# gereonsuch/gr-FDC

Hardware: AMD Instinct MI355X
Metric: complex Msamples/s in, 64k-FFT/256-ch overlap-save; achieved HBM GB/s vs peak (higher is better)
Workload: dtype f32

## Files before the change

gr-fdc_amd/__init__.py:

```python
from ._lib import FdcError, lib, LIB_PATH
from .blocks import overlap_save, vector_cut_vxx, phase_shifting_windowing_vcc, fft_vcc, window_table
from .channelizer import (FrequencyDomainChannelizer, Pipeline, PipelineGroup, IQ_SC16, IQ_SC8, OQ_FC32, plan_preview, FREQMODE, VERBOSEMODE, WINDOWTYPES,
                          nextpow2, get_opt_channelparams, freq_converters, register_host, unregister_host, defaults, fine_tuning_increment, fine_tuning_nu)
from ._lib import (FDC_PIPE_FORCE_GENERIC, FDC_PIPE_NO_POLY, FDC_PIPE_NO_BLOCK, FDC_PIPE_PLAIN_STORES, FDC_PIPE_NT_LOADS,
                   FDC_PIPE_FULL_SPECTRUM, FDC_PIPE_WIDE_UNIFORM, FDC_PIPE_NO_FUSED,
                   FDC_SINKS_HOST_DECISIONS, FDC_SINKS_DEVICE_PAYLOAD, FDC_SINKS_LOOKAHEAD)
from .waterfall import Waterfall, WaterfallImage, Rows as WaterfallRows
from .sharding import span_for_rank, ring_bounds, ring_for_span
from .sinks import Sinks, SinksGroup, PowerActivationChannel, activity_detection_channelizer_vcm, SegmentDetection
```

gr-fdc_amd/_lib.py:

```python
import ctypes as C
import os

_HERE = os.path.dirname(os.path.abspath(__file__))
LIB_PATH = os.environ.get("FDC_AMD_LIB") or os.path.join(_HERE, "libfdc_amd.so")

FDC_OK = 0
STATUS_NAMES = {0: "FDC_OK", -1: "FDC_ERR_INVALID_ARGUMENT", -2: "FDC_ERR_HIP", -3: "FDC_ERR_NO_DEVICE",
                -4: "FDC_ERR_UNSUPPORTED", -5: "FDC_ERR_NOMEM"}


class FdcError(RuntimeError):
    def __init__(self, status, text):
        self.status = status
        super().__init__("%s: %s" % (STATUS_NAMES.get(status, status), text))


class fdc_channel(C.Structure):
    _fields_ = [("f", C.c_int32), ("l", C.c_int32), ("passbw", C.c_float), ("stopbw", C.c_float)]


class fdc_pipeline_cfg(C.Structure):
    _fields_ = [("device_id", C.c_int32), ("blocklen", C.c_int32), ("relinvovl", C.c_int32),
                ("windowtype", C.c_int32), ("nchannels", C.c_int32), ("channels", C.POINTER(fdc_channel)),
                ("max_blocks", C.c_int32), ("chunk_blocks", C.c_int32), ("keep_spectrum", C.c_int32),
                ("flags", C.c_int32), ("min_block_launch", C.c_int32), ("host_sub_blocks", C.c_int32)]


FDC_PIPE_FORCE_GENERIC, FDC_PIPE_NO_POLY, FDC_PIPE_NO_BLOCK, FDC_PIPE_PLAIN_STORES, FDC_PIPE_NT_LOADS = 1, 2, 4, 8, 16
FDC_PIPE_FULL_SPECTRUM = 32
FDC_PIPE_WIDE_UNIFORM = 64
FDC_PIPE_NO_FUSED = 128


class fdc_pac_cfg(C.Structure):
    _fields_ = [("cfreq", C.c_float), ("bw", C.c_float), ("id", C.c_int32)]


class fdc_segment_cfg(C.Structure):
    _fields_ = [("start", C.c_float), ("stop", C.c_float)]


class fdc_sinks_cfg(C.Structure):
    _fields_ = [("device_id", C.c_int32), ("blocklen", C.c_int32), ("relinvovl", C.c_int32),
                ("npac", C.c_int32), ("pac", C.POINTER(fdc_pac_cfg)),
                ("pac_thresh_db", C.c_float), ("pac_maxblocks", C.c_int32), ("pac_deactivation_delay", C.c_int32),
                ("nseg", C.c_int32), ("seg", C.POINTER(fdc_segment_cfg)),
                ("det_thresh_db", C.c_float), ("det_maxblocks", C.c_int32), ("minchandist", C.c_float),
                ("det_deactivation_delay", C.c_int32), ("window_flank_puffer", C.c_double), ("max_blocks", C.c_int32),
                ("det_variant", C.c_int32), ("verbose", C.c_int32), ("det_id", C.c_int32), ("flags", C.c_int32),
                ("threads", C.c_int32), ("seg_id_base", C.c_int32)]


FDC_SINKS_HOST_DECISIONS = 1
FDC_SINKS_DEVICE_PAYLOAD = 2
FDC_SINKS_LOOKAHEAD = 4
FDC_OQ_FC32, FDC_OQ_SC16, FDC_OQ_SC8 = 0, 1, 2


class fdc_pdu(C.Structure):
    _fields_ = [("kind", C.c_int32), ("source", C.c_int32), ("chan_id", C.c_int32), ("finalized", C.c_int32),
                ("part", C.c_int32), ("has_part", C.c_int32), ("rel_bw", C.c_double), ("rel_cfreq", C.c_double),
                ("blockstart", C.c_int64), ("blockend", C.c_int64), ("vectorstart", C.c_int64),
                ("vectorend", C.c_int64), ("nsamples", C.c_int64), ("samples", C.c_void_p), ("id", C.c_char * 72)]


class fdc_waterfall_cfg(C.Structure):
    _fields_ = [("blocklen", C.c_int32), ("blockdecimation", C.c_int32), ("loginput", C.c_int32),
                ("minvaldb", C.c_double), ("maxvaldb", C.c_double), ("colorscheme", C.c_int32)]


_vp = C.c_void_p
SYMBOLS = {
    "fdc_last_error": (C.c_char_p, []),
    "fdc_version": (C.c_char_p, []),
    "fdc_device_count": (C.c_int, []),
    "fdc_selftest_devices": (C.c_int, []),
    "fdc_selftest_exception_barrier": (C.c_int, []),
    "fdc_pipeline_create": (C.c_int, [C.POINTER(fdc_pipeline_cfg), C.POINTER(_vp)]),
    "fdc_pipeline_destroy": (None, [_vp]),
    "fdc_pipeline_input_samples": (C.c_int64, [_vp, C.c_int]),
    "fdc_pipeline_output_samples": (C.c_int64, [_vp, C.c_int]),
    "fdc_pipeline_channel_offset": (C.c_int64, [_vp, C.c_int, C.c_int]),
    "fdc_pipeline_channel_lout": (C.c_int32, [_vp, C.c_int]),
    "fdc_pipeline_work": (C.c_int, [_vp, _vp, C.c_int, C.POINTER(_vp), _vp]),
    "fdc_pipeline_work_real": (C.c_int, [_vp, _vp, C.c_int, C.POINTER(_vp), _vp]),
    "fdc_pipeline_work_span": (C.c_int, [_vp, _vp, _vp, C.c_int64, C.c_int, C.POINTER(_vp), _vp]),
    "fdc_pipeline_work_span_real": (C.c_int, [_vp, _vp, _vp, C.c_int64, C.c_int, C.POINTER(_vp), _vp]),
    "fdc_pipeline_work_iq": (C.c_int, [_vp, C.c_int32, C.c_float, _vp, C.c_int, C.POINTER(_vp), _vp]),
    "fdc_pipeline_work_span_iq": (C.c_int, [_vp, C.c_int32, C.c_float, _vp, _vp, C.c_int64, C.c_int, C.POINTER(_vp), _vp]),
    "fdc_pipeline_process_device_iq": (C.c_int, [_vp, C.c_int32, C.c_float, _vp, C.c_int64, C.c_int, _vp, _vp, _vp]),
    "fdc_pipeline_group_work_iq": (C.c_int, [_vp, C.c_int32, C.c_float, _vp, C.c_int, C.POINTER(_vp), _vp]),
    "fdc_pipeline_set_output_format": (C.c_int, [_vp, C.c_int32, C.c_float]),
    "fdc_pipeline_group_set_output_format": (C.c_int, [_vp, C.c_int32, C.c_float]),
    "fdc_fine_tuning_increment": (C.c_int, [C.c_double, C.POINTER(C.c_uint64)]),
    "fdc_pipeline_set_fine_tuning": (C.c_int, [_vp, C.POINTER(C.c_double), C.c_int]),
    "fdc_pipeline_group_set_fine_tuning": (C.c_int, [_vp, C.POINTER(C.c_double), C.c_int]),
    "fdc_pipeline_group_create": (C.c_int, [C.POINTER(fdc_pipeline_cfg), C.POINTER(C.c_int32), C.c_int, C.c_int, C.POINTER(_vp)]),
    "fdc_pipeline_group_destroy": (None, [_vp]),
    "fdc_pipeline_group_work": (C.c_int, [_vp, _vp, C.c_int, C.POINTER(_vp), _vp]),
    "fdc_pipeline_group_work_real": (C.c_int, [_vp, _vp, C.c_int, C.POINTER(_vp), _vp]),
    "fdc_pipeline_group_reset": (None, [_vp]),
    "fdc_pipeline_group_size": (C.c_int32, [_vp]),
    "fdc_pipeline_group_member": (_vp, [_vp, C.c_int]),
    "fdc_pipeline_group_device": (C.c_int32, [_vp, C.c_int]),
    "fdc_pipeline_group_member_max_blocks": (C.c_int32, [_vp]),
    "fdc_pipeline_group_last_spans": (C.c_int, [_vp, C.POINTER(C.c_int64), C.POINTER(C.c_int32), C.c_int]),
    "fdc_host_register": (C.c_int, [_vp, C.c_size_t]),
    "fdc_host_unregister": (C.c_int, [_vp]),
    "fdc_pipeline_reset": (None, [_vp]),
    "fdc_pipeline_process_device": (C.c_int, [_vp, _vp, C.c_int64, C.c_int, _vp, _vp, _vp]),
    "fdc_pipeline_synchronize": (C.c_int, [_vp]),
    "fdc_pipeline_stream": (_vp, [_vp]),
    "fdc_pipeline_reserve_compute_units": (C.c_int, [_vp, C.c_int32]),
    "fdc_pipeline_chunk_blocks": (C.c_int32, [_vp]),
    "fdc_pipeline_path": (C.c_int32, [_vp]),
    "fdc_pipeline_describe": (C.c_int32, [_vp, C.c_char_p, C.c_int32]),
    "fdc_pipeline_plan_preview": (C.c_int, [C.POINTER(fdc_pipeline_cfg), C.c_char_p, C.c_int32, C.POINTER(C.c_int32)]),
    "fdc_pipeline_enable_timing": (C.c_int, [_vp, C.c_int]),
    "fdc_pipeline_last_kernel_ms": (C.c_int, [_vp, C.POINTER(C.c_float), C.c_int]),
    "fdc_sinks_create": (C.c_int, [C.POINTER(fdc_sinks_cfg), C.POINTER(_vp)]),
    "fdc_sinks_destroy": (None, [_vp]),
    "fdc_pipeline_work_spectrum": (C.c_int, [_vp, _vp, C.c_int, C.POINTER(_vp), _vp, _vp]),
    "fdc_pipeline_work_sinks": (C.c_int, [_vp, _vp, C.c_int, C.POINTER(_vp), _vp, _vp]),
    "fdc_device_numa_node": (C.c_int, [C.c_int]),
    "fdc_selftest_worker_placement": (C.c_int, [C.c_int, C.POINTER(C.c_int32), C.POINTER(C.c_int32)]),
    "fdc_pipeline_process_device_power": (C.c_int, [_vp, _vp, C.c_int64, C.c_int, _vp, _vp, _vp, _vp]),
    "fdc_sinks_group_power": (_vp, [_vp]),
    "fdc_sinks_group_power_ahead": (_vp, [_vp]),
    "fdc_sinks_prepare_from_groups": (C.c_int, [_vp, C.c_int, C.c_int]),
    "fdc_pipeline_flush_sinks": (C.c_int, [_vp, _vp]),
    "fdc_pipeline_sinks_latency": (C.c_int32, [_vp, _vp]),
    "fdc_sinks_work": (C.c_int, [_vp, _vp, C.c_int]),
    "fdc_sinks_work_band": (C.c_int, [_vp, _vp, C.c_int, C.c_int32, C.c_int32]),
    "fdc_sinks_read_band": (C.c_int, [_vp, C.POINTER(C.c_int32), C.POINTER(C.c_int32)]),
    "fdc_sinks_pdu_emit_items": (C.c_int, [_vp, C.POINTER(C.c_int32), C.c_int]),
    "fdc_sinks_pdu_emit_order": (C.c_int, [_vp, C.POINTER(C.c_int32), C.POINTER(C.c_int32), C.c_int]),
    "fdc_sinks_group_create": (C.c_int, [C.POINTER(fdc_sinks_cfg), C.POINTER(C.c_int32), C.c_int, C.POINTER(_vp)]),
    "fdc_sinks_group_destroy": (None, [_vp]),
    "fdc_sinks_group_work": (C.c_int, [_vp, _vp, C.c_int]),
    "fdc_sinks_group_pdu_count": (C.c_int, [_vp]),
    "fdc_sinks_group_pdus": (C.c_int, [_vp, C.POINTER(fdc_pdu), C.c_int]),
    "fdc_sinks_group_size": (C.c_int32, [_vp]),
    "fdc_sinks_group_member": (_vp, [_vp, C.c_int]),
    "fdc_sinks_group_member_info": (C.c_int, [_vp, C.c_int] + [C.POINTER(C.c_int32)] * 5),
    "fdc_sinks_spectrum": (_vp, [_vp]),
    "fdc_sinks_stream": (_vp, [_vp]),
    "fdc_sinks_spectrum_ahead": (_vp, [_vp]),
    "fdc_sinks_fill_stream": (_vp, [_vp]),
    "fdc_sinks_prepare": (C.c_int, [_vp, C.c_int, C.c_int]),
    "fdc_sinks_blocklen": (C.c_int32, [_vp]),
    "fdc_sinks_max_blocks": (C.c_int32, [_vp]),
    "fdc_sinks_work_device": (C.c_int, [_vp, C.c_int]),
    "fdc_sinks_submit_device": (C.c_int, [_vp, C.c_int]),
    "fdc_sinks_flush": (C.c_int, [_vp]),
    "fdc_sinks_engine": (C.c_int32, [_vp]),
    "fdc_sinks_set_payload_format": (C.c_int, [_vp, C.c_int32, C.c_float]),
    "fdc_sinks_payload_format": (C.c_int, [_vp, C.POINTER(C.c_int32), C.POINTER(C.c_float)]),
    "fdc_sinks_payload_route": (C.c_int32, [_vp]),
    "fdc_sinks_group_set_payload_format": (C.c_int, [_vp, C.c_int32, C.c_float]),
    "fdc_set_log_callback": (None, [_vp, _vp]),
    "fdc_sinks_pdu_count": (C.c_int, [_vp]),
    "fdc_sinks_pdu": (C.c_int, [_vp, C.c_int, C.POINTER(fdc_pdu)]),
    "fdc_sinks_pdus": (C.c_int, [_vp, C.POINTER(fdc_pdu), C.c_int]),
    "fdc_sinks_pac_params": (C.c_int, [_vp, C.c_int, C.POINTER(C.c_int32)]),
    "fdc_sinks_segment_params": (C.c_int, [_vp, C.c_int, C.POINTER(C.c_int32)]),
    "fdc_overlap_save_create": (C.c_int, [C.c_int, C.c_int, C.c_int, C.c_int, C.POINTER(_vp)]),
    "fdc_overlap_save_work": (C.c_int, [_vp, _vp, C.c_int, _vp]),
    "fdc_overlap_save_destroy": (None, [_vp]),
    "fdc_vector_cut_create": (C.c_int, [C.c_int, C.c_int, C.c_int, C.c_int, C.c_int, C.POINTER(_vp)]),
    "fdc_vector_cut_work": (C.c_int, [_vp, _vp, C.c_int, _vp]),
    "fdc_vector_cut_destroy": (None, [_vp]),
    "fdc_phase_window_create": (C.c_int, [C.c_int, C.c_int, C.c_int, C.c_int, C.c_float, C.c_float, C.c_int,
                                          C.POINTER(_vp)]),
    "fdc_phase_window_work": (C.c_int, [_vp, _vp, C.c_int, _vp]),
    "fdc_phase_window_destroy": (None, [_vp]),
    "fdc_window_table": (C.c_int, [C.c_int, C.c_int, C.c_float, C.c_float, C.c_int, C.c_int, C.c_int, _vp]),
    "fdc_fft_vcc": (C.c_int, [C.c_int, C.c_int, C.c_int, C.c_int, _vp, C.c_int, _vp]),
    "fdc_waterfall_check": (C.c_int, [C.POINTER(fdc_waterfall_cfg), C.POINTER(fdc_waterfall_cfg)]),
    "fdc_waterfall_create": (C.c_int, [C.c_int, C.POINTER(fdc_waterfall_cfg), C.c_int32, C.POINTER(_vp)]),
    "fdc_waterfall_destroy": (None, [_vp]),
    "fdc_waterfall_reset": (None, [_vp]),
    "fdc_waterfall_set_levels": (C.c_int, [_vp, C.c_double, C.c_double]),
    "fdc_waterfall_set_colorscheme": (C.c_int, [_vp, C.c_int32]),
    "fdc_waterfall_rows_done": (C.c_int64, [_vp]),
    "fdc_waterfall_color_table": (C.c_int, [C.c_int32, _vp, _vp]),
    "fdc_waterfall_edges": (C.c_int, [C.c_int32, C.c_double, C.c_double, _vp]),
    "fdc_waterfall_work": (C.c_int, [_vp, _vp, C.c_int, _vp, _vp, _vp, C.c_int, C.POINTER(C.c_int32)]),
    "fdc_pipeline_work_waterfall": (C.c_int, [_vp, _vp, _vp, C.c_int, C.POINTER(_vp), _vp, _vp, _vp, C.c_int,
                                              C.POINTER(C.c_int32)]),
}

_lib = None


def lib():
    global _lib
    if _lib is None:
        if not os.path.exists(LIB_PATH):
            raise ImportError("gr-fdc_amd: %s is missing — build it with `make -C gr-fdc_amd/csrc` "
                              "(or __graft_entry__.build()); there is no CPU fallback" % LIB_PATH)
        h = C.CDLL(LIB_PATH)
        for name, (res, args) in SYMBOLS.items():
            fn = getattr(h, name)
            fn.restype = res
            fn.argtypes = args
        _lib = h
    return _lib


def check(status):
    if status < 0:
        raise FdcError(status, lib().fdc_last_error().decode())
    return status
```

gr-fdc_amd/channelizer.py:

```python
import ctypes as C
import math

import numpy as np

from . import _lib


class FREQMODE:
    normalized, basebandfs, centerfreqfs = range(3)


class VERBOSEMODE:
    NOLOG, LOGTOCONSOLE, LOGTOFILE = range(3)


class WINDOWTYPES:
    RECTANGULAR, HANN, RAMP = range(3)


def nextpow2(k):
    if k < 1:
        raise ValueError('Cannot evaluate next power 2 of {}'.format(k))
    return 1 << int(math.ceil(math.log2(k)))


def get_opt_channelparams(blocksize, relinvovl, freq, bw):
    occupied = blocksize * bw
    l = nextpow2(occupied)
    if l < 1.2 * occupied:
        l *= 2
    passband = float(occupied) / float(l) * 1.1
    stopband = 1.0
    if passband >= 1.0:
        passband = 1.0
    elif passband < 0.7:
        stopband = passband + 0.25
    centre = int(_round_half_away(freq * blocksize)) % blocksize
    first = centre - l / 2
    if first < 0:
        first = (first + blocksize) % blocksize
    if first + l > blocksize:
        first = blocksize - l
    return int(first), int(l), int(l) - int(l) // relinvovl, float(passband), float(stopband)


def _round_half_away(x):
    ax = abs(x)
    r = math.floor(ax)
    if ax - r >= 0.5:
        r += 1.0
    return r if x >= 0 else -r


def freq_converters(freqmode, fs=1.0, centerfrequency=0.0):
    if freqmode in (FREQMODE.normalized, 'normalized'):
        return (FREQMODE.normalized, lambda f: (f + 0.5) % 1.0, lambda f: f - 0.5, lambda bw: bw % 1.0, lambda bw: bw)
    if freqmode in (FREQMODE.basebandfs, 'basebandfs'):
        return (FREQMODE.basebandfs, lambda f: (f / fs + 0.5) % 1.0, lambda f: (f - 0.5) * fs,
                lambda bw: (bw / fs) % 1.0, lambda bw: bw * fs)
    if freqmode in (FREQMODE.centerfreqfs, 'centerfreqfs'):
        return (FREQMODE.centerfreqfs, lambda f: ((f - centerfrequency) / fs + 0.5) % 1.0,
                lambda f: (f - 0.5) * fs + centerfrequency, lambda bw: (bw / fs) % 1.0, lambda bw: bw * fs)
    raise ValueError('Unknown Frequency mode. Exiting...')


def register_host(arr):
    _lib.check(_lib.lib().fdc_host_register(arr.ctypes.data, arr.nbytes))


def unregister_host(arr):
    _lib.check(_lib.lib().fdc_host_unregister(arr.ctypes.data))


defaults = {}


def _default_cfg_fields():
    flags = 0
    if defaults.get("FDC_FORCE_GENERIC"):
        flags |= _lib.FDC_PIPE_FORCE_GENERIC
    if defaults.get("FDC_NO_POLY"):
        flags |= _lib.FDC_PIPE_NO_POLY
    if defaults.get("FDC_NO_BLOCK"):
        flags |= _lib.FDC_PIPE_NO_BLOCK
    if defaults.get("FDC_FULL_SPECTRUM"):
        flags |= _lib.FDC_PIPE_FULL_SPECTRUM
    if defaults.get("FDC_WIDE_UNIFORM"):
        flags |= _lib.FDC_PIPE_WIDE_UNIFORM
    if defaults.get("FDC_NO_FUSED"):
        flags |= _lib.FDC_PIPE_NO_FUSED
    if "FDC_BLOCK_HINTS" in defaults:
        h = int(defaults["FDC_BLOCK_HINTS"])
        flags |= (0 if h & 1 else _lib.FDC_PIPE_PLAIN_STORES) | (_lib.FDC_PIPE_NT_LOADS if h & 2 else 0)
    return flags, int(defaults.get("FDC_BLOCK_MIN_BLOCKS", 0) or 0), int(defaults.get("FDC_HOST_SUB", 0) or 0)


def plan_preview(blocklen, relinvovl, channels, windowtype=WINDOWTYPES.HANN, max_blocks=64, flags=0):
    chans = [(int(f), int(l), float(p), float(s)) for (f, l, p, s) in channels]
    arr = (_lib.fdc_channel * max(1, len(chans)))()
    for i, (f, l, p, s) in enumerate(chans):
        arr[i].f, arr[i].l, arr[i].passbw, arr[i].stopbw = f, l, p, s
    cfg = _lib.fdc_pipeline_cfg(0, int(blocklen), int(relinvovl), int(windowtype), len(chans), arr, int(max_blocks), 0, 0, int(flags), 0, 0)
    buf = C.create_string_buffer(640)
    asg = (C.c_int32 * max(1, len(chans)))()
    rc = _lib.lib().fdc_pipeline_plan_preview(C.byref(cfg), buf, 640, asg)
    if rc == -1:
        raise ValueError(_lib.lib().fdc_last_error().decode())
    _lib.check(rc)
    return rc, buf.value.decode(), [int(asg[i]) for i in range(len(chans))]


IQ_SC16, IQ_SC8 = 1, 2
IQ_FORMATS = {"sc16": IQ_SC16, "sc8": IQ_SC8}


def iq_format(x):
    dt = np.asarray(x).dtype if not isinstance(x, np.dtype) else x
    if dt == np.int16:
        return IQ_SC16
    if dt == np.int8:
        return IQ_SC8
    raise TypeError("complex integer input is int16 (sc16) or int8 (sc8) interleaved I/Q, not %s" % dt)


def _iq_input(x, scale, H):
    if not isinstance(x, np.ndarray):
        raise TypeError("complex integer input must be a numpy int16 or int8 array")
    fmt = iq_format(x)
    if x.ndim == 2:
        if x.shape[1] != 2:
            raise ValueError("complex integer input of shape (n, 2) holds I and Q in its columns; got shape %s" % (x.shape,))
    elif x.ndim != 1:
        raise ValueError("complex integer input is a flat interleaved array or one of shape (n, 2); got shape %s" % (x.shape,))
    elif x.size % 2:
        raise ValueError("a flat interleaved I/Q array has an even number of values")
    n = x.size // 2
    if H and n % H:
        raise ValueError("input must be a whole number of (N - N/R)-sample items")
    with np.errstate(over="ignore"):
        sc = np.float32(scale)
    if not np.isfinite(sc) or sc == 0:
        raise ValueError("scale must be finite and not zero (float32), got %r" % (scale,))
    return np.ascontiguousarray(x), fmt, n, sc


OQ_FC32 = 0
OQ_FORMATS = {None: OQ_FC32, "fc32": OQ_FC32, "sc16": IQ_SC16, "sc8": IQ_SC8}
_OQ_DTYPES = {IQ_SC16: np.int16, IQ_SC8: np.int8}


def _oq_format(fmt, scale):
    if not (fmt is None or isinstance(fmt, str)) or fmt not in OQ_FORMATS:
        raise ValueError("output format is None, 'fc32', 'sc16' or 'sc8', not %r" % (fmt,))
    try:
        with np.errstate(over="ignore"):
            sc = np.float32(scale)
    except (TypeError, ValueError):
        raise ValueError("scale must be a finite, non-zero number, got %r" % (scale,))
    if not np.isfinite(sc) or sc == 0:
        raise ValueError("scale must be finite and not zero (float32), got %r" % (scale,))
    return OQ_FORMATS[fmt], sc


def fine_tuning_increment(nu):
    inc = C.c_uint64(0)
    rc = _lib.lib().fdc_fine_tuning_increment(float(nu), C.byref(inc))
    if rc == -1:
        raise ValueError(_lib.lib().fdc_last_error().decode())
    _lib.check(rc)
    return int(inc.value)


def fine_tuning_nu(blocksize, freq, f, l):
    d = float(freq) * blocksize - (f + l / 2.0)
    d -= blocksize * math.floor(d / blocksize + 0.5)
    return d / l


def _set_fine_tuning(fn, handle, nchan, nu):
    if nu is None:
        rc = fn(handle, None, nchan)
    else:
        arr = np.ascontiguousarray(nu, dtype=np.float64)
        if arr.ndim != 1:
            raise ValueError("fine tuning takes one frequency per channel")
        rc = fn(handle, arr.ctypes.data_as(C.POINTER(C.c_double)), int(arr.size))
    if rc == -1:
        raise ValueError(_lib.lib().fdc_last_error().decode())
    _lib.check(rc)


class _OutputFormat:
    _oq = OQ_FC32
    _oq_scale = np.float32(1.0)

    def output_format(self):
        return ({OQ_FC32: "fc32", IQ_SC16: "sc16", IQ_SC8: "sc8"}[self._oq], float(self._oq_scale))

    def _new_outs(self, nb):
        if self._oq == OQ_FC32:
            return [np.empty(nb * lo, dtype=np.complex64) for lo in self.lout]
        return [np.empty((nb * lo, 2), dtype=_OQ_DTYPES[self._oq]) for lo in self.lout]

    def _check_outs(self, outs, nb):
        if outs is None:
            return self._new_outs(nb)
        if len(outs) != len(self.lout):
            raise ValueError("outs needs one array per channel")
        dt = np.complex64 if self._oq == OQ_FC32 else _OQ_DTYPES[self._oq]
        per = 1 if self._oq == OQ_FC32 else 2
        for o, lo in zip(outs, self.lout):
            if not isinstance(o, np.ndarray) or o.dtype != dt or not o.flags.c_contiguous or o.size != per * nb * lo:
                if self._oq == OQ_FC32:
                    raise ValueError("outs[c] must be contiguous complex64 with nblocks*lout_c samples")
                raise ValueError("outs[c] must be contiguous %s with nblocks*lout_c interleaved I/Q samples (the output format)" % np.dtype(dt).name)
        return outs


class Pipeline(_OutputFormat):

    def __init__(self, blocklen, relinvovl, channels, windowtype=WINDOWTYPES.HANN, max_blocks=64,
                 device_id=0, chunk_blocks=0, keep_spectrum=False, flags=None, min_block_launch=None, host_sub_blocks=None):
        self._h = C.c_void_p()
        self.N, self.R = int(blocklen), int(relinvovl)
        self.channels = [(int(f), int(l), float(p), float(s)) for (f, l, p, s) in channels]
        arr = (_lib.fdc_channel * max(1, len(self.channels)))()
        for i, (f, l, p, s) in enumerate(self.channels):
            arr[i].f, arr[i].l, arr[i].passbw, arr[i].stopbw = f, l, p, s
        dflags, dmin, dsub = _default_cfg_fields()
        cfg = _lib.fdc_pipeline_cfg(device_id, self.N, self.R, int(windowtype), len(self.channels), arr,
                                    int(max_blocks), int(chunk_blocks), int(bool(keep_spectrum)),
                                    dflags if flags is None else int(flags), dmin if min_block_launch is None else int(min_block_launch),
                                    dsub if host_sub_blocks is None else int(host_sub_blocks))
        rc = _lib.lib().fdc_pipeline_create(C.byref(cfg), C.byref(self._h))
        if rc == -1:
            raise ValueError(_lib.lib().fdc_last_error().decode())
        _lib.check(rc)
        self.max_blocks = int(max_blocks)
        self.keep_spectrum = bool(keep_spectrum)
        self.ovl = self.N // self.R if self.N >= self.R else 0
        self.H = self.N - self.ovl
        self.lout = [_lib.lib().fdc_pipeline_channel_lout(self._h, c) for c in range(len(self.channels))]

    def output_samples(self, nblocks):
        return int(_lib.lib().fdc_pipeline_output_samples(self._h, nblocks))

    def channel_offset(self, c, nblocks):
        return int(_lib.lib().fdc_pipeline_channel_offset(self._h, c, nblocks))

    def set_output_format(self, fmt, scale=1.0):
        code, sc = _oq_format(fmt, scale)
        _lib.check(_lib.lib().fdc_pipeline_set_output_format(self._h, code, float(sc)))
        self._oq, self._oq_scale = code, sc if code else np.float32(1.0)

    def set_fine_tuning(self, nu):
        _set_fine_tuning(_lib.lib().fdc_pipeline_set_fine_tuning, self._h, len(self.channels), nu)

    def work(self, x, want_spectrum=False, sinks=None, outs=None):
        x = np.ascontiguousarray(x, dtype=np.complex64)
        if x.size % self.H:
            raise ValueError("input must be a whole number of (N - N/R)-sample items")
        nb = x.size // self.H
        outs = self._check_outs(outs, nb)
        ptrs = (C.c_void_p * max(1, len(outs)))(*[o.ctypes.data for o in outs])
        spec = np.empty(nb * self.N, dtype=np.complex64) if want_spectrum else None
        if sinks is not None:
            _lib.check(_lib.lib().fdc_pipeline_work_sinks(self._h, x.ctypes.data, nb, ptrs,
                                                         spec.ctypes.data if spec is not None else None, sinks._h))
        else:
            _lib.check(_lib.lib().fdc_pipeline_work(self._h, x.ctypes.data, nb, ptrs,
                                                   spec.ctypes.data if spec is not None else None))
        return (outs, spec) if want_spectrum else outs

    def work_waterfall(self, x, waterfall):
        from .waterfall import Rows, WIDTH
        x = np.ascontiguousarray(x, dtype=np.complex64)
        if x.size % self.H:
            raise ValueError("input must be a whole number of (N - N/R)-sample items")
        nb = x.size // self.H
        outs = [np.empty(nb * lo, dtype=np.complex64) for lo in self.lout]
        ptrs = (C.c_void_p * max(1, len(outs)))(*[o.ctypes.data for o in outs])
        cap = waterfall.rows_for(nb)
        rows, idx, rgb = np.empty((cap, WIDTH), np.float32), np.empty((cap, WIDTH), np.uint16), np.empty((cap, WIDTH, 3), np.uint8)
        n = C.c_int32(0)
        _lib.check(_lib.lib().fdc_pipeline_work_waterfall(self._h, waterfall._h, x.ctypes.data, nb, ptrs, rows.ctypes.data, idx.ctypes.data,
                                                          rgb.ctypes.data, cap, C.byref(n)))
        return outs, Rows(rows[:n.value], idx[:n.value], rgb[:n.value])

    def flush_sinks(self, sinks):
        return _lib.check(_lib.lib().fdc_pipeline_flush_sinks(self._h, sinks._h))

    def sinks_latency(self, sinks):
        return int(_lib.lib().fdc_pipeline_sinks_latency(self._h, sinks._h))

    def work_sinks_raw(self, in_ptr, nblocks, out_ptrs, sinks):
        return _lib.check(_lib.lib().fdc_pipeline_work_sinks(self._h, in_ptr, int(nblocks), out_ptrs, None, sinks._h))

    def work_real(self, x, want_spectrum=False):
        x = np.ascontiguousarray(x, dtype=np.float32)
        if x.size % self.H:
            raise ValueError("input must be a whole number of (N - N/R)-sample items")
        nb = x.size // self.H
        outs = self._new_outs(nb)
        ptrs = (C.c_void_p * max(1, len(outs)))(*[o.ctypes.data for o in outs])
        spec = np.empty(nb * self.N, dtype=np.complex64) if want_spectrum else None
        _lib.check(_lib.lib().fdc_pipeline_work_real(self._h, x.ctypes.data, nb, ptrs,
                                                    spec.ctypes.data if spec is not None else None))
        return (outs, spec) if want_spectrum else outs

    def work_iq(self, x, scale=1.0, want_spectrum=False, outs=None):
        x, fmt, n, sc = _iq_input(x, scale, self.H)
        nb = n // self.H
        outs = self._check_outs(outs, nb)
        ptrs = (C.c_void_p * max(1, len(outs)))(*[o.ctypes.data for o in outs])
        spec = np.empty(nb * self.N, dtype=np.complex64) if want_spectrum else None
        _lib.check(_lib.lib().fdc_pipeline_work_iq(self._h, fmt, float(sc), x.ctypes.data, nb, ptrs,
                                                  spec.ctypes.data if spec is not None else None))
        return (outs, spec) if want_spectrum else outs

    def work_span_iq(self, halo, x, first_block, scale=1.0, want_spectrum=False):
        x, fmt, n, sc = _iq_input(x, scale, self.H)
        hp = None
        if halo is not None:
            halo, hfmt, hn, _ = _iq_input(halo, scale, 0)
            if hfmt != fmt or hn != self.ovl:
                raise ValueError("halo: N/R samples of the input's format")
            hp = halo.ctypes.data
        nb = n // self.H
        outs = self._new_outs(nb)
        ptrs = (C.c_void_p * max(1, len(outs)))(*[o.ctypes.data for o in outs])
        spec = np.empty(nb * self.N, dtype=np.complex64) if want_spectrum else None
        _lib.check(_lib.lib().fdc_pipeline_work_span_iq(self._h, fmt, float(sc), hp, x.ctypes.data, int(first_block), nb, ptrs,
                                                       spec.ctypes.data if spec is not None else None))
        return (outs, spec) if want_spectrum else outs

    def work_raw(self, in_ptr, nblocks, out_ptrs):
        return _lib.check(_lib.lib().fdc_pipeline_work(self._h, in_ptr, int(nblocks), out_ptrs, None))

    def work_spectrum(self, spec_items, want_spectrum=False, sinks=None):
        spec_items = np.ascontiguousarray(spec_items, dtype=np.complex64)
        if spec_items.size % self.N:
            raise ValueError("input must be a whole number of N-sample spectrum items")
        nb = spec_items.size // self.N
        outs = [np.empty(nb * lo, dtype=np.complex64) for lo in self.lout]
        ptrs = (C.c_void_p * max(1, len(outs)))(*[o.ctypes.data for o in outs])
        spec = np.empty(nb * self.N, dtype=np.complex64) if want_spectrum else None
        _lib.check(_lib.lib().fdc_pipeline_work_spectrum(self._h, spec_items.ctypes.data, nb, ptrs,
                                                        spec.ctypes.data if spec is not None else None,
                                                        sinks._h if sinks is not None else None))
        return (outs, spec) if want_spectrum else outs

    def reset(self):
        _lib.lib().fdc_pipeline_reset(self._h)

    def process_device(self, d_ring, first_block, nblocks, d_out, d_spectrum=None, stream=None, d_group_power=None):
        if d_group_power:
            _lib.check(_lib.lib().fdc_pipeline_process_device_power(self._h, d_ring, int(first_block), int(nblocks), d_out, d_spectrum,
                                                                   d_group_power, stream))
        else:
            _lib.check(_lib.lib().fdc_pipeline_process_device(self._h, d_ring, int(first_block), int(nblocks), d_out,
                                                             d_spectrum, stream))

    def process_device_iq(self, fmt, scale, d_ring, first_block, nblocks, d_out, d_spectrum=None, stream=None):
        fmt = IQ_FORMATS.get(fmt, fmt) if isinstance(fmt, str) else int(fmt)
        if fmt not in (IQ_SC16, IQ_SC8):
            raise ValueError("fmt is 'sc16' or 'sc8'")
        _lib.check(_lib.lib().fdc_pipeline_process_device_iq(self._h, fmt, float(np.float32(scale)), d_ring, int(first_block), int(nblocks),
                                                            d_out, d_spectrum, stream))

    def synchronize(self):
        _lib.check(_lib.lib().fdc_pipeline_synchronize(self._h))

    def reserve_compute_units(self, n):
        return _lib.check(_lib.lib().fdc_pipeline_reserve_compute_units(self._h, int(n)))

    def stream(self):
        return _lib.lib().fdc_pipeline_stream(self._h)

    def enable_timing(self, on=True):
        _lib.check(_lib.lib().fdc_pipeline_enable_timing(self._h, int(on)))

    def last_kernel_ms(self):
        ms = (C.c_float * 4)()
        _lib.check(_lib.lib().fdc_pipeline_last_kernel_ms(self._h, ms, 4))
        return [float(v) for v in ms]

    def path(self):
        return int(_lib.lib().fdc_pipeline_path(self._h))

    def describe(self):
        buf = C.create_string_buffer(512)
        _lib.lib().fdc_pipeline_describe(self._h, buf, 512)
        return buf.value.decode()

    def chunk_blocks(self):
        return int(_lib.lib().fdc_pipeline_chunk_blocks(self._h))
# ... 340 lines not shown
```

gr-fdc_amd/csrc/fdc_api.hip:

```cpp
#include "fdc_pipeline.hpp"

#include <cstdarg>
#include <stdexcept>
#include <system_error>

using namespace fdc::pipe;

namespace {

thread_local std::string g_err;

struct HostRange { uintptr_t lo, hi, dev; };
std::mutex g_reg_mu;
std::vector<HostRange> g_reg;

}

namespace fdc {
const char *debug_env(const char *name)
{
    static const bool on = [] { const char *d = getenv("FDC_DEBUG_ENV"); return d && d[0] == '1'; }();
    return on ? getenv(name) : nullptr;
}
int set_error(int code, const char *fmt, ...)
{
    char buf[512];
    va_list ap;
    va_start(ap, fmt);
    vsnprintf(buf, sizeof buf, fmt, ap);
    va_end(ap);
    g_err = buf;
    return code;
}
int pick_device(int device_id)
{
    int n = 0;
    if (hipGetDeviceCount(&n) != hipSuccess || n <= 0)
        return set_error(FDC_ERR_NO_DEVICE, "no HIP device visible (this library has no CPU fallback)");
    if (device_id < 0 || device_id >= n) return set_error(FDC_ERR_INVALID_ARGUMENT, "device_id %d out of range [0,%d)", device_id, n);
    HIPCHK(hipSetDevice(device_id));
    static std::mutex mu;
    static std::vector<char> ready;
    std::lock_guard<std::mutex> lk(mu);
    if ((int)ready.size() < n) ready.resize((size_t)n, 0);
    if (!ready[(size_t)device_id]) {
        const hipError_t e = fdc::init_kernels();
        if (e != hipSuccess) return set_error(FDC_ERR_HIP, "kernel attribute setup failed: %s", hipGetErrorString(e));
        ready[(size_t)device_id] = 1;
    }
    return FDC_OK;
}

namespace pipe {
std::vector<float2> make_twiddles(int n)
{
    std::vector<float2> t(n);
    for (int k = 0; k < n; k++) {
        const double a = -2.0 * M_PI * double(k) / double(n);
        t[k] = make_float2(float(std::cos(a)), float(std::sin(a)));
    }
    return t;
}

bool host_registered(const void *ptr, size_t bytes, void **devptr)
{
    const uintptr_t a = reinterpret_cast<uintptr_t>(ptr);
    std::lock_guard<std::mutex> lk(g_reg_mu);
    for (const HostRange &r : g_reg)
        if (a >= r.lo && a + bytes <= r.hi) {
            if (devptr) *devptr = reinterpret_cast<void *>(r.dev + (a - r.lo));
            return true;
        }
    return false;
}

int out_staging(fdc_pipeline *p)
{
    if (p->sum_lout > 0 && !p->d_out) HIPCHK(p->d_out.alloc((size_t)p->cfg.max_blocks * p->sum_lout));
    return FDC_OK;
}
}
}

namespace fdc {
int pipeline_output_format(const fdc_pipeline *p, float *scale)
{
    if (scale) *scale = p->out_scale;
    return p->out_form;
}
}

extern "C" {

const char *fdc_last_error(void) { return g_err.c_str(); }
const char *fdc_version(void) { return "gr-fdc_amd 0.1 (gfx950)"; }

int fdc_device_count(void)
{
    int n = 0;
    if (hipGetDeviceCount(&n) != hipSuccess) return 0;
    return n;
}

int fdc_selftest_exception_barrier(void)
{
    struct Case { int kind, want; };
    const Case cases[] = {{0, FDC_ERR_NOMEM}, {1, FDC_ERR_NOMEM}, {2, FDC_ERR_HIP}, {3, FDC_ERR_HIP}, {4, 7}};
    for (const Case &c : cases) {
        const int got = fdc::guarded("fdc_selftest_exception_barrier", [&]() -> int {
            switch (c.kind) {
            case 0: throw std::bad_alloc();
            case 1: throw std::system_error(std::make_error_code(std::errc::resource_unavailable_try_again), "thread");
            case 2: throw std::runtime_error("runtime");
            case 3: throw 42;
            default: return 7;
            }
        });
        if (got != c.want) return set_error(FDC_ERR_HIP, "exception barrier: kind %d came back as %d, expected %d", c.kind, got, c.want);
        if (c.want < 0 && g_err.empty()) return set_error(FDC_ERR_HIP, "exception barrier: kind %d left no text", c.kind);
    }
    return FDC_OK;
}

int fdc_selftest_devices(void)
{
    FDC_ENTRY("fdc_selftest_devices")
    const int ndev = fdc_device_count();
    if (ndev <= 0) return set_error(FDC_ERR_NO_DEVICE, "no HIP device visible (this library has no CPU fallback)");
    constexpr int N = 65536, R = 2, C = 256, NB = 96, H = N - N / R, LOUT = 128;
    std::vector<fdc_channel> ch(C);
    for (int c = 0; c < C; c++) ch[(size_t)c] = fdc_channel{256 * c, 256, 0.88f, 1.0f};
    std::vector<float> x((size_t)2 * NB * H);
    uint32_t lcg = 12345u;
    for (float &v : x) { lcg = lcg * 1664525u + 1013904223u; v = (float)((int32_t)(lcg >> 8) - (1 << 23)) * (1.0f / (1 << 23)); }
    std::vector<std::vector<float>> out((size_t)C, std::vector<float>((size_t)2 * NB * LOUT));
    std::vector<void *> outs((size_t)C);
    for (int c = 0; c < C; c++) outs[(size_t)c] = out[(size_t)c].data();
    uint64_t ref = 0;
    auto checksum = [&](double *energy) {
        uint64_t h = 1469598103934665603ull;
        *energy = 0.0;
        for (int c = 0; c < C; c++) {
            const unsigned char *b = reinterpret_cast<const unsigned char *>(out[(size_t)c].data());
            for (size_t i = 0; i < out[(size_t)c].size() * sizeof(float); i++) { h ^= b[i]; h *= 1099511628211ull; }
            for (float v : out[(size_t)c]) *energy += (double)v * v;
        }
        return h;
    };
    fdc_pipeline_cfg cfg{};
    cfg.blocklen = N; cfg.relinvovl = R; cfg.windowtype = FDC_WIN_HANN; cfg.nchannels = C; cfg.channels = ch.data();
    cfg.max_blocks = NB; cfg.host_sub_blocks = NB;
    cfg.min_block_launch = 1;
    for (int d = 0; d < ndev; d++) {
        cfg.device_id = d;
        fdc_pipeline *p = nullptr;
        int rc = fdc_pipeline_create(&cfg, &p);
        if (rc != FDC_OK) return set_error(rc, "selftest: device %d: create failed: %s", d, std::string(g_err).c_str());
        if (fdc_pipeline_path(p) != 3) { fdc_pipeline_destroy(p); return set_error(FDC_ERR_UNSUPPORTED, "selftest: device %d: not on the one-kernel path", d); }
        rc = fdc_pipeline_work(p, x.data(), NB, outs.data(), nullptr);
        fdc_pipeline_destroy(p);
        if (rc != NB) return set_error(rc < 0 ? rc : FDC_ERR_HIP, "selftest: device %d: work failed: %s", d, std::string(g_err).c_str());
        double energy = 0.0;
        const uint64_t h = checksum(&energy);
        if (!(energy > 0.0)) return set_error(FDC_ERR_HIP, "selftest: device %d produced no output", d);
        if (d == 0) ref = h;
        else if (h != ref) return set_error(FDC_ERR_HIP, "selftest: device %d differs from device 0 (checksum %016llx vs %016llx)", d,
                                       (unsigned long long)h, (unsigned long long)ref);
    }
    {
        std::vector<int32_t> devs;
        for (int d = 0; d < std::max(ndev, 2); d++) devs.push_back(d % ndev);
        fdc_pipeline_group *g = nullptr;
        int rc = fdc_pipeline_group_create(&cfg, devs.data(), (int)devs.size(), 4, &g);
        if (rc != FDC_OK) return set_error(rc, "selftest: group over %d device(s): create failed: %s", ndev, std::string(g_err).c_str());
        for (auto &o : out) std::fill(o.begin(), o.end(), 0.0f);
        const int n1 = NB / 3, n2 = NB - n1;
        std::vector<void *> outs2((size_t)C);
        for (int c = 0; c < C; c++) outs2[(size_t)c] = out[(size_t)c].data() + (size_t)2 * n1 * LOUT;
        rc = fdc_pipeline_group_work(g, x.data(), n1, outs.data(), nullptr);
        if (rc == n1) rc = fdc_pipeline_group_work(g, x.data() + (size_t)2 * n1 * H, n2, outs2.data(), nullptr);
        fdc_pipeline_group_destroy(g);
        if (rc != n2) return set_error(rc < 0 ? rc : FDC_ERR_HIP, "selftest: group over %d device(s): work failed: %s", ndev, std::string(g_err).c_str());
        double energy = 0.0;
        const uint64_t h = checksum(&energy);
        if (h != ref) return set_error(FDC_ERR_HIP, "selftest: the group over %d device(s) differs from device 0 (checksum %016llx vs %016llx)", ndev,
                                  (unsigned long long)h, (unsigned long long)ref);
    }
    return ndev;
    FDC_ENTRY_END
}

int fdc_window_table(int windowtype, int blocklen, float passbw, float stopbw, int numphasestates, int step,
                     int normalize, float *w)
{
    FDC_ENTRY("fdc_window_table")
    if (blocklen < 1 || numphasestates < 1 || !w) return set_error(FDC_ERR_INVALID_ARGUMENT, "bad window table arguments");
    fdc::window_table(windowtype, blocklen, passbw, stopbw, numphasestates, step, normalize != 0,
                      reinterpret_cast<std::complex<float> *>(w));
    return FDC_OK;
    FDC_ENTRY_END
}

int fdc_host_register(void *ptr, size_t bytes)
{
    FDC_ENTRY("fdc_host_register")
    if (!ptr || !bytes) return set_error(FDC_ERR_INVALID_ARGUMENT, "fdc_host_register: empty range");
    int n = 0;
    if (hipGetDeviceCount(&n) != hipSuccess || n <= 0) return set_error(FDC_ERR_NO_DEVICE, "no HIP device visible");
    HIPCHK(hipHostRegister(ptr, bytes, hipHostRegisterMapped | hipHostRegisterPortable));
    void *dev = nullptr;
    hipError_t e = hipHostGetDevicePointer(&dev, ptr, 0);
    if (e != hipSuccess) { (void)hipHostUnregister(ptr); return set_error(FDC_ERR_HIP, "hipHostGetDevicePointer failed: %s", hipGetErrorString(e)); }
    const uintptr_t a = reinterpret_cast<uintptr_t>(ptr);
    std::lock_guard<std::mutex> lk(g_reg_mu);
    g_reg.push_back(HostRange{a, a + bytes, reinterpret_cast<uintptr_t>(dev)});
    return FDC_OK;
    FDC_ENTRY_END
}

int fdc_host_unregister(void *ptr)
{
    FDC_ENTRY("fdc_host_unregister")
    const uintptr_t a = reinterpret_cast<uintptr_t>(ptr);
    {
        std::lock_guard<std::mutex> lk(g_reg_mu);
        auto it = std::find_if(g_reg.begin(), g_reg.end(), [a](const HostRange &r) { return r.lo == a; });
        if (it == g_reg.end()) return set_error(FDC_ERR_INVALID_ARGUMENT, "fdc_host_unregister: range was not registered here");
        g_reg.erase(it);
    }
    HIPCHK(hipHostUnregister(ptr));
    return FDC_OK;
    FDC_ENTRY_END
}

void fdc_pipeline_destroy(fdc_pipeline *p)
{
    if (!p) return;
    if (p->stream) (void)hipStreamSynchronize(p->stream);
    if (p->ev_hier) { (void)hipEventSynchronize(p->ev_hier); (void)hipEventDestroy(p->ev_hier); }
    for (auto st : {p->s_in, p->s_out}) if (st) { (void)hipStreamSynchronize(st); (void)hipStreamDestroy(st); }
    for (auto e : p->events) (void)hipEventDestroy(e);
    for (int i = 0; i < 2; i++)
        for (auto e : {p->ev_in[i], p->ev_k[i], p->ev_out[i]}) if (e) (void)hipEventDestroy(e);
    if (p->stream) (void)hipStreamDestroy(p->stream);
    delete p;
}

int fdc_pipeline_create(const fdc_pipeline_cfg *cfg, fdc_pipeline **out)
{
    FDC_ENTRY("fdc_pipeline_create")
    if (!cfg || !out) return set_error(FDC_ERR_INVALID_ARGUMENT, "null argument");
    *out = nullptr;
    int rc = validate_cfg(cfg);
    if (rc != FDC_OK) return rc;
    rc = pick_device(cfg->device_id);
    if (rc != FDC_OK) return rc;

    fdc_pipeline *p = new fdc_pipeline();
    struct Owner { fdc_pipeline *p; ~Owner() { if (p) fdc_pipeline_destroy(p); } } owner{p};
    const int N = cfg->blocklen, R = cfg->relinvovl;
    p->cfg = *cfg; p->cfg.channels = nullptr;
    p->N = N; p->R = R; p->ovl = N / R; p->H = N - p->ovl; p->C = cfg->nchannels;
    std::vector<std::complex<float>> pool;
    build_channel_records(p, cfg, pool);

    const int flags = effective_flags(cfg->flags);
    p->cfg.flags = flags;
    p->cfg_generic = (flags & FDC_PIPE_FORCE_GENERIC) != 0;
    p->block_hints = ((flags & FDC_PIPE_PLAIN_STORES) ? 0 : 1) | ((flags & FDC_PIPE_NT_LOADS) ? 2 : 0);
    if (cfg->min_block_launch >= 1) p->block_min = cfg->min_block_launch;
    if (const char *bm = fdc::debug_env("FDC_BLOCK_MIN_BLOCKS")) if (atoi(bm) >= 1) p->block_min = atoi(bm);

    std::vector<int32_t> flat, rflat;
    group_by_width(p, nullptr, p->groups, p->group_off, p->g_aligned, p->g_out_aligned, flat);
    classify_plan(p, cfg, flags);
    if (p->split) group_by_width(p, &p->rem, p->rgroups, p->rgroup_off, p->rg_aligned, p->rg_out_aligned, rflat);

    int chunk = cfg->chunk_blocks;
    if (chunk <= 0) chunk = (int)std::max<int64_t>(1, (2048ll << 20) / (2ll * N * 8));
    p->chunk = std::min(chunk, cfg->max_blocks);

    rc = build_device_state(p, cfg, pool, flat, rflat);
    if (rc != FDC_OK) return rc;
    owner.p = nullptr;
    *out = p;
    return FDC_OK;
    FDC_ENTRY_END
}

int fdc_pipeline_plan_preview(const fdc_pipeline_cfg *cfg, char *buf, int32_t n, int32_t *assignment)
{
    FDC_ENTRY("fdc_pipeline_plan_preview")
    if (!cfg) return set_error(FDC_ERR_INVALID_ARGUMENT, "null argument");
    const int rc = validate_cfg(cfg);
    if (rc != FDC_OK) return rc;
    std::unique_ptr<fdc_pipeline> p(new fdc_pipeline());
    p->cfg = *cfg; p->cfg.channels = nullptr;
    p->N = cfg->blocklen; p->R = cfg->relinvovl; p->ovl = p->N / p->R; p->H = p->N - p->ovl; p->C = cfg->nchannels;
    std::vector<std::complex<float>> pool;
    build_channel_records(p.get(), cfg, pool);
    const int flags = effective_flags(cfg->flags);
    p->cfg.flags = flags;
    p->cfg_generic = (flags & FDC_PIPE_FORCE_GENERIC) != 0;
    classify_plan(p.get(), cfg, flags);
    if (assignment) {
        for (int c = 0; c < p->C; c++) assignment[c] = -1;
        for (size_t k = 0; k < p->banks.size(); k++) for (int c : p->banks[k].chan) assignment[c] = (int32_t)k;
        for (const auto &al : p->bank_alias) assignment[al.first] = -2 - al.second;
    }
    if (buf && n > 0) fdc_pipeline_describe(p.get(), buf, n);
    return fdc_pipeline_path(p.get());
    FDC_ENTRY_END
}

int64_t fdc_pipeline_input_samples(const fdc_pipeline *p, int nblocks) { return p ? (int64_t)nblocks * p->H : 0; }
int64_t fdc_pipeline_output_samples(const fdc_pipeline *p, int nblocks) { return p ? (int64_t)nblocks * p->sum_lout : 0; }
int64_t fdc_pipeline_channel_offset(const fdc_pipeline *p, int c, int nblocks)
{
    if (!p || c < 0 || c >= p->C) return -1;
    return (int64_t)nblocks * p->chans[c].out_off;
}
int32_t fdc_pipeline_channel_lout(const fdc_pipeline *p, int c)
{
    if (!p || c < 0 || c >= p->C) return -1;
    return p->chans[c].lout;
}
void *fdc_pipeline_stream(fdc_pipeline *p) { return p ? (void *)p->stream : nullptr; }
int fdc_pipeline_reserve_compute_units(fdc_pipeline *p, int32_t n)
{
    FDC_ENTRY("fdc_pipeline_reserve_compute_units")
    if (!p) return fdc::set_error(FDC_ERR_INVALID_ARGUMENT, "null handle");
    if (n < 0 || n >= p->ncu) return fdc::set_error(FDC_ERR_INVALID_ARGUMENT, "%d compute units of %d cannot be left out", (int)n, p->ncu);
    p->reserved_cu = n;
    p->reserve_user = n > 0;
    return p->ncu - n;
    FDC_ENTRY_END
}
int32_t fdc_pipeline_chunk_blocks(const fdc_pipeline *p) { return p ? p->chunk : -1; }
int32_t fdc_pipeline_path(const fdc_pipeline *p)
{
    if (!p) return -1;
    if (p->fused) return 5;
    if (p->poly_block && p->split) return 4;
    if (p->poly_block) return 3;
    if (p->poly_ok) return 2;
    if (p->fwd_block || (p->N == 65536 && !p->cfg_generic)) return 1;
    return 0;
}

int32_t fdc_pipeline_describe(const fdc_pipeline *p, char *buf, int32_t n)
{
    if (!p || !buf || n < 1) return -1;
    char t[640];
    const int path = fdc_pipeline_path(p);
    int k = std::snprintf(t, sizeof(t), "N = %d, R = %d, %d channels; path %d: ", p->N, p->R, p->C, path);
    auto add = [&](const char *fmt, auto... a) { if (k < (int)sizeof(t)) k += std::snprintf(t + k, sizeof(t) - (size_t)k, fmt, a...); };
    auto kernel = [](int L) { return L == 256 ? "k_blk256" : L == 512 ? "k_blk512" : L == 1024 ? "k_blk1024" : "k_blknar"; };
    auto where = [](int L, int r) { return r == 0 ? "on the grid" : 2 * r == L ? "half a channel off the grid" : 4 * r == L ? "a quarter of a channel off the grid" : "three quarters of a channel off the grid"; };
    if (p->fused) {
        int nw = 0;
        for (const auto &w : p->f4_wave) nw += !w.empty();
        add("k_f4096, transform + %d channel transforms in one launch (spectrum in LDS, %s per workgroup, rows on %d wave%s)", p->C,
            p->f4_teams == 1 ? "one block" : "two blocks", nw, nw == 1 ? "" : "s");
    } else if (p->poly_block) {
        bool one_width = true, all256 = true;
        for (const auto &b : p->banks) { one_width = one_width && b.L == p->banks[0].L; all256 = all256 && b.L == 256; }
        if (all256) {
            add("k_blk256, %d tiling%s (r =", (int)p->banks.size(), p->banks.size() == 1 ? "" : "s");
            for (const auto &b : p->banks) add(" %d", b.r);
            add("%s", ")");
        } else if (one_width) {
            add("%s, l = %d, bank of %d %s", kernel(p->banks[0].L), p->banks[0].L, (int)p->banks[0].chan.size(), where(p->banks[0].L, p->banks[0].r));
            for (size_t i = 1; i < p->banks.size(); i++) add(" + bank of %d %s", (int)p->banks[i].chan.size(), where(p->banks[i].L, p->banks[i].r));
        } else {
            for (size_t i = 0; i < p->banks.size(); i++) {
                const auto &b = p->banks[i];
                add("%s%s bank of %d, l = %d", i ? " + " : "", kernel(b.L), (int)b.chan.size(), b.L);
                if (b.L == 256) add(" (r = %d)", b.r); else add(" %s", where(b.L, b.r));
            }
        }
        if (p->banks.size() > 1 && !all256) add(" (%s launches)", p->banks.size() == 2 ? "two" : p->banks.size() == 3 ? "three" : "four");
        if (!p->bank_alias.empty()) add(" + %d copies of channels with the same slice", (int)p->bank_alias.size());
        if (p->split) add(" + %d other channels on a partial spectrum", (int)p->rem.size());
    } else if (p->poly_ok) {
        add("two launches (stage 1 + stage 2), l = %d", p->banks[0].L);
    } else {
        add("%s", "forward transform to a spectrum in memory + channel kernels");
    }
    if (!p->wf_route.empty()) add("; waterfall rows: %s", p->wf_route.c_str());
    if (!p->iq_route.empty()) add("; input %s", p->iq_route.c_str());
    if (!p->oq_route.empty()) add("; output %s", p->oq_route.c_str());
    if (!p->fine_route.empty()) add("; fine tuning: %s", p->fine_route.c_str());
    std::snprintf(buf, (size_t)n, "%s", t);
    return k;
}

int fdc_pipeline_synchronize(fdc_pipeline *p)
{
    FDC_ENTRY("fdc_pipeline_synchronize")
    if (!p) return set_error(FDC_ERR_INVALID_ARGUMENT, "null handle");
    HIPCHK(hipSetDevice(p->cfg.device_id));
    HIPCHK(hipStreamSynchronize(p->stream));
    return FDC_OK;
    FDC_ENTRY_END
}

int fdc_pipeline_enable_timing(fdc_pipeline *p, int enable)
{
    FDC_ENTRY("fdc_pipeline_enable_timing")
    if (!p) return set_error(FDC_ERR_INVALID_ARGUMENT, "null handle");
    p->timing = enable != 0;
    p->timing_stride = enable > 1 ? enable : 1;
    p->timing_seq = 0;
    p->ev_used = 0; p->ev_spans.clear();
    return FDC_OK;
    FDC_ENTRY_END
}

int fdc_pipeline_last_kernel_ms(fdc_pipeline *p, float *ms, int n)
{
    FDC_ENTRY("fdc_pipeline_last_kernel_ms")
    if (!p || !ms || n < 4) return set_error(FDC_ERR_INVALID_ARGUMENT, "need room for 4 values");
    ms[0] = ms[1] = ms[2] = 0.f;
    ms[3] = (float)p->ev_spans.size();
    for (auto &sp : p->ev_spans) {
        float a = 0, b = 0, c = 0;
        HIPCHK(hipEventSynchronize(p->events[sp[3]]));
        HIPCHK(hipEventElapsedTime(&a, p->events[sp[0]], p->events[sp[1]]));
        HIPCHK(hipEventElapsedTime(&b, p->events[sp[1]], p->events[sp[2]]));
        HIPCHK(hipEventElapsedTime(&c, p->events[sp[2]], p->events[sp[3]]));
        switch ((int)sp[4]) {
        case kSpanBanks: ms[0] += a; ms[1] += b; ms[2] += c; break;
        case kSpanTwoLaunch: ms[0] += a; ms[1] += c; break;
        case kSpanSpectrumLds: ms[1] += a + b; ms[2] += c; break;
        default: ms[0] += a; ms[1] += b; ms[2] += c;
        }
    }
    p->ev_used = 0; p->ev_spans.clear();
    return 4;
    FDC_ENTRY_END
}

void fdc_pipeline_reset(fdc_pipeline *p)
{
    if (!p) return;
    p->blockcount = 0;
    if (p->ev_hier && p->hier_ring_busy) (void)hipEventSynchronize(p->ev_hier);
    if (p->d_ring) {
        (void)hipSetDevice(p->cfg.device_id);
        (void)hipMemsetAsync(p->d_ring, 0, sizeof(float2) * (size_t)p->ovl, p->stream);
        if (p->d_iq) (void)hipMemsetAsync(p->d_iq, 0, fdc::kIqRingBytes * (size_t)p->ovl, p->stream);
        (void)hipStreamSynchronize(p->stream);
    }
    p->in_form = -1;
    p->in_scale = 0.f;
    p->iq_route.clear();
    p->oq_route.clear();
    p->fine_route.clear();
}

int fdc_pipeline_set_output_format(fdc_pipeline *p, int32_t format, float scale)
{
    FDC_ENTRY("fdc_pipeline_set_output_format")
    if (!p) return set_error(FDC_ERR_INVALID_ARGUMENT, "null handle");
    if (format != FDC_OQ_FC32 && format != FDC_OQ_SC16 && format != FDC_OQ_SC8) return set_error(FDC_ERR_INVALID_ARGUMENT, "unknown output format %d", (int)format);
    if (!std::isfinite(scale) || scale == 0.0f) return set_error(FDC_ERR_INVALID_ARGUMENT, "the output scale must be finite and not zero");
    if (p->hier_filled > 0)
        return set_error(FDC_ERR_INVALID_ARGUMENT, "a pipelined sinks batch is still inside the handle: fdc_pipeline_flush_sinks until it returns 0 first");
    if (format && !p->d_out) {
        HIPCHK(hipSetDevice(p->cfg.device_id));
        RCCHK(out_staging(p));
    }
    p->out_form = format;
    p->out_scale = format ? scale : 1.0f;
    return FDC_OK;
    FDC_ENTRY_END
}

int fdc_fine_tuning_increment(double nu, uint64_t *inc)
{
    FDC_ENTRY("fdc_fine_tuning_increment")
    if (!inc) return set_error(FDC_ERR_INVALID_ARGUMENT, "null argument");
    if (!(std::fabs(nu) < 0.5)) return set_error(FDC_ERR_INVALID_ARGUMENT, "the fine-tuning frequency must be inside (-0.5, 0.5) cycles per output sample");
    const double r = std::nearbyint(std::ldexp(nu, 64));
    *inc = r < 0 ? (uint64_t)0 - (uint64_t)(-r) : (uint64_t)r;
    return FDC_OK;
    FDC_ENTRY_END
}

int fdc_pipeline_set_fine_tuning(fdc_pipeline *p, const double *nu, int n)
{
    FDC_ENTRY("fdc_pipeline_set_fine_tuning")
    if (!p) return set_error(FDC_ERR_INVALID_ARGUMENT, "null handle");
    if (n != p->C) return set_error(FDC_ERR_INVALID_ARGUMENT, "fine tuning: %d frequencies for %d channels", n, p->C);
    if (p->hier_filled > 0)
        return set_error(FDC_ERR_INVALID_ARGUMENT, "a pipelined sinks batch is still inside the handle: fdc_pipeline_flush_sinks until it returns 0 first");
    std::vector<uint64_t> inc((size_t)p->C, 0);
    bool on = false;
    for (int c = 0; nu && c < p->C; c++) {
        RCCHK(fdc_fine_tuning_increment(nu[c], &inc[(size_t)c]));
        on = on || inc[(size_t)c] != 0;
    }
    if (!on) { p->fine_on = false; p->fine_route.clear(); return FDC_OK; }
    std::vector<fdc::FineChan> fc((size_t)p->C), f4(64, fdc::FineChan{0, 0});
    long long off = 0;
    for (int c = 0; c < p->C; c++) { fc[(size_t)c] = fdc::FineChan{inc[(size_t)c], off}; off += (p->chans[(size_t)c].lout + 1) & ~1; }
    std::vector<float2> step((size_t)off, make_float2(1.0f, 0.0f));
    for (int c = 0; c < p->C; c++)
        for (int j = 0; j < p->chans[(size_t)c].lout; j++)
            step[(size_t)(fc[(size_t)c].step_off + j)] = unit(std::ldexp((double)(inc[(size_t)c] * (uint64_t)j), -64));
    if (p->fused)
        for (int w = 0; w < 4 * p->f4_teams; w++)
            for (size_t k = 0; k < p->f4_wave[w].size() && k < 8; k++) f4[(size_t)(8 * w) + k] = fc[(size_t)(p->f4_wave[w][k] >> 1)];
    HIPCHK(hipSetDevice(p->cfg.device_id));
    HIPCHK(hipStreamSynchronize(p->stream));
    if (!p->d_fine) HIPCHK(p->d_fine.alloc(fc.size()));
    if (!p->d_fstep) HIPCHK(p->d_fstep.alloc(step.size()));
    if (p->fused && !p->d_f4fine) HIPCHK(p->d_f4fine.alloc(f4.size()));
    HIPCHK(hipMemcpy(p->d_fine, fc.data(), sizeof(fdc::FineChan) * fc.size(), hipMemcpyHostToDevice));
    HIPCHK(hipMemcpy(p->d_fstep, step.data(), sizeof(float2) * step.size(), hipMemcpyHostToDevice));
    if (p->fused) HIPCHK(hipMemcpy(p->d_f4fine, f4.data(), sizeof(fdc::FineChan) * f4.size(), hipMemcpyHostToDevice));
    p->fine_on = true;
    return FDC_OK;
    FDC_ENTRY_END
}

}
```

gr-fdc_amd/csrc/fdc_block256.hip:

```cpp
#include "fdc_blockcommon.hpp"
#include "fdc_iq.hpp"

namespace fdc {

extern __shared__ __attribute__((aligned(16))) unsigned char fdc_smem_blk[];

typedef unsigned long long u8v __attribute__((ext_vector_type(8)));

template <int P>
struct BlkGeom {
    static_assert(P == 2 || P == 4 || P == 8, "passes of 32 columns: N = 16384, 32768 or 65536");
    static constexpr int kN1 = 32 * P;
    static constexpr int kN = 256 * kN1;
    static constexpr int kJT = P == 8 ? 4 : 8;
    static constexpr int kJB = P == 8 ? 2 : P == 4 ? 4 : 8;
    static constexpr int kLd = P == 2 ? 32 * P + 2 : 32 * P + 6;
    static constexpr int kTripBytes = 16 * kJT * kLd * 8;
    static constexpr int kOffCt = kTripBytes > kStripsEnd ? kTripBytes : kStripsEnd;
    static constexpr int kOffWrow = P == 8 ? 136960 : kOffCt + 32 * P * 8;
    static constexpr int kOffB = kOffWrow + 16 * 18 * 8;
    static constexpr int kOffSA = kOffB + 32 * 18 * 8;
    static constexpr int kOffSoff = kOffSA + 16 * P * 18 * 8;
    static constexpr int kLds = kOffSoff + kN1 * 4;
    static constexpr int kOffSoffOff = kOffSA + 16 * P * 16 * 8;
    static constexpr int kOffWrowF = kOffSoffOff + kN1 * 4;
    static constexpr int kLdsOff = kOffWrowF + 16 * 18 * 8;
    static_assert(kLdsOff <= 160 * 1024 && kLds <= 160 * 1024, "LDS budget");
    static_assert(kOffCt >= kStripsEnd && kOffCt + 32 * P * 8 <= kOffWrow, "stage-2 trip buffer and twiddles below the tables, tables above the strips");
    static_assert((16 * (kJB - 1) * kLd + 32 * (P - 1)) * 8 < 65536, "ds offsets of a base register");
};


template <int P, bool NT, bool OFF, bool FWD, bool R4 = false, bool HALF = false, class TI = float2, class TO = float2>
__global__ FDC_PLAIN_DS __launch_bounds__(512, (P == 2 && !OFF && !R4 && !FWD) ? 4 : 2) void k_blk256(const TI *__restrict__ in, size_t in_stride, TO *__restrict__ out,
                                                const float2 *__restrict__ tw256, const float2 *__restrict__ twq,
                                                const float2 *__restrict__ cbt, const float *__restrict__ shn,
                                                const long long *__restrict__ slot_off, long long out_base,
                                                long long nb_call, unsigned out_bytes, int nb, int hints,
                                                unsigned long long *__restrict__ dbg , int roff, long long first_block,
                                                float2 *__restrict__ fwd_scratch, const unsigned *__restrict__ keep,
                                                typename IqTail<TI, TO>::type gpow )
{
    typedef BlkGeom<P> GM;
    constexpr bool kIq = !std::is_same<TI, float2>::value, kOq = !std::is_same<TO, float2>::value;
    static_assert(!kIq || !FWD, "integer input: the channelizer forms (the forward transform takes widened input)");
    static_assert(!kOq || !FWD, "integer output: the channelizer forms");
    constexpr unsigned kEs = (unsigned)sizeof(TI);
    constexpr unsigned kOs = (unsigned)sizeof(TO);
    [[maybe_unused]] const float iq_scale = iq_tail_scale(gpow);
    [[maybe_unused]] const float oq_scale = oq_tail_scale(gpow);
    static_assert(!HALF || (!OFF && !FWD), "the half-slot form is a variant of the on-grid channelizer");
    constexpr int kN1 = GM::kN1, kLd = GM::kLd, kJT = GM::kJT, kJB = GM::kJB;
    float2 *scr = reinterpret_cast<float2 *>(fdc_smem_blk);
    float2 *wrow = reinterpret_cast<float2 *>(fdc_smem_blk + GM::kOffWrow);
    float2 *Bt = reinterpret_cast<float2 *>(fdc_smem_blk + GM::kOffB);
    float2 *SA = reinterpret_cast<float2 *>(fdc_smem_blk + GM::kOffSA);
    constexpr int kSaLd = OFF ? 16 : 18;
    unsigned *soff = reinterpret_cast<unsigned *>(fdc_smem_blk + (OFF ? GM::kOffSoffOff : GM::kOffSoff));
    float2 *ctab = reinterpret_cast<float2 *>(fdc_smem_blk + GM::kOffCt);
    const int tid = threadIdx.x;
    const int w = tid >> 6, lane = tid & 63, col = lane & 3, b = lane >> 2, c5 = 4 * w + col;
    unsigned mqs[4] = {~0u, ~0u, ~0u, ~0u};
    if (FWD && keep) {
        const int wu = __builtin_amdgcn_readfirstlane(w) % P;
#pragma unroll
        for (int q = 0; q < 4; q++) mqs[q] = keep[wu * 4 + q];
    }

    const int grid = gridDim.x, first = xcd_first_block();
    if (first >= nb) return;

    constexpr unsigned inbytes = (unsigned)GM::kN * kEs;
    constexpr unsigned kRowGrp = (unsigned)kN1 * 16u * kEs;
    const unsigned voff = (unsigned)(b * kN1 + c5) * kEs;
    [[maybe_unused]] auto ld_in = [&](__amdgpu_buffer_rsrc_t r, unsigned soff, auto aux) __attribute__((always_inline)) -> cf {
        constexpr int kAux = decltype(aux)::value;
        if constexpr (sizeof(TI) == 4) return mk(__uint_as_float(__builtin_amdgcn_raw_buffer_load_b32(r, voff, soff, kAux)), 0.f);
        else return mk(__uint_as_float((unsigned)__builtin_amdgcn_raw_buffer_load_b16(r, voff, soff, kAux)), 0.f);
    };
    const __amdgpu_buffer_rsrc_t rcb = make_rsrc(cbt, (unsigned)kN1 * 16u * 8u);
    const unsigned voffc = (unsigned)(c5 * 16 + b) * 8u;
    cf LA[16], LB[16], cbA, cbB;
    {
        const __amdgpu_buffer_rsrc_t rin = make_rsrc(in + (size_t)first * in_stride, inbytes);
#pragma unroll
        for (int a = 0; a < 16; a++) {
            if constexpr (kIq) LA[a] = ld_in(rin, (unsigned)a * kRowGrp, std::integral_constant<int, 0>{});
            else LA[a] = bld2(rin, voff, (unsigned)a * kRowGrp);
        }
        cbA = bld2(rcb, voffc, 0);
    }
    float2 *wrowF = OFF ? reinterpret_cast<float2 *>(fdc_smem_blk + GM::kOffWrowF) : wrow;
    const int r16 = roff & 15;
    for (int i = tid; i < 256; i += 512) {
        wrow[(i >> 4) * 18 + (i & 15)] = tw256[((i >> 4) * (i & 15)) & 255];
        if (OFF)
            wrowF[(i >> 4) * 18 + (i & 15)] = tw256[((i >> 4) * ((((i & 15) - r16) & 15) + roff)) & 255];
    }
    for (int i = tid; i < kN1; i += 512) {
        const long long o = slot_off[i];
        soff[(i % P) * 32 + ((i / P) & 1) * 16 + rev16((i / P) >> 1)] = o >= 0 ? (unsigned)((o * nb_call + out_base) * kOs) : 0xFFFFFFFFu;
    }
    for (int i = tid; i < 32 * P; i += 512) ctab[i] = tw256[((i / P) * (i % P) * (8 / P)) & 255];
    Bt[(tid >> 4) * 18 + (tid & 15)] = twq[HALF ? tid ^ 8 : tid];
    for (int i = tid; i < 256 * P; i += 512) {
        const int ps = i >> 8, bb = (i >> 4) & 15, q = i & 15, qt = HALF ? q ^ 8 : q;
        const float2 t = twq[(size_t)(32 * ps) * 16 + qt];
        const float s = shn[bb + 16 * qt];
        SA[(ps * 16 + bb) * kSaLd + q] = make_float2(t.x * s, t.y * s);
    }
    __syncthreads();

    float2 *const scrw = scr + w * kStripPts + lane;
    const float2 *const scrr = scr + w * kStripPts + col + 68 * b;
    const float2 *const wr = wrow + b * 18;
    const float2 *const wrf = wrowF + b * 18;
    const float2 *const btr = Bt + c5 * 18;
    const __amdgpu_buffer_rsrc_t rout = make_rsrc(out, out_bytes);
    constexpr bool kScr = FWD || R4;
    const __amdgpu_buffer_rsrc_t rscr = make_rsrc(kScr ? fwd_scratch + (size_t)blockIdx.x * 32768 : fwd_scratch, kScr ? 32768u * 8u : 0u);


    for (int m = first; m < nb; m += grid) {
        const int mnext = m + grid < nb ? m + grid : m;
        const float sgn = (OFF && !R4 && (roff & 1) && ((first_block + m) & 1)) ? -1.0f : 1.0f;
        cf phs = mk(1.f, 0.f);
        if constexpr (OFF && R4) {
            const int pc = (int)((((first_block + m) & 3) * (roff & 3)) & 3);
            phs = mk(pc == 0 ? 1.f : pc == 2 ? -1.f : 0.f, pc == 1 ? 1.f : pc == 3 ? -1.f : 0.f);
        }
        typedef unsigned long long gvec __attribute__((ext_vector_type(P)));
        gvec G[8];
#define FDC_GGET(j, ps) unpack_cf(G[j][ps])
#define FDC_GPUT(j, ps, val) G[j][ps] = pack_cf(val)
        auto one_pass = [&](const int ps, cf (&cur)[16], const cf cbc, cf (&L)[16], cf &cbn) __attribute__((always_inline)) {
            const cf cb = (OFF && R4) ? cmul(cbc, phs) : OFF ? cbc * sgn : cbc;
            const int pn = ps < P - 1 ? ps + 1 : 0;
            const int mb = ps < P - 1 ? m : mnext;
            const __amdgpu_buffer_rsrc_t rin = make_rsrc(in + (size_t)mb * in_stride + 32 * pn, inbytes);
            if constexpr (kIq) {
                if (hints & 2) {
#pragma unroll
                    for (int a = 0; a < 16; a++) L[a] = ld_in(rin, (unsigned)a * kRowGrp, std::integral_constant<int, 2>{});
                } else {
#pragma unroll
                    for (int a = 0; a < 16; a++) L[a] = ld_in(rin, (unsigned)a * kRowGrp, std::integral_constant<int, 0>{});
                }
            } else if (hints & 2) {
#pragma unroll
                for (int a = 0; a < 16; a++) L[a] = bld2_nt(rin, voff, (unsigned)a * kRowGrp);
            } else {
#pragma unroll
                for (int a = 0; a < 16; a++) L[a] = bld2(rin, voff, (unsigned)a * kRowGrp);
            }
            cbn = bld2(rcb, voffc, (unsigned)pn * 4096u);
            if constexpr (kIq) {
#pragma unroll
                for (int a = 0; a < 16; a++) cur[a] = iq_widen_bits(TI{}, __float_as_uint(cur[a].x), iq_scale);
            }
            dft16<false>(cur);
            cf tw[16];
#pragma unroll
            for (int i = 0; i < 8; i++) {
                const float4 t = ld4(&wrf[2 * i]);
                tw[2 * i] = mk(t.x, t.y); tw[2 * i + 1] = mk(t.z, t.w);
            }
            if (OFF) {
#pragma unroll
                for (int p = 0; p < 16; p++) st2(&scrw[68 * ((p - r16) & 15)], cmul(cur[rev16(p)], tw[p]));
            } else {
                st2(&scrw[0], cur[rev16(0)]);
#pragma unroll
                for (int p = 1; p < 16; p++) st2(&scrw[68 * p], cmul(cur[rev16(p)], tw[p]));
            }
            __builtin_amdgcn_wave_barrier();
            cf v[16];
            strip_get(v, scrr);
            if constexpr (FWD) {
                dft16<false>(v);
                const float2 *sar = SA + (ps * 16 + b) * kSaLd;
#pragma unroll
                for (int i = 0; i < 8; i++) {
                    const float4 t0 = ld4(&btr[2 * i]), t1 = ld4(&sar[2 * i]);
                    const cf y0 = cmul(cmul(cmul(v[rev16(2 * i)], mk(t0.x, t0.y)), mk(t1.x, t1.y)), cb);
                    const cf y1 = cmul(cmul(cmul(v[rev16(2 * i + 1)], mk(t0.z, t0.w)), mk(t1.z, t1.w)), cb);
                    if (i < 4) { FDC_GPUT(2 * i, ps, y0); FDC_GPUT(2 * i + 1, ps, y1); }
                    else {
                        bst2(rscr, (unsigned)tid * 8u + (unsigned)(2 * i - 8) * 4096u, (unsigned)ps * 32768u, y0);
                        bst2(rscr, (unsigned)tid * 8u + (unsigned)(2 * i - 7) * 4096u, (unsigned)ps * 32768u, y1);
                    }
                }
            } else {
                dft16<false>(v);
                cf u[16];
                {
                    const float2 *sar = SA + (ps * 16 + b) * kSaLd;
#pragma unroll
                    for (int i = 0; i < 8; i++) {
                        const float4 t0 = ld4(&btr[2 * i]), t1 = ld4(&sar[2 * i]);
                        u[HALF ? 2 * i : (2 * i) ^ 8] = cmul(cmul(v[rev16(2 * i)], mk(t0.x, t0.y)), mk(t1.x, t1.y));
                        u[HALF ? 2 * i + 1 : (2 * i + 1) ^ 8] = cmul(cmul(v[rev16(2 * i + 1)], mk(t0.z, t0.w)), mk(t1.z, t1.w));
                    }
                }
                dft16<true>(u);
#pragma unroll
                for (int i = 0; i < 8; i++) {
                    const float4 t = ld4(&wr[2 * i]);
                    tw[2 * i] = mk(t.x, t.y); tw[2 * i + 1] = mk(t.z, t.w);
                }
                u[rev16(0)] = cmul(u[rev16(0)], cb);
#pragma unroll
                for (int p = 1; p < 16; p++) u[rev16(p)] = cmul(cmulc(u[rev16(p)], tw[p]), cb);
                strip_trip(u, scrw, scrr);
                dft16<true>(u);
#pragma unroll
                for (int j = 0; j < 8; j++) FDC_GPUT(j, ps, u[rev16(8 + j)]);
                if constexpr (R4) {
#pragma unroll
                    for (int j = 0; j < 4; j++) bst2(rscr, (unsigned)tid * 8u + (unsigned)j * 4096u, (unsigned)ps * 16384u, u[rev16(4 + j)]);
                }
            }
        };
        if constexpr (OFF && P == 8) {
#pragma nounroll
            for (int ps = 0; ps < P; ps++) {
                cf cur[16];
#pragma unroll
                for (int a = 0; a < 16; a++) cur[a] = LA[a];
                one_pass(ps, cur, cbA, LA, cbA);
            }
        } else {
#pragma nounroll
            for (int pp = 0; pp < P; pp += 2) {
                one_pass(pp, LA, cbA, LB, cbB);
                one_pass(pp + 1, LB, cbB, LA, cbA);
            }
        }
        auto stage2 = [&](auto get, const int rowbase, auto njc) __attribute__((always_inline)) {
            constexpr int kNJ = decltype(njc)::value;
            constexpr int kNTrip = (kNJ + kJT - 1) / kJT;
            __syncthreads();
            int t2 = tid;
            asm volatile("" : "+v"(t2));
            const int lane2 = t2 & 63, w2 = __builtin_amdgcn_readfirstlane(t2 >> 6), b_2 = lane2 >> 2, c5_2 = 4 * w2 + (lane2 & 3);
            const int klo2 = w2 % P, rh2 = w2 / P;
            float2 *const gw0 = scr + b_2 * kLd + c5_2;
            int rowjb = 16 * kJB * kLd;
            asm volatile("" : "+v"(rowjb));
            float2 *const gw1 = gw0 + rowjb;
            const float2 *const gr = scr + (64 * rh2 + lane2) * kLd + 32 * klo2;
            const uint4 *const sow = reinterpret_cast<const uint4 *>(soff + 32 * klo2);
#pragma unroll
            for (int tr = 0; tr < kNTrip; tr++) {
                const int ja = kNJ - kJT * tr < kJT ? kNJ - kJT * tr : kJT;
                cf ct[P];
                {
                    const float2 *ctr = reinterpret_cast<const float2 *>(fdc_smem_blk + GM::kOffCt) + c5_2 * P;
#pragma unroll
                    for (int i = 0; i < P / 2; i++) {
                        const float4 t = ld4(&ctr[2 * i]);
                        ct[2 * i] = mk(t.x, t.y); ct[2 * i + 1] = mk(t.z, t.w);
                    }
                }
                cf src[kJT][P];
#pragma unroll
                for (int jj = 0; jj < kJT; jj++)
#pragma unroll
                    for (int ps = 0; ps < P; ps++) if (jj < ja) src[jj][ps] = get(kJT * tr + jj, ps);
#pragma unroll
                for (int jj = 0; jj < kJT; jj++) {
                    if (jj >= ja) continue;
                    cf a[P];
#pragma unroll
                    for (int ps = 0; ps < P; ps++) a[ps] = src[jj][ps];
                    pass_dft<P>(a);
                    float2 *const gw = (jj < kJB ? gw0 : gw1) + (jj % kJB) * 16 * kLd;
                    st2(&gw[0], a[0]);
#pragma unroll
                    for (int k = 1; k < P; k++) st2(&gw[32 * k], cmul(a[pass_idx<P>(k)], ct[k]));
                }
                __builtin_amdgcn_sched_barrier(0);
                __syncthreads();
                const bool reads = P == 8 || 4 * rh2 < ja;
                cf v[32];
                if (reads) {
#pragma unroll
                    for (int i = 0; i < 16; i++) {
                        const float4 t = ld4(&gr[2 * i]);
                        v[2 * i] = mk(t.x, t.y); v[2 * i + 1] = mk(t.z, t.w);
                    }
                }
                __syncthreads();
                __builtin_amdgcn_sched_barrier(0);
                if (reads) {
                    dft32<false>(v);
                    const int trow0 = 16 * kJT * tr + 64 * rh2, trow = trow0 + lane2;
                    const unsigned rb = (unsigned)(m * (FWD ? GM::kN : (R4 ? 192 : 128)) + rowbase + trow) * kOs;
                    unsigned mq = FWD ? mqs[((rowbase + trow0) >> 6) & 3] : ~0u;
                    if constexpr (FWD) asm volatile("" : "+s"(mq));
#pragma unroll
                    for (int q = 0; q < 8; q++) {
                        const uint4 t = sow[q];
                        const unsigned so[4] = {t.x, t.y, t.z, t.w};
#pragma unroll
                        for (int e = 0; e < 4; e++) {
                            const unsigned o = FWD ? (so[e] | (((mq >> (4 * q + e)) & 1u) - 1u)) : so[e];
                            if constexpr (kOq) {
                                const unsigned u = oq_bits(TO{}, v[4 * q + e], oq_scale);
                                if constexpr (kOs == 4) __builtin_amdgcn_raw_buffer_store_b32(u, rout, (o == 0xFFFFFFFFu ? 0xFFFFFFF0u : o + rb), 0, NT ? 2 : 0);
                                else __builtin_amdgcn_raw_buffer_store_b16((unsigned short)u, rout, (o == 0xFFFFFFFFu ? 0xFFFFFFF0u : o + rb), 0, NT ? 2 : 0);
                            } else
                                bst2t<NT>(rout, (o == 0xFFFFFFFFu ? 0xFFFFFFF0u : o + rb), v[4 * q + e]);
                        }
                    }
                    if constexpr (FWD) {
                        if (gpow) {
                            float t16[16];
#pragma unroll
                            for (int i = 0; i < 16; i++) {
                                const float s0 = __builtin_fmaf(v[i].y, v[i].y, v[i].x * v[i].x);
                                const float s1 = __builtin_fmaf(v[i + 16].y, v[i + 16].y, v[i + 16].x * v[i + 16].x);
                                asm("s_nop 1\n\tv_add_f32_dpp %0, %1, %1 row_ror:8 row_mask:0xf bank_mask:0x3\n\t"
                                    "v_add_f32_dpp %0, %2, %2 row_ror:8 row_mask:0xf bank_mask:0xc" : "=&v"(t16[i]) : "v"(s0), "v"(s1));
                            }
                            float t8[8];
#pragma unroll
                            for (int i = 0; i < 8; i++)
                                asm("s_nop 1\n\tv_add_f32_dpp %0, %1, %1 row_shl:4 row_mask:0xf bank_mask:0x5\n\t"
                                    "v_add_f32_dpp %0, %2, %2 row_shr:4 row_mask:0xf bank_mask:0xa" : "=&v"(t8[i]) : "v"(t16[i]), "v"(t16[i + 8]));
                            const bool b1 = (lane2 & 2) != 0, b0 = (lane2 & 1) != 0;
                            float t4[4], t2[2];
#pragma unroll
                            for (int i = 0; i < 4; i++) {
                                const float keepv = b1 ? t8[i + 4] : t8[i], send = b1 ? t8[i] : t8[i + 4];
                                t4[i] = keepv + __builtin_bit_cast(float, __builtin_amdgcn_update_dpp(0, __builtin_bit_cast(int, send), 0x4E , 0xF, 0xF, false));
                            }
#pragma unroll
                            for (int i = 0; i < 2; i++) {
                                const float keepv = b0 ? t4[i + 2] : t4[i], send = b0 ? t4[i] : t4[i + 2];
                                t2[i] = keepv + __builtin_bit_cast(float, __builtin_amdgcn_update_dpp(0, __builtin_bit_cast(int, send), 0xB1 , 0xF, 0xF, false));
                            }
                            const int i16 = lane2 & 15, rho = lane2 >> 4, gsrc = 2 * (i16 & 1);
                            const int a0 = (16 * gsrc + 4 * rho + (i16 >> 2)) * 4, a1 = a0 + 64;
                            const int z0 = __builtin_bit_cast(int, t2[0]), z1 = __builtin_bit_cast(int, t2[1]);
                            const int f0a = __builtin_amdgcn_ds_bpermute(a0, z0), f0b = __builtin_amdgcn_ds_bpermute(a0, z1);
                            const int f1a = __builtin_amdgcn_ds_bpermute(a1, z0), f1b = __builtin_amdgcn_ds_bpermute(a1, z1);
                            const bool odd = (i16 & 2) != 0;
                            float2 pr;
                            pr.x = __builtin_bit_cast(float, odd ? f0b : f0a);
                            pr.y = __builtin_bit_cast(float, odd ? f1b : f1a);
                            const int reg = 8 * rho + (i16 >> 1), slot = klo2 + P * ((reg >> 4) + 2 * (4 * (reg & 3) + ((reg & 15) >> 2)));
                            *reinterpret_cast<float2 *>(gpow + (size_t)m * (GM::kN / 16) + 16 * slot + (rowbase + trow0) / 16 + gsrc) = pr;
                        }
                    }
                }
                __builtin_amdgcn_sched_barrier(0);
            }
        };
        stage2([&](int j, int ps) { return FDC_GGET(j, ps); }, R4 ? 64 : 0, std::integral_constant<int, 8>{});
        if constexpr (FWD) {
            asm volatile("s_waitcnt vmcnt(0)" ::: "memory");
            stage2([&](int j, int ps) { return bld2_sc1(rscr, (unsigned)tid * 8u + (unsigned)(j * 4096 + ps * 32768), 0u); }, 128,
                   std::integral_constant<int, 8>{});
        }
        if constexpr (R4) {
            asm volatile("s_waitcnt vmcnt(0)" ::: "memory");
            stage2([&](int j, int ps) { return bld2_sc1(rscr, (unsigned)tid * 8u + (unsigned)(j * 4096 + ps * 16384), 0u); }, 0,
                   std::integral_constant<int, 4>{});
        }
    }
}

template <class TI>
static hipError_t init_block_kernels_in()
{
    hipError_t e;
#define FDC_SETB(P, A, B, R4) \
    e = hipFuncSetAttribute(reinterpret_cast<const void *>(k_blk256<P, A, B, false, R4, false, TI>), hipFuncAttributeMaxDynamicSharedMemorySize, \
                            B ? BlkGeom<P>::kLdsOff : BlkGeom<P>::kLds); \
    if (e != hipSuccess) return e;
#define FDC_SETH(P, A, R4) \
    e = hipFuncSetAttribute(reinterpret_cast<const void *>(k_blk256<P, A, false, false, R4, true, TI>), hipFuncAttributeMaxDynamicSharedMemorySize, BlkGeom<P>::kLds); \
    if (e != hipSuccess) return e;
#define FDC_SETP(P) \
    FDC_SETB(P, true, false, false) FDC_SETB(P, false, false, false) FDC_SETB(P, true, true, false) FDC_SETB(P, false, true, false) \
    FDC_SETB(P, true, false, true) FDC_SETB(P, false, false, true) FDC_SETB(P, true, true, true) FDC_SETB(P, false, true, true) \
    FDC_SETH(P, true, false) FDC_SETH(P, false, false) FDC_SETH(P, true, true) FDC_SETH(P, false, true)
    FDC_SETP(2) FDC_SETP(4) FDC_SETP(8)
#undef FDC_SETP
#undef FDC_SETH
#undef FDC_SETB
    return hipSuccess;
}

template <class TI, class TO> struct kOqR4Narrowed {
    static constexpr bool value = std::is_same<TI, float2>::value && !std::is_same<TO, float2>::value;
};

template <class TI, class TO>
static hipError_t init_block_kernels_oq()
{
    hipError_t e;
#define FDC_SETB(P, B, R4) \
    e = hipFuncSetAttribute(reinterpret_cast<const void *>(k_blk256<P, true, B, false, R4, false, TI, TO>), hipFuncAttributeMaxDynamicSharedMemorySize, \
                            B ? BlkGeom<P>::kLdsOff : BlkGeom<P>::kLds); \
    if (e != hipSuccess) return e;
#define FDC_SETH(P, R4) \
    e = hipFuncSetAttribute(reinterpret_cast<const void *>(k_blk256<P, true, false, false, R4, true, TI, TO>), hipFuncAttributeMaxDynamicSharedMemorySize, BlkGeom<P>::kLds); \
    if (e != hipSuccess) return e;
#define FDC_SETP(P) \
    FDC_SETB(P, false, false) FDC_SETB(P, true, false) FDC_SETB(P, false, true) FDC_SETB(P, true, true) FDC_SETH(P, false) FDC_SETH(P, true)
    FDC_SETP(2) FDC_SETP(4)
    FDC_SETB(8, false, false) FDC_SETB(8, true, false) FDC_SETH(8, false)
    if constexpr (!kOqR4Narrowed<TI, TO>::value) { FDC_SETB(8, false, true) FDC_SETB(8, true, true) FDC_SETH(8, true) }
#undef FDC_SETP
#undef FDC_SETH
#undef FDC_SETB
    return hipSuccess;
}

hipError_t init_block_kernels()
{
    hipError_t e = init_block_kernels_in<sc16>();
    if (e != hipSuccess) return e;
    if ((e = init_block_kernels_in<sc8>()) != hipSuccess) return e;
    if ((e = init_block_kernels_oq<float2, sc16>()) != hipSuccess) return e;
    if ((e = init_block_kernels_oq<float2, sc8>()) != hipSuccess) return e;
    if ((e = init_block_kernels_oq<sc16, sc16>()) != hipSuccess) return e;
    if ((e = init_block_kernels_oq<sc16, sc8>()) != hipSuccess) return e;
    if ((e = init_block_kernels_oq<sc8, sc16>()) != hipSuccess) return e;
    if ((e = init_block_kernels_oq<sc8, sc8>()) != hipSuccess) return e;
#define FDC_SETB(P, A, B, F, R4) \
    e = hipFuncSetAttribute(reinterpret_cast<const void *>(k_blk256<P, A, B, F, R4>), hipFuncAttributeMaxDynamicSharedMemorySize, \
                            B ? BlkGeom<P>::kLdsOff : BlkGeom<P>::kLds); \
    if (e != hipSuccess) return e;
#define FDC_SETP(P) \
    FDC_SETB(P, true, false, false, false) FDC_SETB(P, false, false, false, false) FDC_SETB(P, true, true, false, false) \
    FDC_SETB(P, false, true, false, false) FDC_SETB(P, true, false, false, true) FDC_SETB(P, false, false, false, true) \
    FDC_SETB(P, true, true, false, true) FDC_SETB(P, false, true, false, true)
    FDC_SETP(2) FDC_SETP(4) FDC_SETP(8)
    FDC_SETB(8, true, false, true, false) FDC_SETB(8, false, false, true, false) FDC_SETB(4, true, false, true, false) FDC_SETB(4, false, false, true, false)
    FDC_SETB(2, true, false, true, false) FDC_SETB(2, false, false, true, false)
#undef FDC_SETP
#undef FDC_SETB
#define FDC_SETH(P, A, R4) \
    e = hipFuncSetAttribute(reinterpret_cast<const void *>(k_blk256<P, A, false, false, R4, true>), hipFuncAttributeMaxDynamicSharedMemorySize, BlkGeom<P>::kLds); \
    if (e != hipSuccess) return e;
#define FDC_SETHP(P) FDC_SETH(P, true, false) FDC_SETH(P, false, false) FDC_SETH(P, true, true) FDC_SETH(P, false, true)
    FDC_SETHP(2) FDC_SETHP(4) FDC_SETHP(8)
#undef FDC_SETHP
#undef FDC_SETH
    return hipSuccess;
}

bool poly_block_supports(int N) { return N == 16384 || N == 32768 || N == 65536; }

template <class TI, class TO = float2>
static hipError_t poly_block_in(const BlockLaunch &b, const TI *in, TO *out, float iq_scale, float oq_scale = 1.0f)
{
    if (b.nb_chunk <= 0) return hipSuccess;
    if (b.L != 256 || b.r < 0 || b.r >= 256) return hipErrorInvalidValue;
    constexpr bool kIq = !std::is_same<TI, float2>::value, kOq = !std::is_same<TO, float2>::value;
    const bool nt = (b.hints & 1) != 0, r4 = b.R == 4;
    if (kOq && !nt) return hipErrorInvalidValue;
    auto iq_tail = [](float si, float so) -> typename IqTail<TI, TO>::type {
        if constexpr (!kIq && !kOq) return (void)si, (void)so, (float *)nullptr;
        else if constexpr (kIq && kOq) return make_float2(si, so);
        else if constexpr (kIq) return (void)so, si;
        else return (void)si, so;
    };
    const bool halfslot = b.half();
    if (!poly_block_supports(b.N) || (b.R != 2 && !r4) || (r4 && !b.scratch)) return hipErrorInvalidValue;
    const int grid = b.grid(b.N == 16384 && b.R == 2 && (!b.r || halfslot) ? 2 : 1);
#define FDC_L(P, A, O, R4, H, roff) \
    hipExtLaunchKernelGGL((k_blk256<P, A || kOq, O, false, R4, H, TI, TO>), dim3((unsigned)grid), dim3(512), O ? BlkGeom<P>::kLdsOff : BlkGeom<P>::kLds, b.s, \
                          b.ev_start, b.ev_stop, 0u, in, b.in_stride, out, b.tw256, b.twq, b.cbt, b.shn, b.slot_off, (long long)b.mbase * (R4 ? 192 : 128), \
                          (long long)b.nb_call, b.out_bytes, b.nb_chunk, b.hints, (unsigned long long *)nullptr, roff, b.first_block, \
                          R4 ? b.scratch : (float2 *)nullptr, (const unsigned *)nullptr, iq_tail(iq_scale, oq_scale))
#define FDC_LB(P, A, O, R4) FDC_L(P, A, O, R4, false, b.r)
#define FDC_LH(P, A, R4) FDC_L(P, A, false, R4, true, 0)
#define FDC_R4(P) if constexpr (P != 8 || !kOqR4Narrowed<TI, TO>::value)
#define FDC_LP(P) \
    do { \
        if (halfslot) { \
            if (r4) { FDC_R4(P) { if (nt) FDC_LH(P, true, true); else FDC_LH(P, false, true); } else return hipErrorInvalidValue; } \
            else { if (nt) FDC_LH(P, true, false); else FDC_LH(P, false, false); } \
        } else if (r4 && b.r) { FDC_R4(P) { if (nt) FDC_LB(P, true, true, true); else FDC_LB(P, false, true, true); } else return hipErrorInvalidValue; } \
        else if (r4) { FDC_R4(P) { if (nt) FDC_LB(P, true, false, true); else FDC_LB(P, false, false, true); } else return hipErrorInvalidValue; } \
        else if (b.r) { if (nt) FDC_LB(P, true, true, false); else FDC_LB(P, false, true, false); } \
        else { if (nt) FDC_LB(P, true, false, false); else FDC_LB(P, false, false, false); } \
    } while (0)
    if (b.N == 65536) FDC_LP(8); else if (b.N == 32768) FDC_LP(4); else FDC_LP(2);
#undef FDC_LP
#undef FDC_R4
#undef FDC_LH
#undef FDC_LB
#undef FDC_L
    return hipGetLastError();
}

hipError_t launch_poly_block(const BlockLaunch &b) { return poly_block_in(b, b.in, b.out, 1.0f); }

hipError_t launch_poly_block_iq(const BlockLaunch &b, int fmt, float scale, const void *in)
{
    if (fmt == kIqSc16) return poly_block_in(b, static_cast<const sc16 *>(in), b.out, scale);
    if (fmt == kIqSc8) return poly_block_in(b, static_cast<const sc8 *>(in), b.out, scale);
    return hipErrorInvalidValue;
}

template <class TO>
static hipError_t poly_block_oq_in(const BlockLaunch &b, int ifmt, float iscale, const void *in, TO *out, float oscale)
{
    if (ifmt == kIqFloat) return poly_block_in<float2, TO>(b, static_cast<const float2 *>(in), out, 1.0f, oscale);
    if (ifmt == kIqSc16) return poly_block_in<sc16, TO>(b, static_cast<const sc16 *>(in), out, iscale, oscale);
    if (ifmt == kIqSc8) return poly_block_in<sc8, TO>(b, static_cast<const sc8 *>(in), out, iscale, oscale);
    return hipErrorInvalidValue;
}

hipError_t launch_poly_block_oq(const BlockLaunch &b, int ifmt, float iscale, const void *in, int ofmt, float oscale, void *out)
{
    if (ofmt == kIqSc16) return poly_block_oq_in(b, ifmt, iscale, in, static_cast<sc16 *>(out), oscale);
    if (ofmt == kIqSc8) return poly_block_oq_in(b, ifmt, iscale, in, static_cast<sc8 *>(out), oscale);
    return hipErrorInvalidValue;
}

hipError_t launch_block_fft(int N, const float2 *in, size_t in_stride, float2 *out, int nitems, const float2 *tw256,
                            const float2 *twq, const float2 *cbt0, const float *shn1, const long long *slot_off,
                            float2 *scratch , int ncu, int hints, hipStream_t s, hipEvent_t *ev,
                            const unsigned *keep, float *gpow )
{
    if (!poly_block_supports(N)) return hipErrorInvalidValue;
    const int per = (int)(((size_t)1 << 28) / (size_t)N);
    for (int m0 = 0; m0 < nitems; m0 += per) {
        const int nb = nitems - m0 < per ? nitems - m0 : per;
        int grid = ncu > 0 ? ncu : 256;
        if (grid > nb) grid = nb;
        hipEvent_t e0 = ev && m0 == 0 ? ev[0] : nullptr, e2 = ev && m0 + nb >= nitems ? ev[1] : nullptr;
#define FDC_LF(P, A) \
        hipExtLaunchKernelGGL((k_blk256<P, A, false, true>), dim3((unsigned)grid), dim3(512), BlkGeom<P>::kLds, s, e0, e2, 0u, in + (size_t)m0 * in_stride, \
                              in_stride, out + (size_t)m0 * (size_t)N, tw256, twq, cbt0, shn1, slot_off, 0ll, 1ll, \
                              (unsigned)((size_t)nb * (size_t)N * 8), nb, hints, (unsigned long long *)nullptr, 0, 0ll, scratch, keep, \
                              gpow ? gpow + (size_t)m0 * (size_t)(N / 16) : (float *)nullptr)
        const bool nt = (hints & 1) != 0;
        if (N == 65536) { if (nt) FDC_LF(8, true); else FDC_LF(8, false); }
        else if (N == 32768) { if (nt) FDC_LF(4, true); else FDC_LF(4, false); }
        else { if (nt) FDC_LF(2, true); else FDC_LF(2, false); }
#undef FDC_LF
    }
    if (ev) { hipError_t e = hipEventRecord(ev[2], s); if (e != hipSuccess) return e; }
    return hipGetLastError();
}

}
```

gr-fdc_amd/csrc/fdc_enqueue.hip:

```cpp
#include "fdc_pipeline.hpp"

namespace fdc { namespace pipe {

static int get_event(fdc_pipeline *p, size_t *idx)
{
    if (p->ev_used == p->events.size()) {
        hipEvent_t e;
        HIPCHK(hipEventCreate(&e));
        p->events.push_back(e);
    }
    *idx = p->ev_used++;
    return FDC_OK;
}

DeviceCall device_call(const fdc_pipeline *p, void *stream, void *d_spectrum, int fmt, float scale)
{
    DeviceCall call;
    call.fmt = fmt; call.scale = scale;
    call.stream = stream ? static_cast<hipStream_t>(stream) : p->stream;
    call.spectrum = d_spectrum;
    call.ncu = p->ncu - p->reserved_cu;
    return call;
}

int channels_wide(fdc_pipeline *p, const float2 *spec, float2 *d_out, const int32_t *d_gids, int ngroup, int l, const Span &span, hipStream_t s)
{
    const int nb = span.nb;
    const int per = (int)std::max<long long>(1, std::min<long long>(nb, (long long)p->big_pts / ((long long)ngroup * l)));
    const int lout = l - l / p->R;
    for (int m0 = 0; m0 < nb; m0 += per) {
        const int n = std::min(per, nb - m0);
        HIPCHK(fdc::launch_wide_tasks(p->d_wtasks, p->d_chans, d_gids, ngroup, p->R, n, span.m0 + m0, span.nblocks, span.first_block, s));
        HIPCHK(fdc::launch_extract_wide(spec + (size_t)m0 * p->N, p->N, p->d_wtasks, n * ngroup, l, l - lout, p->d_wins, p->d_big, d_out, p->d_tw, p->ntab, s,
                                        (float)l));
    }
    return FDC_OK;
}

static int run_channel_groups(fdc_pipeline *p, bool rem, const float2 *spec, float2 *d_out, const Span &span, hipStream_t s)
{
    const auto &groups = rem ? p->rgroups : p->groups;
    const auto &off = rem ? p->rgroup_off : p->group_off;
    const auto &al = rem ? p->rg_aligned : p->g_aligned;
    const auto &oal = rem ? p->rg_out_aligned : p->g_out_aligned;
    const int32_t *ids = rem ? p->d_rgroups : p->d_groups;
    for (size_t g = 0; g < groups.size(); g++) {
        const int l = groups[g].first, ng = (int)groups[g].second.size();
        if (l > 4096)
            RCCHK(channels_wide(p, spec, d_out, ids + off[g], ng, l, span, s));
        else if (l == 256 && ((256 / p->R) & 1) == 0 && !p->cfg_generic)
            HIPCHK(fdc::launch_channels256(spec, d_out, p->d_chans, ids + off[g], ng, al[g] != 0, oal[g] != 0, p->N, p->R, span.nb, span.m0, span.nblocks,
                                           span.first_block, p->d_wins, p->d_tw256, s));
        else if ((l == 512 || l == 1024) && l <= p->N && !p->cfg_generic)
            HIPCHK(fdc::launch_channels_wide(spec, d_out, p->d_chans, ids + off[g], ng, l, p->N, p->R, span.nb, span.m0, span.nblocks, span.first_block,
                                             p->d_wins, p->d_tw, p->ntab, s));
        else
            HIPCHK(fdc::launch_channels(spec, d_out, p->d_chans, ids + off[g], ng, l, p->N, p->R, span.nb, span.m0, span.nblocks, span.first_block, p->d_wins,
                                        p->d_tw, p->ntab, s));
    }
    return FDC_OK;
}

static int run_remainder(fdc_pipeline *p, const DeviceCall &call, const float2 *in0, float2 *d_out, const Span &span, hipEvent_t ev2, hipEvent_t ev3)
{
    hipStream_t s = call.stream;
    const int nb = span.nb;
    if (p->fwd_block && nb >= p->block_min)
        HIPCHK(fdc::launch_block_fft(p->N, in0, (size_t)p->H, p->d_spec, nb, p->d_tw256, p->d_ftwq, p->d_fcbt, p->d_fshn,
                                          p->d_fslot, p->d_fscr, call.ncu, p->block_hints, s, nullptr, p->d_keep));
    else if (p->N == 65536)
        HIPCHK(fdc::launch_fft65536(in0, (size_t)p->H, p->d_spec, p->d_tmp, nb, p->N / 2, 1.0f / (float)p->N, p->d_tw256,
                                    p->d_twf, s, nullptr));
    else
        HIPCHK(fdc::launch_fft(in0, (size_t)p->H, p->d_spec, p->d_tmp, p->N, nb, false, 0, p->N / 2, 1.0f / (float)p->N, p->d_tw, p->ntab,
                               s, nullptr, p->d_twf, p->cfg_generic));
    if (ev2) HIPCHK(hipEventRecord(ev2, s));
    RCCHK(run_channel_groups(p, true, p->d_spec, d_out, span, s));
    if (ev3) HIPCHK(hipEventRecord(ev3, s));
    return FDC_OK;
}

static int launch_bank(fdc_pipeline *p, const DeviceCall &call, const fdc_pipeline::Bank &bk, fdc::BlockLaunch b, const void *raw, void *oq)
{
    b.in_stride = (size_t)p->H;
    b.slot_off = bk.d_slot_off;
    b.ncu = call.ncu; b.hints = p->block_hints;
    b.s = call.stream;
    b.N = p->N; b.R = p->R; b.scratch = p->d_fscr;
    b.L = bk.L; b.r = bk.r;
    b.cbt = bk.d_cbt; b.shn = bk.d_shn; b.tab = bk.d_tab;
    b.tw256 = p->d_tw256;
    b.twq = bk.L == 512 ? p->d_twq512 : bk.L == 1024 ? p->d_twq1k : p->d_twq;
    b.twl = bk.L == 512 ? p->d_tw512 : bk.L == 1024 ? p->d_tw1k : nullptr;
    if (oq) {
        if (bk.L != 256) return set_error(FDC_ERR_UNSUPPORTED, "integer stores in a %d-bin bank", bk.L);
        HIPCHK(fdc::launch_poly_block_oq(b, raw ? call.fmt : 0, call.scale, raw ? raw : static_cast<const void *>(b.in), call.ofmt, call.oscale, oq));
        return FDC_OK;
    }
    if (raw) {
        if (bk.L != 256) return set_error(FDC_ERR_UNSUPPORTED, "integer loads in a %d-bin bank", bk.L);
        HIPCHK(fdc::launch_poly_block_iq(b, call.fmt, call.scale, raw));
        return FDC_OK;
    }
    switch (bk.L) {
    case 256: HIPCHK(fdc::launch_poly_block(b)); break;
    case 512: HIPCHK(fdc::launch_poly_block512(b)); break;
    case 1024: HIPCHK(fdc::launch_poly_block1024(b)); break;
    default: HIPCHK(fdc::launch_poly_block_narrow(b));
    }
    return FDC_OK;
}

static bool int_kernels(const fdc_pipeline *p, const DeviceCall &call)
{
    if (call.spectrum || call.rows || p->cfg_generic) return false;
    if (p->fused) return true;
    if (!p->poly_ok || !p->poly_block || p->split) return false;
    for (const auto &b : p->banks) if (b.L != 256) return false;
    return true;
}

static bool iq_fused(const fdc_pipeline *p, const DeviceCall &call, bool few)
{
    return int_kernels(p, call) && (p->fused || !(few && two_launch_possible(p)));
}

static bool oq_fused(const fdc_pipeline *p, const DeviceCall &call, int nblocks)
{
    if (!int_kernels(p, call)) return false;
    if (p->fused) return true;
    if (p->fine_on) return false;
    if (!(p->block_hints & 1) || (!call.fmt && p->N == 65536 && p->R == 4)) return false;
    for (int m0 = 0; m0 < nblocks; m0 += p->chunk)
        if (std::min(p->chunk, nblocks - m0) < p->block_min && two_launch_possible(p)) return false;
    return true;
}

int process_device_impl(fdc_pipeline *p, DeviceCall &call, const void *d_ring, int64_t first_block, int nblocks, void *d_out)
{
    if (nblocks < 0 || first_block < 0) return set_error(FDC_ERR_INVALID_ARGUMENT, "negative block count/index");
    if (nblocks == 0) return FDC_OK;
    if (!d_ring || (p->C > 0 && !d_out)) return set_error(FDC_ERR_INVALID_ARGUMENT, "null device buffer");
    void *const d_spectrum = call.spectrum;
    if (d_spectrum && !p->cfg.keep_spectrum && !call.own_spectrum) return set_error(FDC_ERR_INVALID_ARGUMENT, "spectrum output needs keep_spectrum");
    if ((int64_t)nblocks * p->sum_lout * 8 > 0xFFFFF000ll)
        return set_error(FDC_ERR_INVALID_ARGUMENT, "nblocks %d x %lld output samples per block is more than the 4 GiB one call may produce", nblocks, (long long)p->sum_lout);
    HIPCHK(hipSetDevice(p->cfg.device_id));
    hipStream_t s = call.stream;
    const int fmt = call.fmt, ofmt = call.ofmt;
    const float2 *ring = static_cast<const float2 *>(d_ring);
    const unsigned char *iring = static_cast<const unsigned char *>(d_ring);
    const size_t esz = fdc::iq_bytes(fmt);
    const bool ofused = ofmt && oq_fused(p, call, nblocks);
    call.ofused = ofused;
    if (ofmt && !ofused && !call.fout) return set_error(FDC_ERR_INVALID_ARGUMENT, "integer output: no float staging");
    float2 *o = ofmt && !ofused ? call.fout : static_cast<float2 *>(d_out);
    const size_t osz = ofused ? fdc::iq_bytes(ofmt) : sizeof(float2);
    unsigned char *const ob = ofused ? static_cast<unsigned char *>(d_out) : reinterpret_cast<unsigned char *>(o);
    const bool use_poly = p->poly_ok && !d_spectrum;
    const unsigned out_bytes = (unsigned)((int64_t)nblocks * p->sum_lout * (int64_t)osz);
    const bool fine = p->fine_on && p->C > 0, fine_fused = fine && p->fused && !d_spectrum;
    auto rotate = [&](const Span &g) -> int {
        if (fine) HIPCHK(fdc::launch_fine_rotate(o, p->d_chans, p->d_fine, p->d_fstep, p->C, g.nb, g.m0, g.nblocks, g.first_block, s));
        return FDC_OK;
    };
    for (int m0 = 0; m0 < nblocks; m0 += p->chunk) {
        const int nb = std::min(p->chunk, nblocks - m0);
        const Span grp{nb, m0, nblocks, first_block};
        float2 *spec = d_spectrum ? static_cast<float2 *>(d_spectrum) + (size_t)m0 * p->N : p->d_spec;
        hipEvent_t ev[3]; hipEvent_t *evp = nullptr; std::array<size_t, 5> span{};
        const bool tg = p->timing && (p->timing_seq++ % p->timing_stride) == 0;
        if (tg) {
            for (int i = 0; i < 4; i++) RCCHK(get_event(p, &span[i]));
            for (int i = 0; i < 3; i++) ev[i] = p->events[span[i]];
            evp = ev;
        }
        const float2 *in0 = ring + (size_t)m0 * p->H;
        const void *raw0 = iring + (size_t)m0 * p->H * esz;
        const bool few = nb < p->block_min;
        const bool ifused = fmt && iq_fused(p, call, few);
        if (fmt && !ifused) {
            HIPCHK(fdc::launch_iq_to_complex(fmt, call.scale, raw0, call.wide, (size_t)nb * p->H + (size_t)p->ovl, s));
            in0 = call.wide;
            call.all_fused = false;
        }
        if (p->fused && !d_spectrum) {
            if (tg) HIPCHK(hipEventRecord(p->events[span[0]], s));
            float *wf = call.rows ? call.rows + (size_t)(first_block - call.rows_first + m0) * fdc::kWfWidth : nullptr;
            if (fine_fused)
                HIPCHK(fdc::launch_fused4096_fine(ifused ? fmt : 0, call.scale, ifused ? raw0 : static_cast<const void *>(in0), (size_t)p->H, ofused ? ofmt : 0, call.oscale,
                                                  ofused ? d_out : static_cast<void *>(o), nb, p->R, m0, nblocks, first_block, p->d_tw, p->ntab, p->d_wins, p->d_f4rows,
                                                  p->f4_cls, p->f4_teams, p->d_f4fine, p->d_fstep, s));
            else if (ofused)
                HIPCHK(fdc::launch_fused4096_oq(ifused ? fmt : 0, call.scale, ifused ? raw0 : static_cast<const void *>(in0), (size_t)p->H, ofmt, call.oscale, d_out, nb,
                                                p->R, m0, nblocks, first_block, p->d_tw, p->ntab, p->d_wins, p->d_f4rows, p->f4_cls, p->f4_teams, s));
            else if (ifused)
                HIPCHK(fdc::launch_fused4096_iq(fmt, call.scale, raw0, (size_t)p->H, o, nb, p->R, m0, nblocks, first_block, p->d_tw, p->ntab, p->d_wins, p->d_f4rows,
                                                p->f4_cls, p->f4_teams, s));
            else
                HIPCHK(fdc::launch_fused4096(in0, (size_t)p->H, o, nb, p->R, m0, nblocks, first_block, p->d_tw, p->ntab, p->d_wins, p->d_f4rows, p->f4_cls, p->f4_teams, s, wf));
            if (tg) { HIPCHK(hipEventRecord(p->events[span[1]], s)); span[2] = span[3] = span[1]; span[4] = kSpanBanks; p->ev_spans.push_back(span); }
            continue;
        }
        if (use_poly && p->poly_block && !(few && two_launch_possible(p))) {
            fdc::BlockLaunch b{};
            b.in = in0; b.out = o;
            b.nb_chunk = nb; b.mbase = m0; b.nb_call = nblocks;
            b.first_block = first_block + m0; b.out_bytes = out_bytes;
            for (size_t k = 0; k < p->banks.size(); k++) {
                b.ev_start = tg && k == 0 ? p->events[span[0]] : nullptr;
                b.ev_stop = tg && k + 1 == p->banks.size() ? p->events[span[1]] : nullptr;
                RCCHK(launch_bank(p, call, p->banks[k], b, ifused ? raw0 : nullptr, ofused ? d_out : nullptr));
            }
            for (const auto &al : p->bank_alias) {
                const fdc::ChanDev &dc = p->chans[(size_t)al.first], &sc = p->chans[(size_t)al.second];
                HIPCHK(hipMemcpyAsync(ob + osz * ((size_t)nblocks * dc.out_off + (size_t)m0 * dc.lout), ob + osz * ((size_t)nblocks * sc.out_off + (size_t)m0 * sc.lout),
                                      osz * (size_t)nb * dc.lout, hipMemcpyDeviceToDevice, s));
            }
            if (p->split) RCCHK(run_remainder(p, call, in0, o, grp, tg ? p->events[span[2]] : nullptr, tg ? p->events[span[3]] : nullptr));
            else if (tg) span[2] = span[3] = span[1];
            if (tg) { span[4] = kSpanBanks; p->ev_spans.push_back(span); }
            RCCHK(rotate(grp));
            continue;
        }
        if (use_poly) {
            const fdc_pipeline::Bank &bk = p->banks[0];
            if (tg) HIPCHK(hipEventRecord(p->events[span[0]], s));
            if (bk.L != 256)
                HIPCHK(fdc::launch_poly_stage1_generic(in0, (size_t)p->H, p->d_g, p->N, bk.L, p->R, nb, bk.d_shn, p->d_tw, p->ntab, p->d_t2g, s));
            else
                HIPCHK(fdc::launch_poly_stage1(in0, (size_t)p->H, p->d_g, p->N / 256, p->R, nb, p->d_tw256, p->d_twq, bk.d_cbt, bk.d_shn, call.ncu, s));
            if (tg) { HIPCHK(hipEventRecord(p->events[span[1]], s)); span[2] = span[1]; }
            if (bk.L != 256)
                HIPCHK(fdc::launch_poly_stage2_generic(p->d_g, o, p->N / bk.L, p->R, nb, m0, nblocks, bk.d_slot_off, p->d_tw, p->ntab, s, bk.L));
            else if (p->N != 65536 && p->N != 262144)
                HIPCHK(fdc::launch_poly_stage2_generic(p->d_g, o, p->N / 256, p->R, nb, m0, nblocks, bk.d_slot_off, p->d_tw, p->ntab, s));
            else
                HIPCHK(fdc::launch_poly_stage2(p->d_g, o, p->N / 256, p->R, nb, m0, nblocks, p->d_tw256, p->d_tw1024, bk.d_slot_off, out_bytes, call.ncu, s));
            if (p->split) RCCHK(run_remainder(p, call, in0, o, grp, nullptr, nullptr));
            RCCHK(rotate(grp));
            if (tg) {
                HIPCHK(hipEventRecord(p->events[span[3]], s));
                span[4] = kSpanTwoLaunch;
                p->ev_spans.push_back(span);
            }
            continue;
        }
        float *const gp = (call.gpow && d_spectrum) ? call.gpow + (size_t)(spec - call.gpow_origin) / 16 : nullptr;
        if (p->fwd_block && !few)
            HIPCHK(fdc::launch_block_fft(p->N, in0, (size_t)p->H, spec, nb, p->d_tw256, p->d_ftwq, p->d_fcbt,
                                              p->d_fshn, p->d_fslot, p->d_fscr, call.ncu, p->block_hints, s, evp, d_spectrum ? nullptr : p->d_keep, gp));
        else {
            if (p->N == 65536 && !p->cfg_generic)
                HIPCHK(fdc::launch_fft65536(in0, (size_t)p->H, spec, p->d_tmp, nb, p->N / 2,
                                            1.0f / (float)p->N, p->d_tw256, p->d_twf, s, evp));
            else
                HIPCHK(fdc::launch_fft(in0, (size_t)p->H, spec, p->d_tmp, p->N, nb, false, 0, p->N / 2,
                                       1.0f / (float)p->N, p->d_tw, p->ntab, s, evp, p->d_twf, p->cfg_generic, d_spectrum ? ~0ull : p->keep4096));
            if (gp) HIPCHK(fdc::launch_group_power(spec, p->N, nb, gp, s));
        }
        RCCHK(run_channel_groups(p, false, spec, o, grp, s));
        RCCHK(rotate(grp));
        if (tg) {
            HIPCHK(hipEventRecord(p->events[span[3]], s));
            span[4] = p->N <= fdc::kMaxLdsFft ? kSpanSpectrumLds : kSpanSpectrum;
            p->ev_spans.push_back(span);
        }
    }
    if (ofmt && !ofused && call.narrow && p->C > 0) HIPCHK(fdc::launch_complex_to_iq(ofmt, call.oscale, call.fout, d_out, (size_t)nblocks * p->sum_lout, s));
    if (fine) p->fine_route = fine_fused ? "fused" : "rotated";
    return FDC_OK;
}

std::string route(int fmt, bool fused, const char *otherwise)
{
    return std::string(fmt == FDC_IQ_SC16 ? "sc16" : "sc8") + ": " + (fused ? "fused" : otherwise);
}

static int process_device_oq(fdc_pipeline *p, DeviceCall &call, const void *d_ring, int64_t first_block, int nblocks, void *d_out)
{
    const int ofmt = p->out_form;
    if (!ofmt || nblocks <= 0) return process_device_impl(p, call, d_ring, first_block, nblocks, d_out);
    call.ofmt = ofmt; call.oscale = p->out_scale; call.fout = p->d_out;
    if (!oq_fused(p, call, nblocks)) {
        if (nblocks > p->cfg.max_blocks)
            return set_error(FDC_ERR_INVALID_ARGUMENT, "integer output on this plan: nblocks %d above max_blocks %d", nblocks, p->cfg.max_blocks);
        if (!p->d_out && p->sum_lout > 0) return set_error(FDC_ERR_HIP, "integer output: no float staging");
    }
    const int rc = process_device_impl(p, call, d_ring, first_block, nblocks, d_out);
    if (rc == FDC_OK) p->oq_route = route(ofmt, call.ofused, "narrowed");
    return rc;
}

int check_iq_form(int32_t format, float scale)
{
    if (format != FDC_IQ_SC16 && format != FDC_IQ_SC8) return set_error(FDC_ERR_INVALID_ARGUMENT, "unknown complex integer format %d", (int)format);
    if (!std::isfinite(scale) || scale == 0.0f) return set_error(FDC_ERR_INVALID_ARGUMENT, "the scale must be finite and not zero");
    return FDC_OK;
}

} }

using namespace fdc::pipe;

extern "C" {

int fdc_pipeline_process_device(fdc_pipeline *p, const void *d_ring, int64_t first_block, int nblocks,
                                void *d_out, void *d_spectrum, void *stream)
{
    FDC_ENTRY("fdc_pipeline_process_device")
    if (!p) return set_error(FDC_ERR_INVALID_ARGUMENT, "null handle");
    DeviceCall call = device_call(p, stream, d_spectrum);
    return process_device_oq(p, call, d_ring, first_block, nblocks, d_out);
    FDC_ENTRY_END
}

int fdc_pipeline_process_device_iq(fdc_pipeline *p, int32_t format, float scale, const void *d_ring, int64_t first_block, int nblocks,
                                   void *d_out, void *d_spectrum, void *stream)
{
    FDC_ENTRY("fdc_pipeline_process_device_iq")
    if (!p) return set_error(FDC_ERR_INVALID_ARGUMENT, "null handle");
    RCCHK(check_iq_form(format, scale));
    if (reinterpret_cast<uintptr_t>(d_ring) & 3) return set_error(FDC_ERR_INVALID_ARGUMENT, "the integer ring must be 4-byte aligned");
    DeviceCall call = device_call(p, stream, d_spectrum, format, scale);
    if (nblocks > 0 && !p->d_iqw) {
        bool need = false;
        for (int m0 = 0; m0 < nblocks && !need; m0 += p->chunk) need = !iq_fused(p, call, std::min(p->chunk, nblocks - m0) < p->block_min);
        if (need) {
            HIPCHK(hipSetDevice(p->cfg.device_id));
            HIPCHK(p->d_iqw.alloc((size_t)p->chunk * p->H + (size_t)p->ovl));
        }
    }
    call.wide = p->d_iqw;
    const int rc = process_device_oq(p, call, d_ring, first_block, nblocks, d_out);
    if (rc == FDC_OK && nblocks > 0) p->iq_route = route(format, call.all_fused, "widened");
    return rc;
    FDC_ENTRY_END
}

int fdc_pipeline_process_device_power(fdc_pipeline *p, const void *d_ring, int64_t first_block, int nblocks, void *d_out, void *d_spectrum,
                                      void *d_group_power, void *stream)
{
    FDC_ENTRY("fdc_pipeline_process_device_power")
    if (!p) return set_error(FDC_ERR_INVALID_ARGUMENT, "null handle");
    if (p->out_form) return set_error(FDC_ERR_INVALID_ARGUMENT, "fdc_pipeline_process_device_power writes complex float outputs only (the handle's output format is not FC32)");
    if (p->fine_on) return set_error(FDC_ERR_INVALID_ARGUMENT, "fdc_pipeline_process_device_power writes the channels as they are cut: switch fine tuning off first");
    if (d_group_power && (!d_spectrum || (p->N & 15))) return set_error(FDC_ERR_INVALID_ARGUMENT, "group powers go with a spectrum output of a block length that is a multiple of 16");
    DeviceCall call = device_call(p, stream, d_spectrum);
    call.gpow = static_cast<float *>(d_group_power);
    call.gpow_origin = static_cast<const float2 *>(d_spectrum);
    return process_device_impl(p, call, d_ring, first_block, nblocks, d_out);
    FDC_ENTRY_END
}

}
```

gr-fdc_amd/csrc/fdc_kernels.h:

```cpp
#pragma once
#include <hip/hip_runtime.h>
#include <stdint.h>

namespace fdc {

constexpr int kThreads = 256;
constexpr int kMaxLdsFft = 8192;

struct ChanDev {
    int32_t f;
    int32_t l;
    int32_t lout;
    int32_t shift;
    int64_t out_off;
    int32_t win_off;
    int32_t pad;
};

struct PowerCell { int32_t start, len; float scale; int32_t pad; };
struct ExtractTask {
    int32_t slot;
    int32_t start;
    int32_t win_off;
    int32_t pad;
    int64_t out_off;
};

struct TileGeom {
    int L, log2L, TC, log2TC, ld, NB;
    size_t lds_bytes() const { return (size_t)L * ld * sizeof(float2); }
};
TileGeom tile_geom(int L);

struct BigGeom { int N, N1, N2; TileGeom a , b ; };
BigGeom big_geom(int N);

hipError_t init_kernels();

hipError_t launch_fft(const float2 *in, size_t in_stride, float2 *out, float2 *tmp, int N, int nitems,
                      bool inverse, int in_rot, int out_rot, float scale, const float2 *tw, int ntab,
                      hipStream_t s, hipEvent_t *ev ,
                      const float2 *twf = nullptr ,
                      bool generic_only = false ,
                      unsigned long long keep4096 = ~0ull );

hipError_t launch_channels(const float2 *spec, float2 *out, const ChanDev *chans, const int32_t *group,
                           int ngroup, int l, int N, int R, int nb_chunk, int mbase, int nb_call,
                           int64_t first_block, const float2 *wins, const float2 *tw, int ntab, hipStream_t s);

hipError_t init_fast_kernels();
hipError_t launch_fft65536(const float2 *in, size_t in_stride, float2 *out, float2 *tmp, int nitems, int out_rot,
                           float scale, const float2 *tw256, const float2 *twf, hipStream_t s, hipEvent_t *ev);
hipError_t launch_channels256(const float2 *spec, float2 *out, const ChanDev *chans, const int32_t *group,
                              int ngroup, bool aligned, bool out_aligned, int N, int R, int nb_chunk, int mbase,
                              int nb_call, int64_t first_block, const float2 *wins, const float2 *tw256,
                              hipStream_t s);

hipError_t init_wide_kernels();
hipError_t launch_channels_wide(const float2 *spec, float2 *out, const ChanDev *chans, const int32_t *group, int ngroup, int l,
                                int N, int R, int nb_chunk, int mbase, int nb_call, int64_t first_block, const float2 *wins,
                                const float2 *tw, int ntab, hipStream_t s);

hipError_t launch_fft4096(const float2 *in, size_t in_stride, float2 *out, int nitems, bool inverse, int in_rot, int out_rot,
                          float scale, const float2 *tw, int ntab, hipStream_t s,
                          unsigned long long keep = ~0ull );

struct F4Row { int32_t f, win_off, shift, xch, lout, valid; long long out_off; };
hipError_t init_fused4096_kernels();
int fused4096_tile_points();
hipError_t launch_fused4096(const float2 *in, size_t in_stride, float2 *out, int nb_chunk, int R, int mbase, int nb_call, int64_t first_block,
                            const float2 *tw, int ntab, const float2 *wins, const F4Row *rows, unsigned wcls, int teams , hipStream_t s,
                            float *wf = nullptr );
hipError_t launch_fused4096_iq(int fmt, float scale, const void *in, size_t in_stride, float2 *out, int nb_chunk, int R, int mbase, int nb_call,
                               int64_t first_block, const float2 *tw, int ntab, const float2 *wins, const F4Row *rows, unsigned wcls, int teams, hipStream_t s);
hipError_t launch_fused4096_oq(int ifmt, float iscale, const void *in, size_t in_stride, int ofmt, float oscale, void *out, int nb_chunk, int R, int mbase,
                               int nb_call, int64_t first_block, const float2 *tw, int ntab, const float2 *wins, const F4Row *rows, unsigned wcls, int teams,
                               hipStream_t s);

struct FineChan;
hipError_t launch_fused4096_fine(int ifmt, float iscale, const void *in, size_t in_stride, int ofmt, float oscale, void *out, int nb_chunk, int R, int mbase,
                                 int nb_call, int64_t first_block, const float2 *tw, int ntab, const float2 *wins, const F4Row *rows, unsigned wcls, int teams,
                                 const FineChan *fine_rows, const float2 *fine_step, hipStream_t s);

struct ScatterEnt { float2 *dst; long long out_off; int lout; int pad; };
hipError_t launch_scatter_out(const float2 *src, const ScatterEnt *tab, int nchan, int nb, long long row0, hipStream_t s);
hipError_t launch_scatter_oq(int src_fmt, const void *src, int ofmt, float scale, const ScatterEnt *tab, int nchan, int nb, long long row0, hipStream_t s);

hipError_t launch_poly_stage1(const float2 *in, size_t in_stride, float2 *g, int N1, int R, int nb_chunk,
                              const float2 *tw256, const float2 *twq, const float2 *cbt, const float *shn,
                              int ncu , hipStream_t s);
hipError_t launch_poly_stage2(const float2 *g, float2 *out, int N1 , int R, int nb_chunk, int mbase,
                              int nb_call, const float2 *tw256, const float2 *tw1024 ,
                              const long long *slot_off, unsigned out_bytes ,
                              int ncu, hipStream_t s);

hipError_t launch_poly_stage2_generic(const float2 *g, float2 *out, int N1, int R, int nb_chunk, int mbase, int nb_call,
                                      const long long *slot_off, const float2 *tw, int ntab, hipStream_t s,
                                      int L = 256 );
hipError_t launch_poly_stage1_generic(const float2 *in, size_t in_stride, float2 *g, int N, int L, int R, int nb_chunk, const float *shn,
                                      const float2 *tw, int ntab, const float2 *t2, hipStream_t s);
int poly_stage1_generic_tile_columns(int N, int L);

struct BlockLaunch {
    const float2 *in;
    size_t in_stride;
    float2 *out;
    int nb_chunk, mbase, nb_call;
    const long long *slot_off;
    unsigned out_bytes;
    int ncu;
    int hints;
    hipStream_t s;
    hipEvent_t ev_start, ev_stop;
    int N, R;
    float2 *scratch;
    int L, r;
    long long first_block;
    const float2 *cbt;
    const float *shn;
    const float2 *tw256, *twq;
    const float2 *twl;
    const float2 *tab;

    bool half() const { return r == L / 2; }
    int grid(int per_cu = 1) const
    {
        const int g = (ncu > 0 ? ncu : 256) * per_cu;
        return g > nb_chunk ? nb_chunk : g;
    }
};

hipError_t init_block_kernels();
hipError_t launch_poly_block(const BlockLaunch &b);
hipError_t launch_poly_block_iq(const BlockLaunch &b, int fmt, float scale, const void *in);
hipError_t launch_poly_block_oq(const BlockLaunch &b, int ifmt, float iscale, const void *in, int ofmt, float oscale, void *out);
bool poly_block_supports(int N);

hipError_t init_block512_kernels();
hipError_t launch_poly_block512(const BlockLaunch &b);
bool poly_block512_supports(int N, int R);

hipError_t init_block1024_kernels();
hipError_t launch_poly_block1024(const BlockLaunch &b);
bool poly_block1024_supports(int N, int R);

bool poly_block_narrow_supports(int N, int L, int R);
hipError_t init_block_narrow_kernels();
int poly_block_narrow_table_points(int L, int N);
void poly_block_narrow_tables(int L, int N, const float *shn, float2 *img, bool half = false ,
                              int r = 0 );
hipError_t launch_poly_block_narrow(const BlockLaunch &b);

hipError_t launch_block_fft(int N, const float2 *in, size_t in_stride, float2 *out, int nitems, const float2 *tw256,
                            const float2 *twq, const float2 *cbt0 , const float *shn1 ,
                            const long long *slot_off , float2 *scratch ,
                            int ncu, int hints, hipStream_t s,
                            hipEvent_t *ev ,
                            const unsigned *keep = nullptr ,
                            float *gpow = nullptr );
hipError_t launch_cell_power_groups(const float2 *spec, const float *gpow, int N, const PowerCell *cells, int ncells, int nblocks, float *out, hipStream_t s);
hipError_t launch_group_power(const float2 *spec, int N, int nblocks, float *gpow, hipStream_t s);

hipError_t launch_real_to_complex(const float *in, float2 *out, size_t n, hipStream_t s);
hipError_t launch_iq_to_complex(int fmt, float scale, const void *in, float2 *out, size_t n, hipStream_t s);
hipError_t launch_complex_to_iq(int fmt, float scale, const float2 *in, void *out, size_t n, hipStream_t s);

hipError_t launch_fine_rotate(float2 *out, const ChanDev *chans, const FineChan *fine, const float2 *step, int nchan, int nb_chunk, int mbase, int nb_call,
                              int64_t first_block, hipStream_t s);

hipError_t launch_scale(const float2 *in, float2 *out, size_t n, float k, hipStream_t s);

hipError_t launch_cell_power(const float2 *spec, int N, const PowerCell *cells, int ncells, int nblocks, float *out,
                             hipStream_t s);
hipError_t launch_extract_wide(const float2 *spec, int N, const ExtractTask *tasks, int ntasks, int w, int skip, const float2 *wins,
                               float2 *tmp, float2 *out, const float2 *tw, int ntab, hipStream_t s, float scale = 1.0f);
hipError_t launch_wide_tasks(ExtractTask *tasks, const ChanDev *chans, const int32_t *group, int ngroup, int R, int nb_chunk, int mbase, int nb_call,
                             int64_t first_block, hipStream_t s);
constexpr int kMaxExtractClasses = 12;
struct ExtractClass { int32_t tile0, task0, ntasks, log2w, log2TC, ld, skip, pad; };
struct ExtractClasses { ExtractClass c[kMaxExtractClasses]; int32_t n; };
hipError_t launch_extract_multi(const float2 *spec, int N, const ExtractTask *tasks, const int *w, const size_t *first, const size_t *cnt,
                                int nclass, int R, const float2 *wins, float2 *out, const float2 *tw, int ntab, hipStream_t s);
hipError_t launch_extract(const float2 *spec, int N, const ExtractTask *tasks, int ntasks, int w, int skip,
                          const float2 *wins, float2 *out, const float2 *tw, int ntab, hipStream_t s);

hipError_t launch_extract256(const float2 *spec, int N, const ExtractTask *tasks, int ntasks, int skip, const float2 *wins, float2 *out,
                             const float2 *tw256, hipStream_t s);
hipError_t launch_extract256_narrow(int fmt, float scale, const float2 *spec, int N, const ExtractTask *tasks, int ntasks, int skip, const float2 *wins,
                                    float2 *out, void *nout, long long used_a, const float2 *tw256, hipStream_t s);

hipError_t launch_overlap_save(const unsigned char *ring, unsigned char *out, size_t in_item_bytes,
                               size_t out_item_bytes, int nitems, hipStream_t s);
hipError_t launch_vector_cut(const unsigned char *in, unsigned char *out, size_t in_item_bytes, size_t shift_bytes,
                             size_t out_item_bytes, int nitems, hipStream_t s);
hipError_t launch_phase_window(const float2 *in, float2 *out, const float2 *win, int l, int R, int shift,
                               int counter0, int nitems, hipStream_t s);

}
```

gr-fdc_amd/csrc/fdc_pipeline.hpp:

```cpp
#pragma once
#include "../../include/fdc_amd.h"
#include "fdc_buffers.hpp"
#include "fdc_kernels.h"
#include "fdc_window.hpp"
#include "fdc_guard.hpp"
#include "fdc_plan_cost.hpp"
#include "fdc_waterfall.hpp"
#include "fdc_iq.hpp"
#include "fdc_fine.hpp"

#include <algorithm>
#include <array>
#include <cmath>
#include <complex>
#include <cstdio>
#include <cstdlib>
#include <cstring>
#include <memory>
#include <mutex>
#include <string>
#include <utility>
#include <vector>

namespace fdc {
int pick_device(int device_id);
const char *debug_env(const char *name);
}
using fdc::pick_device;
using fdc::set_error;

#define HIPCHK(expr)                                                                                        \
    do {                                                                                                    \
        hipError_t _e = (expr);                                                                             \
        if (_e != hipSuccess) return set_error(FDC_ERR_HIP, "%s failed: %s", #expr, hipGetErrorString(_e)); \
    } while (0)
#define RCCHK(expr) do { const int _rc = (expr); if (_rc != FDC_OK) return _rc; } while (0)
#define CHK_DEV(expr)                                                                           \
    do {                                                                                        \
        hipError_t _e = (expr);                                                                 \
        if (_e != hipSuccess)                                                                   \
            return set_error(_e == hipErrorOutOfMemory ? FDC_ERR_NOMEM : FDC_ERR_HIP, "%s failed: %s", #expr, hipGetErrorString(_e)); \
    } while (0)

#define FDC_ENTRY(name) return fdc::guarded(name, [&]() -> int {
#define FDC_ENTRY_END });

constexpr int kBlockMinBlocks = 96;

struct fdc_pipeline {
    fdc_pipeline_cfg cfg{};
    int N = 0, R = 0, ovl = 0, H = 0, C = 0;
    int chunk = 0;
    int64_t sum_lout = 0;
    std::vector<fdc::ChanDev> chans;
    std::vector<std::pair<int, std::vector<int32_t>>> groups;
    std::vector<size_t> group_off;
    hipStream_t stream = nullptr;
    fdc::DevBuf<float2> d_tw; int ntab = 0;
    fdc::DevBuf<float2> d_wins;
    fdc::DevBuf<float2> d_tw256;
    fdc::DevBuf<float2> d_tw1024;
    fdc::DevBuf<float2> d_twf;
    std::vector<char> g_aligned, g_out_aligned;
    struct Bank {
        int L = 256, r = 0;
        float passbw = 0, stopbw = 0;
        std::vector<int> chan;
        fdc::DevBuf<float2> d_cbt;
        fdc::DevBuf<float> d_shn;
        fdc::DevBuf<long long> d_slot_off;
        fdc::DevBuf<float2> d_tab;
    };
    std::vector<Bank> banks;
    bool poly_ok = false;
    bool poly_block = false;
    std::vector<std::pair<int, int>> bank_alias;
    fdc::DevBuf<float2> d_tw512, d_twq512;
    fdc::DevBuf<float2> d_tw1k, d_twq1k;
    fdc::DevBuf<float2> d_t2g;
    bool split = false;
    std::vector<int> rem;
    std::vector<std::pair<int, std::vector<int32_t>>> rgroups;
    std::vector<size_t> rgroup_off;
    std::vector<char> rg_aligned, rg_out_aligned;
    fdc::DevBuf<int32_t> d_rgroups;
    int block_hints = 1;
    int block_min = kBlockMinBlocks;
    fdc::DevBuf<float2> d_g;
    int ncu = 0;
    int reserved_cu = 0;
    fdc::DevBuf<float2> d_twq;
    bool fwd_block = false;
    bool fused = false;
    std::vector<int> f4_wave[8];
    unsigned f4_cls = 0;
    int f4_teams = 2;
    fdc::DevBuf<fdc::F4Row> d_f4rows;
    fdc::DevBuf<float2> d_ftwq, d_fcbt;
    fdc::DevBuf<float> d_fshn;
    fdc::DevBuf<long long> d_fslot;
    fdc::DevBuf<float2> d_fscr;
    fdc::DevBuf<fdc::ChanDev> d_chans;
    fdc::DevBuf<int32_t> d_groups;
    unsigned long long keep4096 = ~0ull;
    fdc::DevBuf<unsigned> d_keep;
    fdc::DevBuf<float2> d_big;
    fdc::DevBuf<fdc::ExtractTask> d_wtasks;
    size_t big_pts = 0;
    int big_l = 0;
    fdc::DevBuf<float2> d_tmp;
    fdc::DevBuf<float2> d_spec;
    fdc::DevBuf<float2> d_ring;
    fdc::DevBuf<float2> d_specfull;
    fdc::DevBuf<float> d_real;
    int in_form = -1;
    float in_scale = 0.f;
    fdc::DevBuf<unsigned char> d_iq;
    fdc::DevBuf<float2> d_iqw;
    std::string iq_route;
    int out_form = 0;
    float out_scale = 1.f;
    fdc::DevBuf<unsigned char> d_oq;
    std::string oq_route;
    bool fine_on = false;
    fdc::DevBuf<fdc::FineChan> d_fine, d_f4fine;
    fdc::DevBuf<float2> d_fstep;
    std::string fine_route;
    fdc::DevBuf<float2> d_out;
    int64_t blockcount = 0;
    hipStream_t s_in = nullptr, s_out = nullptr;
    hipEvent_t ev_in[2] = {nullptr, nullptr}, ev_k[2] = {nullptr, nullptr}, ev_out[2] = {nullptr, nullptr};
    fdc::PinBuf<float2> pin_out[2];
    fdc::MappedBuf<fdc::ScatterEnt> pin_tab;
    fdc::ScatterEnt *d_tab = nullptr;
    int sub = 0;
    int hier_filled = 0;
    fdc_sinks *hier_bank = nullptr;
    hipEvent_t ev_hier = nullptr;
    bool hier_ring_busy = false;
    bool hier_broken = false;
    bool reserve_user = false;
    std::string wf_route;
    bool cfg_generic = false;
    bool timing = false;
    int timing_stride = 1;
    long long timing_seq = 0;
    std::vector<hipEvent_t> events;
    size_t ev_used = 0;
    std::vector<std::array<size_t, 5>> ev_spans;
};

namespace fdc { namespace pipe {

struct Span { int nb, m0, nblocks; int64_t first_block; };

struct DeviceCall {
    int fmt = 0; float scale = 1.0f; float2 *wide = nullptr;
    int ofmt = 0; float oscale = 1.0f; float2 *fout = nullptr; bool narrow = true;
    hipStream_t stream = nullptr;
    void *spectrum = nullptr;
    bool own_spectrum = false;
    float *gpow = nullptr; const float2 *gpow_origin = nullptr;
    float *rows = nullptr; int64_t rows_first = 0;
    int ncu = 0;
    bool all_fused = true, ofused = false;
};

enum { kSpanBanks = 0 , kSpanTwoLaunch = 1 ,
       kSpanSpectrumLds = 2 , kSpanSpectrum = 3  };

inline bool ispow2(int v) { return v > 0 && (v & (v - 1)) == 0; }

inline float2 unit(double turns)
{
    const double a = -2.0 * M_PI * turns;
    return make_float2(float(std::cos(a)), float(std::sin(a)));
}

inline bool two_launch_possible(const fdc_pipeline *p)
{
    return p->poly_ok && p->banks.size() == 1 && p->banks[0].r == 0 && p->bank_alias.empty();
}

std::vector<float2> make_twiddles(int n);
bool host_registered(const void *ptr, size_t bytes, void **devptr = nullptr);
int out_staging(fdc_pipeline *p);

int validate_cfg(const fdc_pipeline_cfg *cfg);
int effective_flags(int flags);
void build_channel_records(fdc_pipeline *p, const fdc_pipeline_cfg *cfg, std::vector<std::complex<float>> &pool);
void group_by_width(const fdc_pipeline *p, const std::vector<int> *ids, std::vector<std::pair<int, std::vector<int32_t>>> &groups,
                    std::vector<size_t> &off, std::vector<char> &al, std::vector<char> &oal, std::vector<int32_t> &flat);
void classify_plan(fdc_pipeline *p, const fdc_pipeline_cfg *cfg, int flags);
int build_device_state(fdc_pipeline *p, const fdc_pipeline_cfg *cfg, const std::vector<std::complex<float>> &pool,
                       const std::vector<int32_t> &flat, const std::vector<int32_t> &rflat);

DeviceCall device_call(const fdc_pipeline *p, void *stream, void *d_spectrum, int fmt = 0, float scale = 1.0f);
int process_device_impl(fdc_pipeline *p, DeviceCall &call, const void *d_ring, int64_t first_block, int nblocks, void *d_out);
int channels_wide(fdc_pipeline *p, const float2 *spec, float2 *d_out, const int32_t *d_gids, int ngroup, int l, const Span &span, hipStream_t s);
int check_iq_form(int32_t format, float scale);
std::string route(int fmt, bool fused, const char *otherwise);

} }
```

gr-fdc_amd/csrc/fdc_plan.hip:

```cpp
#include "fdc_pipeline.hpp"

#include <map>
#include <tuple>

namespace fdc { namespace pipe {

int validate_cfg(const fdc_pipeline_cfg *cfg)
{
    const int N = cfg->blocklen, R = cfg->relinvovl;
    if (!ispow2(N) || N < 2) return set_error(FDC_ERR_INVALID_ARGUMENT, "blocklen %d must be a power of two >= 2", N);
    if (!ispow2(R) || R < 2 || R > N) return set_error(FDC_ERR_INVALID_ARGUMENT, "relinvovl %d must be a power of two in [2, blocklen]", R);
    if (N > (1 << 24)) return set_error(FDC_ERR_UNSUPPORTED, "blocklen %d above 2^24", N);
    if (cfg->nchannels < 0 || (cfg->nchannels > 0 && !cfg->channels)) return set_error(FDC_ERR_INVALID_ARGUMENT, "bad channel list");
    if (cfg->max_blocks < 1) return set_error(FDC_ERR_INVALID_ARGUMENT, "max_blocks must be >= 1");
    for (int c = 0; c < cfg->nchannels; c++) {
        const fdc_channel &ch = cfg->channels[c];
        if (!ispow2(ch.l) || ch.l > N) return set_error(FDC_ERR_INVALID_ARGUMENT, "channel %d: l=%d must be a power of two <= blocklen", c, ch.l);
        if (ch.f < 0 || ch.f + ch.l > N) return set_error(FDC_ERR_INVALID_ARGUMENT, "channel %d: slice [%d,%d) outside the spectrum", c, ch.f, ch.f + ch.l);
        if (ch.passbw <= 0.0f) return set_error(FDC_ERR_INVALID_ARGUMENT, "channel %d: PassBw must not be <= 0", c);
        if (ch.stopbw <= 0.0f) return set_error(FDC_ERR_INVALID_ARGUMENT, "channel %d: StopBw must not be <= 0", c);
        if (ch.stopbw < ch.passbw) return set_error(FDC_ERR_INVALID_ARGUMENT, "channel %d: StopBw must not be < PassBw", c);
    }
    int64_t per_block = 0;
    for (int c = 0; c < cfg->nchannels; c++) per_block += cfg->channels[c].l - cfg->channels[c].l / R;
    if (per_block * 8 * (int64_t)cfg->max_blocks > 0xFFFFF000ll)
        return set_error(FDC_ERR_INVALID_ARGUMENT, "max_blocks %d x %lld output samples per block is more than the 4 GiB one call may produce (at most %lld blocks per call for this plan)",
                    cfg->max_blocks, (long long)per_block, (long long)(0xFFFFF000ll / (per_block * 8)));
    return FDC_OK;
}

void group_by_width(const fdc_pipeline *p, const std::vector<int> *ids, std::vector<std::pair<int, std::vector<int32_t>>> &groups,
                    std::vector<size_t> &off, std::vector<char> &al, std::vector<char> &oal, std::vector<int32_t> &flat)
{
    std::map<int, std::vector<int32_t>> bylen;
    if (ids) for (int c : *ids) bylen[p->chans[(size_t)c].l].push_back(c);
    else for (int c = 0; c < p->C; c++) bylen[p->chans[(size_t)c].l].push_back(c);
    for (auto &kv : bylen) {
        bool a = true, o = true;
        for (int c : kv.second) {
            if (p->chans[(size_t)c].f & 1) a = false;
            if ((p->chans[(size_t)c].out_off & 1) || (p->chans[(size_t)c].lout & 1)) o = false;
        }
        al.push_back(a); oal.push_back(o);
        off.push_back(flat.size());
        groups.emplace_back(kv.first, kv.second);
        flat.insert(flat.end(), kv.second.begin(), kv.second.end());
    }
}

void build_channel_records(fdc_pipeline *p, const fdc_pipeline_cfg *cfg, std::vector<std::complex<float>> &pool)
{
    std::map<std::tuple<int, float, float>, int> winmap;
    int64_t off = 0;
    for (int c = 0; c < p->C; c++) {
        const fdc_channel &ch = cfg->channels[c];
        fdc::ChanDev d{};
        d.f = ch.f; d.l = ch.l; d.lout = ch.l - ch.l / p->R;
        d.shift = ((ch.f % p->R) + p->R) % p->R;
        d.out_off = off; off += d.lout;
        auto key = std::make_tuple(ch.l, ch.passbw, ch.stopbw);
        auto it = winmap.find(key);
        if (it == winmap.end()) {
            const int o = (int)pool.size();
            pool.resize(pool.size() + (size_t)p->R * ch.l);
            fdc::window_table(cfg->windowtype, ch.l, ch.passbw, ch.stopbw, p->R, 1, false, pool.data() + o);
            it = winmap.emplace(key, o).first;
        }
        d.win_off = it->second;
        p->chans.push_back(d);
    }
    p->sum_lout = off;
}

static bool bank_has_block_kernel(int N, int R, int L, int r, int flags)
{
    if ((flags & FDC_PIPE_NO_BLOCK) || (R != 2 && R != 4)) return false;
    switch (L) {
    case 256: return fdc::poly_block_supports(N);
    case 512: return fdc::poly_block512_supports(N, R) && (r == 0 || r == L / 2);
    case 1024: return fdc::poly_block1024_supports(N, R) && (r == 0 || r == L / 2);
    case 128: case 64: return fdc::poly_block_narrow_supports(N, L, R) && r % (L / 4) == 0;
    default: return false;
    }
}

struct F4Class { int l, cls, per_wave, pitch; };
constexpr F4Class kF4Classes[] = {{1024, 4, 2, 1056}, {512, 3, 4, 513}, {128, 5, 8, 136}, {64, 6, 8, 68}, {32, 7, 8, 34}, {16, 8, 8, 17}};
static bool plan_fused4096(fdc_pipeline *p, const fdc_pipeline_cfg *cfg, int flags)
{
    for (auto &w : p->f4_wave) w.clear();
    p->f4_cls = 0;
    p->f4_teams = 2;
    if (p->N != 4096 || p->C == 0 || p->cfg_generic || (flags & (FDC_PIPE_NO_POLY | FDC_PIPE_NO_FUSED))) return false;
    long long bins = 0;
    bool wide = false;
    for (int c = 0; c < p->C; c++) {
        const int l = cfg->channels[c].l;
        if (l < 16 || l > 1024 || (l & (l - 1)) || l % p->R) return false;
        bins += l;
        wide = wide || l >= 512;
    }
    if (bins < 512 && !(flags & FDC_PIPE_WIDE_UNIFORM)) return false;
    auto schedule = [&](int T) {
        for (auto &w : p->f4_wave) w.clear();
        std::map<int, std::vector<int>> by;
        for (int c = 0; c < p->C; c++) for (int k = 0; k < T; k++) by[cfg->channels[c].l].push_back(2 * c + k);
        int w = 0;
        unsigned cls = 0;
        long long pts = 272ll * (long long)by[256].size();
        for (const F4Class &k : kF4Classes) {
            const std::vector<int> &rows = by[k.l];
            pts += (long long)k.pitch * (long long)rows.size();
            for (size_t i = 0; i < rows.size(); i += (size_t)k.per_wave, w++) {
                if (w >= 4 * T) return false;
                for (size_t j = i; j < std::min(i + (size_t)k.per_wave, rows.size()); j++) p->f4_wave[w].push_back(rows[j]);
                cls |= (unsigned)k.cls << (4 * w);
            }
        }
        const int avail = 4 * T - w, n256 = (int)by[256].size();
        if (n256 > 8 * avail || pts > (long long)T * fdc::fused4096_tile_points()) return false;
        if (n256) {
            const int nw = n256 <= 4 * avail ? (n256 + 3) / 4 : avail;
            for (int i = 0; i < n256; i++) p->f4_wave[w + i % nw].push_back(by[256][(size_t)i]);
            for (int k = 0; k < nw; k++) cls |= (p->f4_wave[w + k].size() > 4 ? 2u : 1u) << (4 * (w + k));
        }
        p->f4_cls = cls;
        p->f4_teams = T;
        return true;
    };
    static const int teams_env = [] { const char *e = fdc::debug_env("FDC_F4_TEAMS"); return e ? atoi(e) : 0; }();
    if ((!wide || teams_env == 1) && teams_env != 2 && schedule(1)) return true;
    if (schedule(2)) return true;
    for (auto &w : p->f4_wave) w.clear();
    p->f4_cls = 0;
    return false;
}

void classify_plan(fdc_pipeline *p, const fdc_pipeline_cfg *cfg, int flags)
{
    const int N = p->N, R = p->R, C = p->C;
    p->fwd_block = fdc::poly_block_supports(N) && !p->cfg_generic && !(flags & FDC_PIPE_NO_BLOCK);
    p->banks.clear(); p->bank_alias.clear(); p->rem.clear();
    p->poly_ok = p->poly_block = p->split = false;
    p->fused = plan_fused4096(p, cfg, flags);
    if (p->fused) return;
    if (C == 0 || p->cfg_generic || (flags & FDC_PIPE_NO_POLY) || N > (1 << 20) || R > 16) return;
    auto same_window = [&](const fdc_pipeline::Bank &b, const fdc_channel &ch) { return b.passbw == ch.passbw && b.stopbw == ch.stopbw; };

    std::vector<fdc_pipeline::Bank> banks;
    std::vector<std::vector<char>> used;
    std::vector<std::pair<int, int>> alias;
    std::vector<int> rem;
    for (int c = 0; c < C; c++) {
        const fdc_channel &ch = cfg->channels[c];
        const int L = ch.l, r = ch.f % L;
        if (!bank_has_block_kernel(N, R, L, r, flags)) { rem.push_back(c); continue; }
        size_t k = 0;
        for (; k < banks.size(); k++) if (banks[k].L == L && banks[k].r == r && same_window(banks[k], ch)) break;
        if (k == banks.size()) {
            fdc_pipeline::Bank b;
            b.L = L; b.r = r; b.passbw = ch.passbw; b.stopbw = ch.stopbw;
            banks.push_back(std::move(b));
            used.emplace_back((size_t)(N / L) + 1, 0);
        }
        if (used[k][(size_t)(ch.f / L)]) {
            int first = -1;
            for (int c0 : banks[k].chan) if (cfg->channels[c0].f == ch.f) { first = c0; break; }
            alias.emplace_back(c, first);
            continue;
        }
        used[k][(size_t)(ch.f / L)] = 1;
        banks[k].chan.push_back(c);
    }

    if (banks.empty()) {
        const int L = cfg->channels[0].l;
        const bool fits = L == 256 ? N >= 4096
                                   : (L >= 64 && L <= 4096 && L / R >= 1 && N / L >= 16 && N / L <= 4096 && (L == 128 || (flags & FDC_PIPE_WIDE_UNIFORM)));
        if (!fits) return;
        fdc_pipeline::Bank b;
        b.L = L; b.r = 0; b.passbw = cfg->channels[0].passbw; b.stopbw = cfg->channels[0].stopbw;
        std::vector<char> u((size_t)(N / L) + 1, 0);
        for (int c = 0; c < C; c++) {
            const fdc_channel &ch = cfg->channels[c];
            if (ch.l != L || ch.f % L || !same_window(b, ch) || u[(size_t)(ch.f / L)]) return;
            u[(size_t)(ch.f / L)] = 1;
            b.chan.push_back(c);
        }
        p->banks.push_back(std::move(b));
        p->poly_ok = true;
        return;
    }

    const bool may_split = p->fwd_block;
    auto band = [&](const std::vector<int> &ids) { double b = 0; for (int c : ids) b += cfg->channels[c].l; return b / double(N); };
    auto move_to_rem = [&](size_t k) {
        rem.insert(rem.end(), banks[k].chan.begin(), banks[k].chan.end());
        for (size_t i = 0; i < alias.size();) {
            if (std::find(banks[k].chan.begin(), banks[k].chan.end(), alias[i].second) != banks[k].chan.end()) {
                rem.push_back(alias[i].first);
                alias.erase(alias.begin() + (long)i);
            } else i++;
        }
        banks.erase(banks.begin() + (long)k);
    };
    if (!may_split) {
        if (!rem.empty() || (int)banks.size() > fdc::cost::kMaxBanks) return;
    } else {
        auto total = [&](const std::vector<fdc_pipeline::Bank> &bs, double remband) {
            double t = fdc::cost::spectrum_path(remband);
            for (const auto &b : bs) t += fdc::cost::bank_launch(b.L);
            return t;
        };
        const bool forced = (flags & FDC_PIPE_WIDE_UNIFORM) != 0;
        for (;;) {
            if (banks.empty()) break;
            const bool too_many = (int)banks.size() > fdc::cost::kMaxBanks;
            if (forced && !too_many) break;
            const double now = total(banks, band(rem));
            size_t best = banks.size();
            double best_t = too_many ? 1e30 : now;
            for (size_t k = 0; k < banks.size(); k++) {
                std::vector<int> r2(rem);
                r2.insert(r2.end(), banks[k].chan.begin(), banks[k].chan.end());
                for (const auto &al : alias) if (std::find(banks[k].chan.begin(), banks[k].chan.end(), al.second) != banks[k].chan.end()) r2.push_back(al.first);
                double t = fdc::cost::spectrum_path(band(r2));
                for (size_t j = 0; j < banks.size(); j++) if (j != k) t += fdc::cost::bank_launch(banks[j].L);
                if (t < best_t) { best_t = t; best = k; }
            }
            if (best == banks.size()) break;
            move_to_rem(best);
        }
        if (banks.empty()) return;
        if (!forced) {
            std::vector<int> all(C);
            for (int c = 0; c < C; c++) all[(size_t)c] = c;
            if (total(banks, band(rem)) >= fdc::cost::spectrum_path(band(all))) return;
        }
    }
    std::stable_sort(banks.begin(), banks.end(), [](const fdc_pipeline::Bank &x, const fdc_pipeline::Bank &y) { return x.chan.size() > y.chan.size(); });
    std::sort(rem.begin(), rem.end());
    p->banks = std::move(banks);
    p->bank_alias = std::move(alias);
    p->rem = std::move(rem);
    p->split = !p->rem.empty();
    p->poly_ok = p->poly_block = true;
}

static int build_bank_tables(fdc_pipeline *p, const fdc_pipeline_cfg *cfg, fdc_pipeline::Bank &bk)
{
    const int N = p->N, L = bk.L, N1 = N / L, rb = bk.r;
    std::vector<std::complex<float>> shape((size_t)L);
    fdc::window_table(cfg->windowtype, L, bk.passbw, bk.stopbw, 1, 0, true, shape.data());
    std::vector<float> sn((size_t)L);
    for (int k2 = 0; k2 < L; k2++) sn[(size_t)k2] = float(double(shape[(size_t)k2].real()) / double(N));
    std::vector<long long> so((size_t)N1, -1);
    for (int c : bk.chan) so[(size_t)(p->chans[(size_t)c].f / L)] = p->chans[(size_t)c].out_off;
    CHK_DEV(bk.d_slot_off.upload(so));
    std::vector<float2> cb;
    if (L == 256) {
        cb.resize((size_t)N1 * 16);
        for (int n1 = 0; n1 < N1; n1++)
            for (int j = 0; j < 16; j++) {
                const float2 w = unit(double(((long long)n1 * (j + rb)) % N) / double(N));
                const float sg = (n1 & 1) ? -1.0f : 1.0f;
                cb[(size_t)n1 * 16 + j] = make_float2(sg * w.x, sg * w.y);
            }
    } else if ((L == 512 || L == 1024) && p->poly_block) {
        const bool half = rb == L / 2;
        const int parts = L / 256;
        if (half) {
            std::vector<float> snd(sn);
            for (int k2 = 0; k2 < L; k2++) sn[(size_t)k2] = snd[(size_t)(k2 ^ (L / 2))];
        }
        cb.resize((size_t)N1 * 16 * parts);
        for (int n1 = 0; n1 < N1; n1++)
            for (int e = 0; e < 16 * parts; e++) {
                const int i = half ? (e >> 4) ^ (parts / 2) : e >> 4;
                const float2 w = unit(double(((long long)n1 * ((e & 15) + 256 * i + (half ? L / 2 : 0))) % N) / double(N));
                const float sg = (n1 & 1) ? -1.0f : 1.0f;
                cb[(size_t)n1 * 16 * parts + e] = make_float2(sg * w.x, sg * w.y);
            }
    } else if (p->poly_block) {
        const bool half = rb == L / 2;
        const int S = 256 / L;
        std::vector<float2> img((size_t)fdc::poly_block_narrow_table_points(L, N));
        fdc::poly_block_narrow_tables(L, N, sn.data(), img.data(), half, half ? 0 : rb);
        CHK_DEV(bk.d_tab.upload(img));
        const int NV = N / 256;
        cb.resize((size_t)NV * 16);
        for (int V = 0; V < NV; V++)
            for (int b = 0; b < 16; b++) cb[(size_t)V * 16 + b] = unit(double(((long long)S * V * (b + rb)) % N) / double(N));
    }
    CHK_DEV(bk.d_shn.upload(sn));
    if (!cb.empty()) CHK_DEV(bk.d_cbt.upload(cb));
    return FDC_OK;
}

static int build_shared_bank_tables(fdc_pipeline *p)
{
    const int N = p->N;
    auto has = [&](int L) { for (const auto &b : p->banks) if (b.L == L) return true; return false; };
    auto twq_table = [&](int N1) {
        std::vector<float2> tq((size_t)N1 * 16);
        for (int n1 = 0; n1 < N1; n1++)
            for (int q = 0; q < 16; q++) tq[(size_t)n1 * 16 + q] = unit(double((16ll * n1 * q) % N) / double(N));
        return tq;
    };
    if (has(256)) {
        CHK_DEV(p->d_twq.upload(twq_table(N / 256)));
        if (N / 256 == 1024) CHK_DEV(p->d_tw1024.upload(make_twiddles(1024)));
    }
    if (has(512) && p->poly_block) {
        std::vector<float2> t5(256);
        for (int k = 0; k < 256; k++) t5[(size_t)k] = unit(double(k) / 512.0);
        CHK_DEV(p->d_tw512.upload(t5));
        CHK_DEV(p->d_twq512.upload(twq_table(N / 512)));
    }
    if (has(1024) && p->poly_block) {
        CHK_DEV(p->d_tw1k.upload(make_twiddles(1024)));
        CHK_DEV(p->d_twq1k.upload(twq_table(N / 1024)));
    }
    if (p->banks.size() == 1 && p->banks[0].L != 256 && p->banks[0].r == 0 && p->bank_alias.empty()) {
        const int L = p->banks[0].L, TCg = fdc::poly_stage1_generic_tile_columns(N, L);
        std::vector<float2> t2v((size_t)L * TCg);
        for (int k2 = 0; k2 < L; k2++)
            for (int t = 0; t < TCg; t++) t2v[(size_t)k2 * TCg + t] = unit(double(((long long)t * k2) % N) / double(N));
        CHK_DEV(p->d_t2g.upload(t2v));
    }
    return FDC_OK;
}

static int build_forward_tables(fdc_pipeline *p)
{
    const int N = p->N, N1 = N / 256;
    std::vector<float2> tq((size_t)N1 * 16), cb((size_t)N1 * 16);
    for (int n1 = 0; n1 < N1; n1++)
        for (int j = 0; j < 16; j++) {
            tq[(size_t)n1 * 16 + j] = unit(double((16ll * n1 * j) % N) / double(N));
            const float2 w = unit(double(((long long)n1 * j) % N) / double(N));
            const float sg = (n1 & 1) ? -1.0f : 1.0f;
            cb[(size_t)n1 * 16 + j] = make_float2(sg * w.x, sg * w.y);
        }
    std::vector<float> sn(256, float(1.0 / double(N)));
    std::vector<long long> so((size_t)N1);
    for (int c = 0; c < N1; c++) so[(size_t)c] = 256ll * c;
    CHK_DEV(p->d_ftwq.upload(tq));
    CHK_DEV(p->d_fcbt.upload(cb));
    CHK_DEV(p->d_fshn.upload(sn));
    CHK_DEV(p->d_fslot.upload(so));
    return FDC_OK;
}

static int build_keep_map(fdc_pipeline *p)
{
    const int N = p->N;
    std::vector<char> g64((size_t)N / 64, 0);
    bool all = true;
    for (int c = 0; c < p->C; c++) {
        if (p->split && !std::binary_search(p->rem.begin(), p->rem.end(), c)) continue;
        const auto &ch = p->chans[(size_t)c];
        for (int b = ch.f / 64; b <= (ch.f + ch.l - 1) / 64 && b < N / 64; b++) g64[(size_t)b] = 1;
    }
    for (char v : g64) all = all && v;
    if (all) return FDC_OK;
    if (N == 4096) {
        p->keep4096 = 0;
        for (int b = 0; b < 64; b++) if (g64[(size_t)b]) p->keep4096 |= 1ull << b;
        return FDC_OK;
    }
    const int P = N / 8192;
    std::vector<unsigned> kw((size_t)P * 4, 0u);
    for (int klo = 0; klo < P; klo++)
        for (int q = 0; q < 4; q++)
            for (int r = 0; r < 32; r++) {
                const int k0 = r >> 4, k1 = 4 * (r & 3) + ((r & 15) >> 2), c = klo + P * (k0 + 2 * k1);
                if (g64[(size_t)(4 * c + q)]) kw[(size_t)(klo * 4 + q)] |= 1u << r;
            }
    CHK_DEV(p->d_keep.upload(kw));
    return FDC_OK;
}


int build_device_state(fdc_pipeline *p, const fdc_pipeline_cfg *cfg, const std::vector<std::complex<float>> &pool,
                       const std::vector<int32_t> &flat, const std::vector<int32_t> &rflat)
{
    const int N = p->N, R = p->R, flags = p->cfg.flags, chunk = p->chunk;
    CHK_DEV(hipStreamCreateWithFlags(&p->stream, hipStreamNonBlocking));
    p->ntab = N;
    CHK_DEV(p->d_tw.upload(make_twiddles(N)));
    if (p->C > 0) {
        CHK_DEV(p->d_wins.alloc(pool.size()));
        CHK_DEV(hipMemcpy(p->d_wins, pool.data(), sizeof(float2) * pool.size(), hipMemcpyHostToDevice));
        CHK_DEV(p->d_chans.upload(p->chans));
        CHK_DEV(p->d_groups.upload(flat));
        if (!rflat.empty()) CHK_DEV(p->d_rgroups.upload(rflat));
    }
    CHK_DEV(p->d_tw256.upload(make_twiddles(256)));
    if (N > fdc::kMaxLdsFft) {
        const fdc::BigGeom bg = fdc::big_geom(N);
        std::vector<float2> tf((size_t)N);
        for (int k2 = 0; k2 < bg.N2; k2++)
            for (int n1 = 0; n1 < bg.N1; n1++) tf[(size_t)k2 * bg.N1 + n1] = unit(double((long long)n1 * k2) / double(N));
        CHK_DEV(p->d_twf.upload(tf));
    }
    for (auto &bk : p->banks) { const int rc = build_bank_tables(p, cfg, bk); if (rc != FDC_OK) return rc; }
    if (p->fused) {
        std::vector<fdc::F4Row> rows(64);
        int xch = 0;
        for (int w = 0; w < 4 * p->f4_teams; w++) {
            const unsigned cls = (p->f4_cls >> (4 * w)) & 0xfu;
            const int L = cls == 4 ? 1024 : cls == 3 ? 512 : cls >= 5 ? 16 << (8 - (int)cls) : 256, pitch = cls == 4 ? 1056 : cls == 3 ? 513 : cls >= 5 ? L + L / 16 : 272;
            for (int k = 0; k < 8; k++) {
                fdc::F4Row &r = rows[(size_t)(8 * w + k)];
                r = fdc::F4Row{0, 0, 0, 0, L - L / R, 0, 0};
                if (k >= (int)p->f4_wave[w].size()) continue;
                const int code = p->f4_wave[w][(size_t)k];
                const fdc::ChanDev &ch = p->chans[(size_t)(code >> 1)];
                r = fdc::F4Row{ch.f, ch.win_off, ch.shift, xch, ch.lout, 1 + (code & 1), (long long)ch.out_off};
                xch += pitch;
            }
        }
        CHK_DEV(p->d_f4rows.upload(rows));
    }
    { const int rc = build_shared_bank_tables(p); if (rc != FDC_OK) return rc; }
    p->fwd_block = fdc::poly_block_supports(N) && !p->cfg_generic && !(flags & FDC_PIPE_NO_BLOCK);
    if (p->fwd_block) { const int rc = build_forward_tables(p); if (rc != FDC_OK) return rc; }
    {
        hipDeviceProp_t prop;
        CHK_DEV(hipGetDeviceProperties(&prop, cfg->device_id));
        p->ncu = prop.multiProcessorCount > 0 ? prop.multiProcessorCount : 256;
    }
    if (p->fwd_block || (p->poly_block && R == 4)) CHK_DEV(p->d_fscr.alloc(32768 * (size_t)p->ncu));
    if (p->C > 0 && !(flags & FDC_PIPE_FULL_SPECTRUM) && (N == 4096 || p->fwd_block)) {
        const int rc = build_keep_map(p);
        if (rc != FDC_OK) return rc;
    }
    if (two_launch_possible(p)) {
        const int L = p->banks[0].L, gblocks = p->poly_block ? std::min(chunk, p->block_min) : chunk;
        CHK_DEV(p->d_g.alloc((size_t)gblocks * (size_t)(L - L / R) * (size_t)(N / L)));
    }
    {
        size_t widest = 0;
        for (const auto &gr : p->groups) if (gr.first > 4096) { widest = std::max(widest, gr.second.size() * (size_t)gr.first); p->big_l = std::max(p->big_l, gr.first); }
        if (widest) {
            p->big_pts = std::max<size_t>(widest, std::min<size_t>((size_t)32 << 20, widest * (size_t)chunk));
            CHK_DEV(p->d_big.alloc(p->big_pts));
            CHK_DEV(p->d_wtasks.alloc(p->big_pts / 8192 + (size_t)p->C + 1));
        }
    }
    if (N > fdc::kMaxLdsFft) CHK_DEV(p->d_tmp.alloc((size_t)(p->fwd_block ? std::min(chunk, p->block_min) : chunk) * N));
    CHK_DEV(p->d_spec.alloc((size_t)chunk * N));
    return FDC_OK;
}

int effective_flags(int flags)
{
    auto on = [](const char *n) { const char *v = fdc::debug_env(n); return v && v[0] == '1'; };
    if (on("FDC_FORCE_GENERIC")) flags |= FDC_PIPE_FORCE_GENERIC;
    if (on("FDC_NO_POLY")) flags |= FDC_PIPE_NO_POLY;
    if (on("FDC_NO_BLOCK")) flags |= FDC_PIPE_NO_BLOCK;
    if (on("FDC_NO_FUSED")) flags |= FDC_PIPE_NO_FUSED;
    if (const char *bh = fdc::debug_env("FDC_BLOCK_HINTS")) {
        flags &= ~(FDC_PIPE_PLAIN_STORES | FDC_PIPE_NT_LOADS);
        if (!(atoi(bh) & 1)) flags |= FDC_PIPE_PLAIN_STORES;
        if (atoi(bh) & 2) flags |= FDC_PIPE_NT_LOADS;
    }
    return flags;
}

} }
```

include/fdc_amd.h:

```cpp
#ifndef FDC_AMD_H
#define FDC_AMD_H

#include <stddef.h>
#include <stdint.h>

#ifdef __cplusplus
extern "C" {
#endif

typedef enum {
    FDC_OK = 0,
    FDC_ERR_INVALID_ARGUMENT = -1,
    FDC_ERR_HIP = -2,
    FDC_ERR_NO_DEVICE = -3,
    FDC_ERR_UNSUPPORTED = -4,
    FDC_ERR_NOMEM = -5
} fdc_status;

enum { FDC_WIN_RECTANGULAR = 0, FDC_WIN_HANN = 1, FDC_WIN_RAMP = 2 };

const char *fdc_last_error(void);
int fdc_selftest_exception_barrier(void);
const char *fdc_version(void);
int fdc_device_count(void);
int fdc_selftest_devices(void);

typedef struct fdc_pipeline fdc_pipeline;

typedef struct {
    int32_t f;
    int32_t l;
    float passbw;
    float stopbw;
} fdc_channel;

typedef struct {
    int32_t device_id;
    int32_t blocklen;
    int32_t relinvovl;
    int32_t windowtype;
    int32_t nchannels;
    const fdc_channel *channels;
    int32_t max_blocks;
    int32_t chunk_blocks;
    int32_t keep_spectrum;
    int32_t flags;
    int32_t min_block_launch;
    int32_t host_sub_blocks;
} fdc_pipeline_cfg;
enum {
    FDC_PIPE_FORCE_GENERIC = 1,
    FDC_PIPE_NO_POLY = 2,
    FDC_PIPE_NO_BLOCK = 4,
    FDC_PIPE_PLAIN_STORES = 8,
    FDC_PIPE_NT_LOADS = 16,
    FDC_PIPE_FULL_SPECTRUM = 32,
    FDC_PIPE_NO_FUSED = 128,
    FDC_PIPE_WIDE_UNIFORM = 64
};

int fdc_pipeline_create(const fdc_pipeline_cfg *cfg, fdc_pipeline **out);
void fdc_pipeline_destroy(fdc_pipeline *p);

int64_t fdc_pipeline_input_samples(const fdc_pipeline *p, int nblocks);
int64_t fdc_pipeline_output_samples(const fdc_pipeline *p, int nblocks);
int64_t fdc_pipeline_channel_offset(const fdc_pipeline *p, int channel, int nblocks);
int32_t fdc_pipeline_channel_lout(const fdc_pipeline *p, int channel);

int fdc_pipeline_work(fdc_pipeline *p, const void *in, int nblocks, void *const *outs, void *spectrum);
int fdc_pipeline_work_real(fdc_pipeline *p, const void *in, int nblocks, void *const *outs, void *spectrum);

int fdc_pipeline_work_span(fdc_pipeline *p, const void *halo, const void *in, int64_t first_block, int nblocks, void *const *outs,
                           void *spectrum);
int fdc_pipeline_work_span_real(fdc_pipeline *p, const void *halo, const void *in, int64_t first_block, int nblocks, void *const *outs,
                                void *spectrum);

enum { FDC_IQ_SC16 = 1,
       FDC_IQ_SC8  = 2 };
int fdc_pipeline_work_iq(fdc_pipeline *p, int32_t format, float scale, const void *in, int nblocks, void *const *outs, void *spectrum);
int fdc_pipeline_work_span_iq(fdc_pipeline *p, int32_t format, float scale, const void *halo, const void *in, int64_t first_block, int nblocks,
                              void *const *outs, void *spectrum);

enum { FDC_OQ_FC32 = 0,
       FDC_OQ_SC16 = 1,
       FDC_OQ_SC8  = 2 };
int fdc_pipeline_set_output_format(fdc_pipeline *p, int32_t format, float scale);

int fdc_fine_tuning_increment(double nu, uint64_t *inc);
int fdc_pipeline_set_fine_tuning(fdc_pipeline *p, const double *nu, int n);

int fdc_host_register(void *ptr, size_t bytes);
int fdc_host_unregister(void *ptr);
void fdc_pipeline_reset(fdc_pipeline *p);

int fdc_pipeline_process_device(fdc_pipeline *p, const void *d_ring, int64_t first_block, int nblocks,
                                void *d_out, void *d_spectrum, void *stream);
int fdc_pipeline_process_device_iq(fdc_pipeline *p, int32_t format, float scale, const void *d_ring, int64_t first_block, int nblocks,
                                   void *d_out, void *d_spectrum, void *stream);
int fdc_pipeline_process_device_power(fdc_pipeline *p, const void *d_ring, int64_t first_block, int nblocks, void *d_out, void *d_spectrum,
                                      void *d_group_power, void *stream);
int fdc_pipeline_synchronize(fdc_pipeline *p);
void *fdc_pipeline_stream(fdc_pipeline *p);
int fdc_pipeline_reserve_compute_units(fdc_pipeline *p, int32_t n);
int32_t fdc_pipeline_chunk_blocks(const fdc_pipeline *p);
int32_t fdc_pipeline_path(const fdc_pipeline *p);
int32_t fdc_pipeline_describe(const fdc_pipeline *p, char *buf, int32_t n);
int fdc_pipeline_plan_preview(const fdc_pipeline_cfg *cfg, char *buf, int32_t n, int32_t *assignment);

int fdc_pipeline_enable_timing(fdc_pipeline *p, int enable);
int fdc_pipeline_last_kernel_ms(fdc_pipeline *p, float *ms, int n);

typedef struct fdc_pipeline_group fdc_pipeline_group;
int fdc_pipeline_group_create(const fdc_pipeline_cfg *cfg, const int32_t *devices, int ndevices, int min_span_blocks,
                              fdc_pipeline_group **out);
void fdc_pipeline_group_destroy(fdc_pipeline_group *g);
int fdc_pipeline_group_work(fdc_pipeline_group *g, const void *in, int nblocks, void *const *outs, void *spectrum);
int fdc_pipeline_group_work_real(fdc_pipeline_group *g, const void *in, int nblocks, void *const *outs, void *spectrum);
int fdc_pipeline_group_work_iq(fdc_pipeline_group *g, int32_t format, float scale, const void *in, int nblocks, void *const *outs, void *spectrum);
void fdc_pipeline_group_reset(fdc_pipeline_group *g);
int fdc_pipeline_group_set_output_format(fdc_pipeline_group *g, int32_t format, float scale);
int fdc_pipeline_group_set_fine_tuning(fdc_pipeline_group *g, const double *nu, int n);
int32_t fdc_pipeline_group_size(const fdc_pipeline_group *g);
fdc_pipeline *fdc_pipeline_group_member(fdc_pipeline_group *g, int i);
int32_t fdc_pipeline_group_device(const fdc_pipeline_group *g, int i);
int32_t fdc_pipeline_group_member_max_blocks(const fdc_pipeline_group *g);
int fdc_device_numa_node(int device_id);
int fdc_selftest_worker_placement(int node, int32_t *cpus_of_node, int32_t *cpus_of_worker);
int fdc_pipeline_group_last_spans(const fdc_pipeline_group *g, int64_t *first_block, int32_t *nblocks, int cap);

typedef struct fdc_sinks fdc_sinks;
typedef struct { float cfreq, bw; int32_t id; } fdc_pac_cfg;
typedef struct { float start, stop; } fdc_segment_cfg;
typedef struct {
    int32_t device_id, blocklen, relinvovl;
    int32_t npac; const fdc_pac_cfg *pac;
    float pac_thresh_db; int32_t pac_maxblocks, pac_deactivation_delay;
    int32_t nseg; const fdc_segment_cfg *seg;
    float det_thresh_db; int32_t det_maxblocks; float minchandist; int32_t det_deactivation_delay;
    double window_flank_puffer;
    int32_t max_blocks;
    int32_t det_variant;
    int32_t verbose;
    int32_t det_id;
    int32_t flags;
    int32_t threads;
    int32_t seg_id_base;
} fdc_sinks_cfg;
enum {
    FDC_SINKS_HOST_DECISIONS = 1,
    FDC_SINKS_DEVICE_PAYLOAD = 2,
    FDC_SINKS_LOOKAHEAD = 4
};
typedef struct {
    int32_t kind;
    int32_t source;
    int32_t chan_id;
    int32_t finalized, part, has_part;
    double rel_bw, rel_cfreq;
    int64_t blockstart, blockend, vectorstart, vectorend;
    int64_t nsamples;
    const void *samples;
    char id[72];
} fdc_pdu;

typedef void (*fdc_log_fn)(const char *line, void *user);
void fdc_set_log_callback(fdc_log_fn fn, void *user);

int fdc_pipeline_work_spectrum(fdc_pipeline *p, const void *in, int nblocks, void *const *outs, void *spectrum,
                               fdc_sinks *sinks);
int fdc_sinks_create(const fdc_sinks_cfg *cfg, fdc_sinks **out);
int fdc_pipeline_work_sinks(fdc_pipeline *p, const void *in, int nblocks, void *const *outs, void *spectrum,
                            fdc_sinks *sinks);
int fdc_pipeline_flush_sinks(fdc_pipeline *p, fdc_sinks *sinks);
int32_t fdc_pipeline_sinks_latency(const fdc_pipeline *p, const fdc_sinks *sinks);
void fdc_sinks_destroy(fdc_sinks *s);
int fdc_sinks_work(fdc_sinks *s, const void *spectrum, int nitems);
int fdc_sinks_work_band(fdc_sinks *s, const void *spectrum, int nitems, int32_t bin_lo, int32_t bin_hi);
int fdc_sinks_read_band(const fdc_sinks *s, int32_t *lo, int32_t *hi);
void *fdc_sinks_spectrum(fdc_sinks *s);
void *fdc_sinks_stream(fdc_sinks *s);
int32_t fdc_sinks_blocklen(const fdc_sinks *s);
int32_t fdc_sinks_max_blocks(const fdc_sinks *s);
int fdc_sinks_work_device(fdc_sinks *s, int nblocks);
int fdc_sinks_submit_device(fdc_sinks *s, int nblocks);
int fdc_sinks_flush(fdc_sinks *s);
int32_t fdc_sinks_engine(const fdc_sinks *s);
int fdc_sinks_set_payload_format(fdc_sinks *s, int32_t format, float scale);
int fdc_sinks_payload_format(const fdc_sinks *s, int32_t *format, float *scale);
int32_t fdc_sinks_payload_route(const fdc_sinks *s);
void *fdc_sinks_spectrum_ahead(fdc_sinks *s);
void *fdc_sinks_fill_stream(fdc_sinks *s);
int fdc_sinks_prepare(fdc_sinks *s, int nblocks, int ahead);
void *fdc_sinks_group_power(fdc_sinks *s);
void *fdc_sinks_group_power_ahead(fdc_sinks *s);
int fdc_sinks_prepare_from_groups(fdc_sinks *s, int nblocks, int ahead);
int fdc_sinks_pdu_count(const fdc_sinks *s);
int fdc_sinks_pdu(const fdc_sinks *s, int i, fdc_pdu *out);
int fdc_sinks_pdus(const fdc_sinks *s, fdc_pdu *out, int cap);
int fdc_sinks_pdu_emit_items(const fdc_sinks *s, int32_t *item, int cap);
int fdc_sinks_pdu_emit_order(const fdc_sinks *s, int32_t *item, int32_t *pac, int cap);
int fdc_sinks_pac_params(const fdc_sinks *s, int i, int32_t *v8);
int fdc_sinks_segment_params(const fdc_sinks *s, int i, int32_t *v5);

typedef struct fdc_sinks_group fdc_sinks_group;
int fdc_sinks_group_create(const fdc_sinks_cfg *cfg, const int32_t *devices, int ndevices, fdc_sinks_group **out);
void fdc_sinks_group_destroy(fdc_sinks_group *g);
int fdc_sinks_group_work(fdc_sinks_group *g, const void *spectrum, int nitems);
int fdc_sinks_group_pdu_count(const fdc_sinks_group *g);
int fdc_sinks_group_pdus(const fdc_sinks_group *g, fdc_pdu *out, int cap);
int32_t fdc_sinks_group_size(const fdc_sinks_group *g);
fdc_sinks *fdc_sinks_group_member(fdc_sinks_group *g, int i);
int fdc_sinks_group_member_info(const fdc_sinks_group *g, int i, int32_t *device, int32_t *lo, int32_t *hi, int32_t *npac, int32_t *nseg);
int fdc_sinks_group_set_payload_format(fdc_sinks_group *g, int32_t format, float scale);

typedef struct fdc_overlap_save fdc_overlap_save;
int fdc_overlap_save_create(int device_id, int itemsize, int outputlen, int overlaplen, fdc_overlap_save **out);
int fdc_overlap_save_work(fdc_overlap_save *b, const void *in, int nitems, void *out);
void fdc_overlap_save_destroy(fdc_overlap_save *b);

typedef struct fdc_vector_cut fdc_vector_cut;
int fdc_vector_cut_create(int device_id, int itemsize, int veclen, int offset, int blocklen, fdc_vector_cut **out);
int fdc_vector_cut_work(fdc_vector_cut *b, const void *in, int nitems, void *out);
void fdc_vector_cut_destroy(fdc_vector_cut *b);

typedef struct fdc_phase_window fdc_phase_window;
int fdc_phase_window_create(int device_id, int blocklen, int numphasestates, int shifts, float passbw,
                            float stopbw, int windowtype, fdc_phase_window **out);
int fdc_phase_window_work(fdc_phase_window *b, const void *in, int nitems, void *out);
void fdc_phase_window_destroy(fdc_phase_window *b);

int fdc_window_table(int windowtype, int blocklen, float passbw, float stopbw, int numphasestates,
                     int step, int normalize, float *w);

int fdc_fft_vcc(int device_id, int n, int forward, int shift, const void *in, int nitems, void *out);

typedef struct fdc_waterfall fdc_waterfall;
typedef struct {
    int32_t blocklen;
    int32_t blockdecimation;
    int32_t loginput;
    double minvaldb, maxvaldb;
    int32_t colorscheme;
} fdc_waterfall_cfg;
int fdc_waterfall_check(const fdc_waterfall_cfg *cfg, fdc_waterfall_cfg *normalized);
int fdc_waterfall_create(int device_id, const fdc_waterfall_cfg *cfg, int32_t max_items, fdc_waterfall **out);
void fdc_waterfall_destroy(fdc_waterfall *w);
void fdc_waterfall_reset(fdc_waterfall *w);
int fdc_waterfall_set_levels(fdc_waterfall *w, double minvaldb, double maxvaldb);
int fdc_waterfall_set_colorscheme(fdc_waterfall *w, int32_t scheme);
int64_t fdc_waterfall_rows_done(const fdc_waterfall *w);
int fdc_waterfall_color_table(int32_t scheme, uint8_t *rgb, uint8_t *frame);
int fdc_waterfall_edges(int32_t loginput, double minvaldb, double maxvaldb, double *edges);
int fdc_waterfall_work(fdc_waterfall *w, const float *power, int nitems, float *rows, uint16_t *index, uint8_t *rgb, int cap_rows,
                       int32_t *nrows);
int fdc_pipeline_work_waterfall(fdc_pipeline *p, fdc_waterfall *w, const void *in, int nblocks, void *const *outs, float *rows,
                                uint16_t *index, uint8_t *rgb, int cap_rows, int32_t *nrows);

#ifdef __cplusplus
}
#endif
#endif
```

Baseline: 200,200.

## Use 16-byte global stores in block channelizer via permlane32 swap and padded LDS layout

Adds a W16 variant of the 256-point block channelizer kernel. It reorders trip rows in LDS with padding so that lane pairs hold adjacent output samples, exchanges halves with permlane32_swap, and issues 16-byte stores instead of 8-byte ones. The variant is selected by default when the output is 16-byte aligned and slot offsets are even, and a new STORES_8B flag keeps the old path available. The aim is to halve the store instruction count and widen the write transactions, at the cost of extra cross-lane permutes, a changed LDS layout with possible bank conflicts, and more kernel instantiations.

```diff
diff --git a/gr-fdc_amd/__init__.py b/gr-fdc_amd/__init__.py
--- a/gr-fdc_amd/__init__.py
+++ b/gr-fdc_amd/__init__.py
@@ -3,7 +3,7 @@
 from .channelizer import (FrequencyDomainChannelizer, Pipeline, PipelineGroup, IQ_SC16, IQ_SC8, OQ_FC32, plan_preview, FREQMODE, VERBOSEMODE, WINDOWTYPES,
                           nextpow2, get_opt_channelparams, freq_converters, register_host, unregister_host, defaults, fine_tuning_increment, fine_tuning_nu)
 from ._lib import (FDC_PIPE_FORCE_GENERIC, FDC_PIPE_NO_POLY, FDC_PIPE_NO_BLOCK, FDC_PIPE_PLAIN_STORES, FDC_PIPE_NT_LOADS,
-                   FDC_PIPE_FULL_SPECTRUM, FDC_PIPE_WIDE_UNIFORM, FDC_PIPE_NO_FUSED,
+                   FDC_PIPE_FULL_SPECTRUM, FDC_PIPE_WIDE_UNIFORM, FDC_PIPE_NO_FUSED, FDC_PIPE_STORES_8B,
                    FDC_SINKS_HOST_DECISIONS, FDC_SINKS_DEVICE_PAYLOAD, FDC_SINKS_LOOKAHEAD)
 from .waterfall import Waterfall, WaterfallImage, Rows as WaterfallRows
 from .sharding import span_for_rank, ring_bounds, ring_for_span
diff --git a/gr-fdc_amd/_lib.py b/gr-fdc_amd/_lib.py
--- a/gr-fdc_amd/_lib.py
+++ b/gr-fdc_amd/_lib.py
@@ -30,6 +30,7 @@
 FDC_PIPE_FULL_SPECTRUM = 32
 FDC_PIPE_WIDE_UNIFORM = 64
 FDC_PIPE_NO_FUSED = 128
+FDC_PIPE_STORES_8B = 256
 
 
 class fdc_pac_cfg(C.Structure):
diff --git a/gr-fdc_amd/channelizer.py b/gr-fdc_amd/channelizer.py
--- a/gr-fdc_amd/channelizer.py
+++ b/gr-fdc_amd/channelizer.py
@@ -91,7 +91,7 @@
         flags |= _lib.FDC_PIPE_NO_FUSED
     if "FDC_BLOCK_HINTS" in defaults:
         h = int(defaults["FDC_BLOCK_HINTS"])
-        flags |= (0 if h & 1 else _lib.FDC_PIPE_PLAIN_STORES) | (_lib.FDC_PIPE_NT_LOADS if h & 2 else 0)
+        flags |= (0 if h & 1 else _lib.FDC_PIPE_PLAIN_STORES) | (_lib.FDC_PIPE_NT_LOADS if h & 2 else 0) | (_lib.FDC_PIPE_STORES_8B if h & 4 else 0)
     return flags, int(defaults.get("FDC_BLOCK_MIN_BLOCKS", 0) or 0), int(defaults.get("FDC_HOST_SUB", 0) or 0)
 
 
diff --git a/gr-fdc_amd/csrc/fdc_api.hip b/gr-fdc_amd/csrc/fdc_api.hip
--- a/gr-fdc_amd/csrc/fdc_api.hip
+++ b/gr-fdc_amd/csrc/fdc_api.hip
@@ -267,7 +267,7 @@
     const int flags = effective_flags(cfg->flags);
     p->cfg.flags = flags;
     p->cfg_generic = (flags & FDC_PIPE_FORCE_GENERIC) != 0;
-    p->block_hints = ((flags & FDC_PIPE_PLAIN_STORES) ? 0 : 1) | ((flags & FDC_PIPE_NT_LOADS) ? 2 : 0);
+    p->block_hints = ((flags & FDC_PIPE_PLAIN_STORES) ? 0 : 1) | ((flags & FDC_PIPE_NT_LOADS) ? 2 : 0) | ((flags & FDC_PIPE_STORES_8B) ? 4 : 0);
     if (cfg->min_block_launch >= 1) p->block_min = cfg->min_block_launch;
     if (const char *bm = fdc::debug_env("FDC_BLOCK_MIN_BLOCKS")) if (atoi(bm) >= 1) p->block_min = atoi(bm);
 
diff --git a/gr-fdc_amd/csrc/fdc_block256.hip b/gr-fdc_amd/csrc/fdc_block256.hip
--- a/gr-fdc_amd/csrc/fdc_block256.hip
+++ b/gr-fdc_amd/csrc/fdc_block256.hip
@@ -7,7 +7,7 @@
 
 typedef unsigned long long u8v __attribute__((ext_vector_type(8)));
 
-template <int P>
+template <int P, bool W16 = false>
 struct BlkGeom {
     static_assert(P == 2 || P == 4 || P == 8, "passes of 32 columns: N = 16384, 32768 or 65536");
     static constexpr int kN1 = 32 * P;
@@ -15,7 +15,10 @@
     static constexpr int kJT = P == 8 ? 4 : 8;
     static constexpr int kJB = P == 8 ? 2 : P == 4 ? 4 : 8;
     static constexpr int kLd = P == 2 ? 32 * P + 2 : 32 * P + 6;
-    static constexpr int kTripBytes = 16 * kJT * kLd * 8;
+    static constexpr int kPad = !W16 ? 0 : P == 2 ? 8 : 12;
+    static constexpr int kJBW = P == 4 ? 4 : kJT;
+    static constexpr int row_off(int jj) { return (8 * (jj & 3) + 64 * (jj >> 2)) * kLd + 2 * (jj >> 2) * kPad; }
+    static constexpr int kTripBytes = (16 * kJT * kLd + (16 * kJT / 32 - 1) * kPad) * 8;
     static constexpr int kOffCt = kTripBytes > kStripsEnd ? kTripBytes : kStripsEnd;
     static constexpr int kOffWrow = P == 8 ? 136960 : kOffCt + 32 * P * 8;
     static constexpr int kOffB = kOffWrow + 16 * 18 * 8;
@@ -28,10 +31,14 @@
     static_assert(kLdsOff <= 160 * 1024 && kLds <= 160 * 1024, "LDS budget");
     static_assert(kOffCt >= kStripsEnd && kOffCt + 32 * P * 8 <= kOffWrow, "stage-2 trip buffer and twiddles below the tables, tables above the strips");
     static_assert((16 * (kJB - 1) * kLd + 32 * (P - 1)) * 8 < 65536, "ds offsets of a base register");
+    static_assert((row_off(kJBW - 1) + 32 * (P - 1)) * 8 < 65536 && (row_off(kJT - 1) - row_off(kJBW % kJT) + 32 * (P - 1)) * 8 < 65536,
+                  "ds offsets of a base register, 16-byte-store layout");
+    static_assert((kPad * 8) % 16 == 0 && (kLd * 8) % 16 == 0, "16-byte reads of a trip row");
+    static_assert(((63 * kLd + kPad) * 8 + 32 * P * 8) <= kTripBytes, "the last row of the first 64 positions ends inside the trip");
 };
 
 
-template <int P, bool NT, bool OFF, bool FWD, bool R4 = false, bool HALF = false, class TI = float2, class TO = float2>
+template <int P, bool NT, bool OFF, bool FWD, bool R4 = false, bool HALF = false, class TI = float2, class TO = float2, bool W16 = false>
 __global__ FDC_PLAIN_DS __launch_bounds__(512, (P == 2 && !OFF && !R4 && !FWD) ? 4 : 2) void k_blk256(const TI *__restrict__ in, size_t in_stride, TO *__restrict__ out,
                                                 const float2 *__restrict__ tw256, const float2 *__restrict__ twq,
                                                 const float2 *__restrict__ cbt, const float *__restrict__ shn,
@@ -41,7 +48,7 @@
                                                 float2 *__restrict__ fwd_scratch, const unsigned *__restrict__ keep,
                                                 typename IqTail<TI, TO>::type gpow )
 {
-    typedef BlkGeom<P> GM;
+    typedef BlkGeom<P, W16> GM;
     constexpr bool kIq = !std::is_same<TI, float2>::value, kOq = !std::is_same<TO, float2>::value;
     static_assert(!kIq || !FWD, "integer input: the channelizer forms (the forward transform takes widened input)");
     static_assert(!kOq || !FWD, "integer output: the channelizer forms");
@@ -50,7 +57,8 @@
     [[maybe_unused]] const float iq_scale = iq_tail_scale(gpow);
     [[maybe_unused]] const float oq_scale = oq_tail_scale(gpow);
     static_assert(!HALF || (!OFF && !FWD), "the half-slot form is a variant of the on-grid channelizer");
-    constexpr int kN1 = GM::kN1, kLd = GM::kLd, kJT = GM::kJT, kJB = GM::kJB;
+    static_assert(!W16 || (!FWD && !kOq), "16-byte stores: the channelizer forms with float2 output");
+    constexpr int kN1 = GM::kN1, kLd = GM::kLd, kJT = GM::kJT, kJB = W16 ? GM::kJBW : GM::kJB;
     float2 *scr = reinterpret_cast<float2 *>(fdc_smem_blk);
     float2 *wrow = reinterpret_cast<float2 *>(fdc_smem_blk + GM::kOffWrow);
     float2 *Bt = reinterpret_cast<float2 *>(fdc_smem_blk + GM::kOffB);
@@ -99,7 +107,9 @@
     }
     for (int i = tid; i < kN1; i += 512) {
         const long long o = slot_off[i];
-        soff[(i % P) * 32 + ((i / P) & 1) * 16 + rev16((i / P) >> 1)] = o >= 0 ? (unsigned)((o * nb_call + out_base) * kOs) : 0xFFFFFFFFu;
+        const int reg = ((i / P) & 1) * 16 + rev16((i / P) >> 1);
+        if constexpr (W16) soff[(i % P) * 32 + (reg & 1) * 16 + (reg >> 1)] = o >= 0 ? (unsigned)((o * nb_call + out_base) * kOs) : 0xFFFFFFFFu;
+        else soff[(i % P) * 32 + ((i / P) & 1) * 16 + rev16((i / P) >> 1)] = o >= 0 ? (unsigned)((o * nb_call + out_base) * kOs) : 0xFFFFFFFFu;
     }
     for (int i = tid; i < 32 * P; i += 512) ctab[i] = tw256[((i / P) * (i % P) * (8 / P)) & 255];
     Bt[(tid >> 4) * 18 + (tid & 15)] = twq[HALF ? tid ^ 8 : tid];
@@ -244,12 +254,15 @@
             asm volatile("" : "+v"(t2));
             const int lane2 = t2 & 63, w2 = __builtin_amdgcn_readfirstlane(t2 >> 6), b_2 = lane2 >> 2, c5_2 = 4 * w2 + (lane2 & 3);
             const int klo2 = w2 % P, rh2 = w2 / P;
-            float2 *const gw0 = scr + b_2 * kLd + c5_2;
-            int rowjb = 16 * kJB * kLd;
-            asm volatile("" : "+v"(rowjb));
-            float2 *const gw1 = gw0 + rowjb;
-            const float2 *const gr = scr + (64 * rh2 + lane2) * kLd + 32 * klo2;
-            const uint4 *const sow = reinterpret_cast<const uint4 *>(soff + 32 * klo2);
+            float2 *const gw0 = W16 ? scr + ((b_2 >> 1) + 32 * (b_2 & 1)) * kLd + (b_2 & 1) * GM::kPad + c5_2 : scr + b_2 * kLd + c5_2;
+            float2 *gw1 = gw0;
+            if constexpr (!W16 || kJB < kJT) {
+                int rowjb = W16 ? GM::row_off(kJB) : 16 * kJB * kLd;
+                asm volatile("" : "+v"(rowjb));
+                gw1 = gw0 + rowjb;
+            }
+            const float2 *const gr = scr + (64 * rh2 + lane2) * kLd + (W16 ? (2 * rh2 + (lane2 >> 5)) * GM::kPad : 0) + 32 * klo2;
+            const uint4 *const sow = reinterpret_cast<const uint4 *>(soff + 32 * klo2 + (W16 ? 16 * (lane2 >> 5) : 0));
 #pragma unroll
             for (int tr = 0; tr < kNTrip; tr++) {
                 const int ja = kNJ - kJT * tr < kJT ? kNJ - kJT * tr : kJT;
@@ -274,7 +287,7 @@
 #pragma unroll
                     for (int ps = 0; ps < P; ps++) a[ps] = src[jj][ps];
                     pass_dft<P>(a);
-                    float2 *const gw = (jj < kJB ? gw0 : gw1) + (jj % kJB) * 16 * kLd;
+                    float2 *const gw = (jj < kJB ? gw0 : gw1) + (W16 ? GM::row_off(jj) - (jj < kJB ? 0 : GM::row_off(kJB % kJT)) : (jj % kJB) * 16 * kLd);
                     st2(&gw[0], a[0]);
 #pragma unroll
                     for (int k = 1; k < P; k++) st2(&gw[32 * k], cmul(a[pass_idx<P>(k)], ct[k]));
@@ -294,10 +307,25 @@
                 __builtin_amdgcn_sched_barrier(0);
                 if (reads) {
                     dft32<false>(v);
-                    const int trow0 = 16 * kJT * tr + 64 * rh2, trow = trow0 + lane2;
+                    const int trow0 = 16 * kJT * tr + 64 * rh2, trow = trow0 + (W16 ? 2 * (lane2 & 31) : lane2);
                     const unsigned rb = (unsigned)(m * (FWD ? GM::kN : (R4 ? 192 : 128)) + rowbase + trow) * kOs;
                     unsigned mq = FWD ? mqs[((rowbase + trow0) >> 6) & 3] : ~0u;
                     if constexpr (FWD) asm volatile("" : "+s"(mq));
+                    if constexpr (W16) {
+#pragma unroll
+                        for (int q = 0; q < 4; q++) {
+                            const uint4 t = sow[q];
+                            const unsigned so[4] = {t.x, t.y, t.z, t.w};
+#pragma unroll
+                            for (int e = 0; e < 4; e++) {
+                                const cf ev = v[8 * q + 2 * e], od = v[8 * q + 2 * e + 1];
+                                const auto sx = __builtin_amdgcn_permlane32_swap(__float_as_uint(ev.x), __float_as_uint(od.x), false, false);
+                                const auto sy = __builtin_amdgcn_permlane32_swap(__float_as_uint(ev.y), __float_as_uint(od.y), false, false);
+                                bst4<NT>(rout, (so[e] == 0xFFFFFFFFu ? 0xFFFFFFE0u : so[e] + rb), mk(__uint_as_float(sx[0]), __uint_as_float(sy[0])),
+                                         mk(__uint_as_float(sx[1]), __uint_as_float(sy[1])));
+                            }
+                        }
+                    } else {
 #pragma unroll
                     for (int q = 0; q < 8; q++) {
                         const uint4 t = sow[q];
@@ -312,6 +340,7 @@
                             } else
                                 bst2t<NT>(rout, (o == 0xFFFFFFFFu ? 0xFFFFFFF0u : o + rb), v[4 * q + e]);
                         }
+                    }
                     }
                     if constexpr (FWD) {
                         if (gpow) {
@@ -375,13 +404,16 @@
 static hipError_t init_block_kernels_in()
 {
     hipError_t e;
-#define FDC_SETB(P, A, B, R4) \
-    e = hipFuncSetAttribute(reinterpret_cast<const void *>(k_blk256<P, A, B, false, R4, false, TI>), hipFuncAttributeMaxDynamicSharedMemorySize, \
-                            B ? BlkGeom<P>::kLdsOff : BlkGeom<P>::kLds); \
+#define FDC_SETBW(P, A, B, R4, W) \
+    e = hipFuncSetAttribute(reinterpret_cast<const void *>(k_blk256<P, A, B, false, R4, false, TI, float2, W>), hipFuncAttributeMaxDynamicSharedMemorySize, \
+                            B ? BlkGeom<P, W>::kLdsOff : BlkGeom<P, W>::kLds); \
     if (e != hipSuccess) return e;
-#define FDC_SETH(P, A, R4) \
-    e = hipFuncSetAttribute(reinterpret_cast<const void *>(k_blk256<P, A, false, false, R4, true, TI>), hipFuncAttributeMaxDynamicSharedMemorySize, BlkGeom<P>::kLds); \
+#define FDC_SETHW(P, A, R4, W) \
+    e = hipFuncSetAttribute(reinterpret_cast<const void *>(k_blk256<P, A, false, false, R4, true, TI, float2, W>), hipFuncAttributeMaxDynamicSharedMemorySize, \
+                            BlkGeom<P, W>::kLds); \
     if (e != hipSuccess) return e;
+#define FDC_SETB(P, A, B, R4) FDC_SETBW(P, A, B, R4, false) FDC_SETBW(P, A, B, R4, true)
+#define FDC_SETH(P, A, R4) FDC_SETHW(P, A, R4, false) FDC_SETHW(P, A, R4, true)
 #define FDC_SETP(P) \
     FDC_SETB(P, true, false, false) FDC_SETB(P, false, false, false) FDC_SETB(P, true, true, false) FDC_SETB(P, false, true, false) \
     FDC_SETB(P, true, false, true) FDC_SETB(P, false, false, true) FDC_SETB(P, true, true, true) FDC_SETB(P, false, true, true) \
@@ -390,6 +422,8 @@
 #undef FDC_SETP
 #undef FDC_SETH
 #undef FDC_SETB
+#undef FDC_SETHW
+#undef FDC_SETBW
     return hipSuccess;
 }
 
@@ -421,8 +455,9 @@
 
 hipError_t init_block_kernels()
 {
-    hipError_t e = init_block_kernels_in<sc16>();
+    hipError_t e = init_block_kernels_in<float2>();
     if (e != hipSuccess) return e;
+    if ((e = init_block_kernels_in<sc16>()) != hipSuccess) return e;
     if ((e = init_block_kernels_in<sc8>()) != hipSuccess) return e;
     if ((e = init_block_kernels_oq<float2, sc16>()) != hipSuccess) return e;
     if ((e = init_block_kernels_oq<float2, sc8>()) != hipSuccess) return e;
@@ -430,26 +465,11 @@
     if ((e = init_block_kernels_oq<sc16, sc8>()) != hipSuccess) return e;
     if ((e = init_block_kernels_oq<sc8, sc16>()) != hipSuccess) return e;
     if ((e = init_block_kernels_oq<sc8, sc8>()) != hipSuccess) return e;
-#define FDC_SETB(P, A, B, F, R4) \
-    e = hipFuncSetAttribute(reinterpret_cast<const void *>(k_blk256<P, A, B, F, R4>), hipFuncAttributeMaxDynamicSharedMemorySize, \
-                            B ? BlkGeom<P>::kLdsOff : BlkGeom<P>::kLds); \
+#define FDC_SETF(P, A) \
+    e = hipFuncSetAttribute(reinterpret_cast<const void *>(k_blk256<P, A, false, true, false>), hipFuncAttributeMaxDynamicSharedMemorySize, BlkGeom<P>::kLds); \
     if (e != hipSuccess) return e;
-#define FDC_SETP(P) \
-    FDC_SETB(P, true, false, false, false) FDC_SETB(P, false, false, false, false) FDC_SETB(P, true, true, false, false) \
-    FDC_SETB(P, false, true, false, false) FDC_SETB(P, true, false, false, true) FDC_SETB(P, false, false, false, true) \
-    FDC_SETB(P, true, true, false, true) FDC_SETB(P, false, true, false, true)
-    FDC_SETP(2) FDC_SETP(4) FDC_SETP(8)
-    FDC_SETB(8, true, false, true, false) FDC_SETB(8, false, false, true, false) FDC_SETB(4, true, false, true, false) FDC_SETB(4, false, false, true, false)
-    FDC_SETB(2, true, false, true, false) FDC_SETB(2, false, false, true, false)
-#undef FDC_SETP
-#undef FDC_SETB
-#define FDC_SETH(P, A, R4) \
-    e = hipFuncSetAttribute(reinterpret_cast<const void *>(k_blk256<P, A, false, false, R4, true>), hipFuncAttributeMaxDynamicSharedMemorySize, BlkGeom<P>::kLds); \
-    if (e != hipSuccess) return e;
-#define FDC_SETHP(P) FDC_SETH(P, true, false) FDC_SETH(P, false, false) FDC_SETH(P, true, true) FDC_SETH(P, false, true)
-    FDC_SETHP(2) FDC_SETHP(4) FDC_SETHP(8)
-#undef FDC_SETHP
-#undef FDC_SETH
+    FDC_SETF(8, true) FDC_SETF(8, false) FDC_SETF(4, true) FDC_SETF(4, false) FDC_SETF(2, true) FDC_SETF(2, false)
+#undef FDC_SETF
     return hipSuccess;
 }
 
@@ -469,14 +489,17 @@
         else if constexpr (kIq) return (void)so, si;
         else return (void)si, so;
     };
+    const bool w16 = !kOq && !(b.hints & 4) && reinterpret_cast<uintptr_t>(out) % 16 == 0 && (b.even_slots || !(b.nb_call & 1));
     const bool halfslot = b.half();
     if (!poly_block_supports(b.N) || (b.R != 2 && !r4) || (r4 && !b.scratch)) return hipErrorInvalidValue;
     const int grid = b.grid(b.N == 16384 && b.R == 2 && (!b.r || halfslot) ? 2 : 1);
-#define FDC_L(P, A, O, R4, H, roff) \
-    hipExtLaunchKernelGGL((k_blk256<P, A || kOq, O, false, R4, H, TI, TO>), dim3((unsigned)grid), dim3(512), O ? BlkGeom<P>::kLdsOff : BlkGeom<P>::kLds, b.s, \
+#define FDC_LW(P, A, O, R4, H, roff, W) \
+    hipExtLaunchKernelGGL((k_blk256<P, A || kOq, O, false, R4, H, TI, TO, W>), dim3((unsigned)grid), dim3(512), O ? BlkGeom<P, W>::kLdsOff : BlkGeom<P, W>::kLds, b.s, \
                           b.ev_start, b.ev_stop, 0u, in, b.in_stride, out, b.tw256, b.twq, b.cbt, b.shn, b.slot_off, (long long)b.mbase * (R4 ? 192 : 128), \
                           (long long)b.nb_call, b.out_bytes, b.nb_chunk, b.hints, (unsigned long long *)nullptr, roff, b.first_block, \
                           R4 ? b.scratch : (float2 *)nullptr, (const unsigned *)nullptr, iq_tail(iq_scale, oq_scale))
+#define FDC_L(P, A, O, R4, H, roff) \
+    do { if constexpr (!kOq) { if (w16) { FDC_LW(P, A, O, R4, H, roff, true); break; } } FDC_LW(P, A, O, R4, H, roff, false); } while (0)
 #define FDC_LB(P, A, O, R4) FDC_L(P, A, O, R4, false, b.r)
 #define FDC_LH(P, A, R4) FDC_L(P, A, false, R4, true, 0)
 #define FDC_R4(P) if constexpr (P != 8 || !kOqR4Narrowed<TI, TO>::value)
@@ -496,6 +519,7 @@
 #undef FDC_LH
 #undef FDC_LB
 #undef FDC_L
+#undef FDC_LW
     return hipGetLastError();
 }
 
diff --git a/gr-fdc_amd/csrc/fdc_enqueue.hip b/gr-fdc_amd/csrc/fdc_enqueue.hip
--- a/gr-fdc_amd/csrc/fdc_enqueue.hip
+++ b/gr-fdc_amd/csrc/fdc_enqueue.hip
@@ -83,7 +83,7 @@
 static int launch_bank(fdc_pipeline *p, const DeviceCall &call, const fdc_pipeline::Bank &bk, fdc::BlockLaunch b, const void *raw, void *oq)
 {
     b.in_stride = (size_t)p->H;
-    b.slot_off = bk.d_slot_off;
+    b.slot_off = bk.d_slot_off; b.even_slots = bk.even_off;
     b.ncu = call.ncu; b.hints = p->block_hints;
     b.s = call.stream;
     b.N = p->N; b.R = p->R; b.scratch = p->d_fscr;
diff --git a/gr-fdc_amd/csrc/fdc_kernels.h b/gr-fdc_amd/csrc/fdc_kernels.h
--- a/gr-fdc_amd/csrc/fdc_kernels.h
+++ b/gr-fdc_amd/csrc/fdc_kernels.h
@@ -107,6 +107,7 @@
     float2 *out;
     int nb_chunk, mbase, nb_call;
     const long long *slot_off;
+    bool even_slots;
     unsigned out_bytes;
     int ncu;
     int hints;
diff --git a/gr-fdc_amd/csrc/fdc_pipeline.hpp b/gr-fdc_amd/csrc/fdc_pipeline.hpp
--- a/gr-fdc_amd/csrc/fdc_pipeline.hpp
+++ b/gr-fdc_amd/csrc/fdc_pipeline.hpp
@@ -69,6 +69,7 @@
         fdc::DevBuf<float2> d_cbt;
         fdc::DevBuf<float> d_shn;
         fdc::DevBuf<long long> d_slot_off;
+        bool even_off = false;
         fdc::DevBuf<float2> d_tab;
     };
     std::vector<Bank> banks;
diff --git a/gr-fdc_amd/csrc/fdc_plan.hip b/gr-fdc_amd/csrc/fdc_plan.hip
--- a/gr-fdc_amd/csrc/fdc_plan.hip
+++ b/gr-fdc_amd/csrc/fdc_plan.hip
@@ -257,6 +257,8 @@
     std::vector<long long> so((size_t)N1, -1);
     for (int c : bk.chan) so[(size_t)(p->chans[(size_t)c].f / L)] = p->chans[(size_t)c].out_off;
     CHK_DEV(bk.d_slot_off.upload(so));
+    bk.even_off = true;
+    for (long long o : so) if (o > 0 && (o & 1)) bk.even_off = false;
     std::vector<float2> cb;
     if (L == 256) {
         cb.resize((size_t)N1 * 16);
@@ -462,9 +464,10 @@
     if (on("FDC_NO_BLOCK")) flags |= FDC_PIPE_NO_BLOCK;
     if (on("FDC_NO_FUSED")) flags |= FDC_PIPE_NO_FUSED;
     if (const char *bh = fdc::debug_env("FDC_BLOCK_HINTS")) {
-        flags &= ~(FDC_PIPE_PLAIN_STORES | FDC_PIPE_NT_LOADS);
+        flags &= ~(FDC_PIPE_PLAIN_STORES | FDC_PIPE_NT_LOADS | FDC_PIPE_STORES_8B);
         if (!(atoi(bh) & 1)) flags |= FDC_PIPE_PLAIN_STORES;
         if (atoi(bh) & 2) flags |= FDC_PIPE_NT_LOADS;
+        if (atoi(bh) & 4) flags |= FDC_PIPE_STORES_8B;
     }
     return flags;
 }
diff --git a/include/fdc_amd.h b/include/fdc_amd.h
--- a/include/fdc_amd.h
+++ b/include/fdc_amd.h
@@ -56,6 +56,7 @@
     FDC_PIPE_NT_LOADS = 16,
     FDC_PIPE_FULL_SPECTRUM = 32,
     FDC_PIPE_NO_FUSED = 128,
+    FDC_PIPE_STORES_8B = 256,
     FDC_PIPE_WIDE_UNIFORM = 64
 };
 
diff --git a/profiles/r07/lds_layout.py b/profiles/r07/lds_layout.py
--- /dev/null
+++ b/profiles/r07/lds_layout.py
@@ -0,0 +1,70 @@
+#!/usr/bin/env python3
+
+READ_GROUPS = [[0, 1, 2, 3, 12, 13, 14, 15, 20, 21, 22, 23, 24, 25, 26, 27], [4, 5, 6, 7, 8, 9, 10, 11, 16, 17, 18, 19, 28, 29, 30, 31]]
+READ_GROUPS += [[l + 32 for l in g] for g in READ_GROUPS]
+
+
+def worst(groups, addr, width, banks):
+    w = 1
+    for g in groups:
+        per_bank = {}
+        for lane in g:
+            for d in range(width):
+                a = addr(lane) + d
+                per_bank.setdefault(a % banks, set()).add(a)
+        w = max(w, max(len(s) for s in per_bank.values()))
+    return w
+
+
+def geom(P, wide):
+    kld = 32 * P + (2 if P == 2 else 6)
+    pad = 0 if not wide else (8 if P == 2 else 12)
+    return kld, pad
+
+
+def writer(P, wide, wave, jj, k):
+    kld, pad = geom(P, wide)
+
+    def addr(lane):
+        b, c5 = lane >> 2, 4 * wave + (lane & 3)
+        if wide:
+            pos = (b >> 1) + 32 * (b & 1) + 8 * (jj & 3) + 64 * (jj >> 2)
+        else:
+            pos = b + 16 * jj
+        return 2 * (pos * kld + (pos >> 5) * pad + c5 + 32 * k)
+    return addr
+
+
+def reader(P, wide, klo, rh, i):
+    kld, pad = geom(P, wide)
+
+    def addr(lane):
+        pos = 64 * rh + lane
+        return 2 * (pos * kld + (pos >> 5) * pad + 32 * klo + 2 * i)
+    return addr
+
+
+def rows_of_positions(P):
+    jt = 4 if P == 8 else 8
+    pos_of = {}
+    for jj in range(jt):
+        for b in range(16):
+            pos_of[b + 16 * jj] = (b >> 1) + 32 * (b & 1) + 8 * (jj & 3) + 64 * (jj >> 2)
+    assert sorted(pos_of.values()) == list(range(16 * jt))
+    for r, p in pos_of.items():
+        rh, lane = p >> 6, p & 63
+        assert r == 64 * rh + 2 * (lane & 31) + (lane >> 5)
+
+
+if __name__ == "__main__":
+    wgroups = [list(range(16 * g, 16 * g + 16)) for g in range(4)]
+    for P in (2, 4, 8):
+        rows_of_positions(P)
+        jt = 4 if P == 8 else 8
+        for wide in (False, True):
+            w64 = max(worst(wgroups, writer(P, wide, w, jj, k), 2, 64) for w in range(8) for jj in range(jt) for k in range(P))
+            w32 = max(worst(wgroups, writer(P, wide, w, jj, k), 2, 32) for w in range(8) for jj in range(jt) for k in range(P))
+            r64 = max(worst(READ_GROUPS, reader(P, wide, klo, rh, i), 4, 64) for klo in range(P) for rh in range(jt // 4) for i in range(16))
+            kld, pad = geom(P, wide)
+            print("P = %d  %-7s stores  row %3d points, pad %2d: ds_write_b64 %d-way (64 banks) %d-way (32 banks); ds_read_b128 %d-way"
+                  % (P, "16-byte" if wide else "8-byte", kld, pad, w64, w32, r64))
```

After: 201,200, median of 6. No clear change (+0.5%).
